# LouisBearing/BirdSoundClassif

Measured on AMD Instinct MI355X. Metric: clips/sec (3 s @ 22.05 kHz) detect fwd, higher is better.
Workload: dtype f32; 1 GPU; BASELINE.json configs[1]: 1xMI355X inference, batch=64 synthetic 3 s clips (PCM16 @22.05 kHz resident in HBM) through the HIP STFT front end + detector forward + device post-processing, detections returned to the host; batch_per_gpu=64, distinct_clips=64, lanes=2

## Files before the change

birdsoundclassif_amd/_lib.py:

```python
import ctypes as C
import os
import subprocess

_HERE = os.path.dirname(os.path.abspath(__file__))
LIB_PATH = os.environ.get('NBM_LIB') or os.path.join(_HERE, 'libnbm_hip.so')
CSRC = os.path.join(_HERE, 'csrc')

_lib = None


class GemmDesc(C.Structure):
    _fields_ = [('x', C.c_void_p), ('w', C.c_void_p), ('y', C.c_void_p),
                ('scale', C.c_void_p), ('shift', C.c_void_p), ('residual', C.c_void_p),
                ('x_gs', C.c_int64), ('w_gs', C.c_int64), ('y_gs', C.c_int64), ('res_gs', C.c_int64),
                ('groups', C.c_int),
                ('B', C.c_int), ('H', C.c_int), ('W', C.c_int), ('Cin', C.c_int),
                ('N', C.c_int),
                ('kh', C.c_int), ('kw', C.c_int), ('stride', C.c_int), ('pad', C.c_int),
                ('Ho', C.c_int), ('Wo', C.c_int),
                ('x_ld', C.c_int), ('w_ld', C.c_int), ('y_ld', C.c_int), ('res_ld', C.c_int),
                ('alpha', C.c_float), ('act', C.c_int), ('shift_per_row', C.c_int),
                ('up', C.c_void_p), ('up_H', C.c_int), ('up_W', C.c_int),
                ('rows', C.c_void_p), ('rows_blocks', C.c_void_p),
                ('rows_mode', C.c_int), ('rows_count', C.c_int), ('rows_TH', C.c_int), ('rows_TW', C.c_int),
                ('mask', C.c_void_p), ('mask_ld', C.c_int), ('bits_out', C.c_void_p)]


class GconvDesc(C.Structure):
    _fields_ = [('x', C.c_void_p), ('w', C.c_void_p), ('y', C.c_void_p), ('scale', C.c_void_p), ('shift', C.c_void_p),
                ('B', C.c_int), ('H', C.c_int), ('W', C.c_int), ('groups', C.c_int), ('Cg', C.c_int),
                ('kh', C.c_int), ('kw', C.c_int), ('stride', C.c_int), ('pad', C.c_int), ('Ho', C.c_int), ('Wo', C.c_int),
                ('x_ld', C.c_int), ('y_ld', C.c_int), ('relu', C.c_int)]


class GconvBwdDesc(C.Structure):
    _fields_ = [('g', C.c_void_p), ('y', C.c_void_p), ('w', C.c_void_p), ('x', C.c_void_p), ('out', C.c_void_p),
                ('scale', C.c_void_p), ('workspace', C.c_void_p), ('workspace_bytes', C.c_longlong),
                ('B', C.c_int), ('H', C.c_int), ('W', C.c_int), ('groups', C.c_int), ('Cg', C.c_int),
                ('kh', C.c_int), ('kw', C.c_int), ('stride', C.c_int), ('pad', C.c_int), ('Ho', C.c_int), ('Wo', C.c_int),
                ('g_ld', C.c_int), ('y_ld', C.c_int), ('x_ld', C.c_int), ('out_ld', C.c_int),
                ('accumulate', C.c_int), ('splits', C.c_int)]


class RoiDesc(C.Structure):
    _fields_ = [('fmap', C.c_void_p * 5), ('fh', C.c_int * 5), ('fw', C.c_int * 5),
                ('n_levels', C.c_int), ('C', C.c_int),
                ('rois', C.c_void_p), ('n_roi', C.c_void_p), ('B', C.c_int), ('roi_cap', C.c_int),
                ('pe_f', C.c_void_p), ('pe_t', C.c_void_p), ('img_h', C.c_int), ('img_w', C.c_int),
                ('pool', C.c_void_p), ('pe', C.c_void_p), ('level', C.c_void_p)]


class AugmentParams(C.Structure):
    _fields_ = [('gain', C.c_float), ('coef', C.c_float), ('denom', C.c_float), ('neg_coef', C.c_float),
                ('neg_denom', C.c_float), ('flags', C.c_int32), ('hard_index', C.c_int32), ('pad', C.c_int32),
                ('noise_seed', C.c_uint64)]


class BwdDesc(C.Structure):
    _fields_ = [('g', C.c_void_p), ('w', C.c_void_p), ('x', C.c_void_p), ('out', C.c_void_p),
                ('a_scale', C.c_void_p), ('row_scale', C.c_void_p), ('residual', C.c_void_p), ('mask', C.c_void_p),
                ('g_gs', C.c_int64), ('w_gs', C.c_int64), ('x_gs', C.c_int64), ('out_gs', C.c_int64), ('res_gs', C.c_int64),
                ('groups', C.c_int),
                ('B', C.c_int), ('H', C.c_int), ('W', C.c_int), ('Cin', C.c_int), ('N', C.c_int),
                ('kh', C.c_int), ('kw', C.c_int), ('stride', C.c_int), ('pad', C.c_int), ('Ho', C.c_int), ('Wo', C.c_int),
                ('g_ld', C.c_int), ('w_ld', C.c_int), ('x_ld', C.c_int), ('out_ld', C.c_int), ('res_ld', C.c_int),
                ('mask_ld', C.c_int), ('alpha', C.c_float), ('bias_grad', C.c_void_p), ('residual2', C.c_void_p), ('res2_ld', C.c_int),
                ('mask_bits', C.c_void_p)]


class GemmPlan(C.Structure):
    _fields_ = [('name', C.c_char_p), ('rc', C.c_int), ('kernel', C.c_int), ('grid', C.c_int * 3), ('block', C.c_int),
                ('m_tiles', C.c_int), ('n_tiles', C.c_int), ('vec_epi', C.c_int), ('fast', C.c_int), ('slices', C.c_int),
                ('phased', C.c_int), ('ph_tiles', C.c_int * 4), ('splits', C.c_int), ('k_chunk', C.c_int),
                ('plain', C.c_int), ('b_generic', C.c_int), ('narrow_m', C.c_int), ('halves', C.c_int)]


_P, _I, _L, _F, _U64 = C.c_void_p, C.c_int, C.c_int64, C.c_float, C.c_uint64

SIGNATURES = {
    'nbm_graph_census': [_P, C.POINTER(C.c_longlong * 6)],
    'nbm_copy_rect': [_P, _P, _L, _L, _I, _L, _L, _I, _I, _P],
    'nbm_gemm_conv': [C.POINTER(GemmDesc), _P],
    'nbm_gconv3x3': [C.POINTER(GconvDesc), _P],
    'nbm_gconv3x3_dgrad': [C.POINTER(GconvBwdDesc), _P],
    'nbm_gconv3x3_wgrad': [C.POINTER(GconvBwdDesc), _P],
    'nbm_gconv3x3_wgrad_workspace': [C.POINTER(GconvBwdDesc), C.POINTER(C.c_longlong)],
    'nbm_pcm16_to_wave': [_P, _L, _I, _I, _I, _P, _L, _L, _P, _L, _I, _I, _P],
    'nbm_resample_to_wave': [_P, _L, _I, _L, _I, _I, _P, _I, _L, _L, _P, _L, _I, _I, _I, _P],
    'nbm_wav_decode': [_P, _L, _I, _I, _I, _I, _L, _P, _L, _P],
    'nbm_minmax_init': [_P, _I, _P],
    'nbm_stft_db': [_P, _L, _I, _I, _I, _I, _P, _I, _I, _I, _F, _P, _L, _I, _P, _P],
    'nbm_spec_windows': [_P, _L, _I, _I, _I, _I, _P, _P, _I, _I, _I, _P, _P],
    'nbm_spec_windows_table': [_P, _I, _I, _P, _I, _I, _P],
    'nbm_init_conv': [_P, _L, _P, _P, _I, _P, _P],
    'nbm_stem7x7': [_P, _I, _I, _I, _P, _P, _P, _P, _P, _P, _P],
    'nbm_stem7x7_wgrad': [_P, _P, _I, _I, _I, _P, _P, _P],
    'nbm_maxpool3x3s2': [_P, _I, _I, _I, _I, _P, _I, _I, _P, _P],
    'nbm_space_to_batch2': [_P, _I, _I, _I, _I, _P, _I, _P],
    'nbm_avgpool2x2': [_P, _I, _I, _I, _I, _P, _P],
    'nbm_avgpool2x2_bwd': [_P, _I, _I, _I, _I, _P, _P],
    'nbm_upsample_bilinear_add': [_P, _I, _I, _I, _I, _P, _P, _I, _I, _P],
    'nbm_softmax_rows': [_P, _L, _I, _L, _P],
    'nbm_dwconv3x3': [_P, _I, _I, _I, _I, _I, _I, _P, _P, _P, _L, _P, _I, _I, _P],
    'nbm_silu': [_P, _P, _L, _P],
    'nbm_layernorm': [_P, _L, _I, _P, _P, _F, _P, _P],
    'nbm_mha_small': [_P, _P, _P, _I, _I, _I, _P, _I, _I, _I, _I, _I, _L, _L, _P, _F, _P],
    'nbm_mha_segments': [_P, _P, _P, _I, _I, _I, _P, _I, _I, _I, _I, _I, _I, _P, _P, _I, _F, _P],
    'nbm_pair_softmax': [_P, _L, _I, _I, _P, _I, _P],
    'nbm_rpn_decode': [_P, _P, _P, _I, _I, _I, _I, _I, _I, _P, _P, _P, _P],
    'nbm_nan_images': [_P, _I, _L, _P, _P],
    'nbm_rpn_select': [_P, _P, _P, _I, _I, _I, _I, _I, _P, _P, _P, _P, _P],
    'nbm_nms_batched': [_P, _P, _P, _I, _I, _F, _I, _P, _P, _P, _P, _P, _P, _P],
    'nbm_rpn_select_big_workspace': [_I, _I, C.POINTER(C.c_int64)],
    'nbm_rpn_select_big': [_P, _P, _P, _I, _I, _I, _I, _I, _P, _L, _P, _P, _P, _P, _P],
    'nbm_nms_big_workspace': [_I, _I, C.POINTER(C.c_int64)],
    'nbm_nms_big': [_P, _P, _P, _I, _I, _F, _I, _P, _L, _P, _P, _P, _P, _P],
    'nbm_roi_pool': [C.POINTER(RoiDesc), _P],
    'nbm_rcnn_post': [_P, _P, _I, _I, _P, _P, _I, _I, _I, _F, _F, _I, _P, _P, _P],
    'nbm_merge_collect': [_P, _P, _I, _I, _I, _I, _I, _L, _P, _P, _P, _P, _P, _P],
    'nbm_merge_nms_workspace': [_I, C.POINTER(C.c_int64)],
    'nbm_merge_nms': [_P, _P, _I, _F, _P, _L, _P, _P, _P],
    'nbm_merge_gather': [_P, _P, _P, _P, _P, _I, _P, _P, _P],
    'nbm_conv_dgrad': [C.POINTER(BwdDesc), _P],
    'nbm_conv_wgrad': [C.POINTER(BwdDesc), _P],
    'nbm_gemm_plan': [_I, _P, C.POINTER(GemmPlan)],
    'nbm_relu_bwd': [_P, _P, _P, _L, _P],
    'nbm_silu_bwd': [_P, _P, _P, _L, _P],
    'nbm_axpby': [_P, _P, _P, _F, _F, _L, _L, _P],
    'nbm_colsum': [_P, _L, _I, _I, _P, _P],
    'nbm_leaky_relu_bwd': [_P, _P, _P, _F, _L, _P],
    'nbm_layernorm_bwd': [_P, _P, _P, _L, _I, _F, _P, _P, _P, _P],
    'nbm_mha_small_bwd': [_P, _P, _P, _P, _I, _I, _I, _I, _P, _P, _P, _I, _I, _I, _P, _I, _I, _I, _I, _L, _L, _P, _F, _P],
    'nbm_zero_roi_windows': [_P, _I, _I, _I, _P, _P, _I, _I, _I, _P],
    'nbm_zero_pattern': [_P, _I, _I, _I, _I, _I, _P],
    'nbm_zero_tiles': [_P, _I, _I, _I, _I, _P, _I, _P, _P],
    'nbm_tiles_gather': [_P, _I, _I, _I, _I, _P, _I, _P, _P, _P],
    'nbm_tiles_scatter_add': [_P, _I, _I, _I, _I, _P, _I, _P, _P, _P],
    'nbm_proposal_iou': [_P, _P, _P, _I, _I, _I, _P, _P, _P],
    'nbm_anchor_targets': [_P, _I, _P, _P, _I, _I, _F, _F, _P, _P, _P, _P],
    'nbm_maxpool3x3s2_bwd': [_P, _P, _P, _I, _I, _I, _I, _I, _I, _P, _P, _P],
    'nbm_upsample_bilinear_bwd': [_P, _I, _I, _I, _I, _P, _I, _I, _I, _P],
    'nbm_tiles_upsample_bilinear_bwd_add': [_P, _I, _I, _I, _I, _P, _I, _P, _P, _I, _I, _P],
    'nbm_png_unfilter_gray8': [_P, _L, _I, _I, _I, _P, _L, _P, _P],
    'nbm_image_half_std_u8': [_P, _L, _I, _L, _P, _P],
    'nbm_randn_fill': [_U64, _L, _P, _P],
    'nbm_augment_batch': [_P, _P, _P, _I, _I, _I, _P, _P, _P, _P, _P, _P, _P],
    'nbm_u8_to_unit': [_P, _L, _P, _P],
    'nbm_wino_input': [_P, _I, _I, _I, _I, _P, _I, _P],
    'nbm_wino_output': [_P, _P, _P, _P, _I, _I, _I, _I, _I, _P, _I, _P, _P],
    'nbm_wino_outgrad': [_P, _I, _I, _I, _I, _P, _P, _I, _P],
    'nbm_wino_weight': [_P, _P, _I, _I, _I, _I, _P, _P],
    'nbm_wino_weight_grad': [_P, _P, _I, _I, _I, _P, _P],
    'nbm_wino23_rows': [_P, _I, _I, _I, _I, _P, _P],
    'nbm_wino23_conv_fused': [_P, _P, _P, _P, _P, _I, _I, _I, _I, _I, _I, _P, _I, _P],
    'nbm_wino23_rows_tiles': [_P, _I, _I, _I, _I, _P, _I, _P, _P, _P, _I, _P],
    'nbm_wino23_conv_fused_tiles': [_P, _P, _P, _P, _P, _I, _I, _I, _I, _I, _I, _P, _P, _I, _P, _P, _P],
    'nbm_roi_tiles': [_P, _P, _I, _I, _I, _I, _P, _P, _P, _I, _P, _P, _P],
    'nbm_wino23_input_tiles': [_P, _I, _I, _I, _I, _P, _I, _P, _P, _P],
    'nbm_wino23_outgrad_tiles': [_P, _I, _I, _I, _I, _P, _I, _P, _P, _P, _I, _P],
    'nbm_cell_outgrad': [_P, _I, _I, _I, _I, _I, _P, _P, _P],
    'nbm_cell_weight': [_P, _I, _I, _P, _I, _P, _I, _P],
    'nbm_cell_weight_fold': [_P, _P, _I, _I, _I, _I, _F, _P, _I, _P, _I, _P],
    'nbm_cell_weight_grad': [_P, _I, _I, _I, _P, _P],
    'nbm_cell_input': [_P, _I, _I, _I, _I, _I, _P, _I, _I, _P],
    'nbm_cell_input_up': [_P, _P, _I, _I, _I, _I, _I, _I, _I, _P, _I, _I, _P],
    'nbm_cell_patches': [_P, _I, _I, _I, _I, _I, _P, _I, _I, _P],
    'nbm_cell_patches_up': [_P, _P, _I, _I, _I, _I, _I, _I, _I, _P, _I, _I, _P],
    'nbm_cell_dgrad_output': [_P, _I, _I, _I, _I, _I, _P, _I, _I, _I, _P, _P],
    'nbm_cell_output': [_P, _P, _I, _I, _I, _I, _I, _P, _P],
    'nbm_weighted_sum': [_P, _P, _P, _P, _P, _L, _P],
    'nbm_weighted_sum_bwd': [_P, _P, _P, _P, _P, _P, _P, _P, _P, _L, _P],
    'nbm_softmax_rows_bwd': [_P, _P, _P, _L, _I, _F, _P],
    'nbm_pair_softmax_bwd': [_P, _P, _P, _L, _P],
    'nbm_dwconv3x3_bwd': [_P, _P, _P, _I, _I, _I, _I, _I, _I, _P, _P, _P, _I, _I, _P],
    'nbm_dwconv3x3_bwd_acc': [_P, _P, _I, _I, _I, _I, _I, _I, _P, _I, _I, _P],
    'nbm_film_fwd': [_P, _P, _P, _L, _I, _P],
    'nbm_film_bwd': [_P, _P, _P, _P, _P, _L, _I, _P],
    'nbm_bn_train_fwd': [_P, _L, _I, _P, _P, _F, _F, _P, _P, _P, _P, _P, _P, _P],
    'nbm_bn_train_bwd': [_P, _P, _L, _I, _P, _P, _P, _P, _P, _P, _P, _P],
    'nbm_roi_pool_bwd': [C.POINTER(C.c_void_p), C.POINTER(C.c_int), C.POINTER(C.c_int), _I, _I, _P, _P, _I, _I, _P, _P],
    'nbm_sqnorm_accum': [_P, _L, _P, _P],
    'nbm_adamw_step': [_P, _P, _P, _P, _L, _F, _F, _F, _F, _F, _I, _P, _F, _P],
}


def build(verbose=False):
    r = subprocess.run(['make', '-C', CSRC, '-j4'], capture_output=True, text=True)
    if verbose or r.returncode:
        print(r.stdout[-4000:], r.stderr[-4000:])
    if r.returncode:
        raise RuntimeError('building libnbm_hip.so failed')
    return LIB_PATH


def load():
    global _lib
    if _lib is not None:
        return _lib
    import torch
    if not os.path.isfile(LIB_PATH):
        raise RuntimeError(f'{LIB_PATH} is missing: build it with `python -c "import __graft_entry__ as g; g.build()"` '
                           '(the NBM hot path has no CPU / eager fallback)')
    lib = C.CDLL(LIB_PATH)
    lib.nbm_version.restype = C.c_char_p
    lib.nbm_version.argtypes = []
    for name, argtypes in SIGNATURES.items():
        fn = getattr(lib, name)
        fn.argtypes = argtypes
        fn.restype = C.c_int
    _lib = lib
    return lib


class NbmHipError(RuntimeError):
    pass


_CODES = {-1: 'NBM_EINVAL (bad argument / shape)', -2: 'NBM_EALIGN (pointer or pitch not 16-byte aligned)',
          -3: 'NBM_EUNSUPPORTED'}


def check(rc, name):
    if rc != 0:
        raise NbmHipError(f'{name} failed: {_CODES.get(rc, f"hipError_t {rc}")}')
```

birdsoundclassif_amd/csrc/igemm.hip:

```cpp
#include <stdlib.h>
#include "nbm_common.h"
#include "igemm_params.h"
#include "igemm_plan.h"
#include <type_traits>

namespace {

constexpr int BK = 32;
constexpr int PITCH = 36;

enum { A_FAST = 0, A_GENERIC = 1 };
enum { EPI_STD = 0 };

using nbm_igemm::IgemmParams;

template <int BM, int BN, int WM, int WN, int AMODE, int EPI, int STAGES = 2, bool ROWS = false>
__global__ __launch_bounds__(256, BM > 128 ? 1 : STAGES == 1 ? 3 : 2) void igemm_kernel(const IgemmParams p) {
  constexpr int MT = WM / 32, NT = WN / 32;
  constexpr int WAVES_N = BN / WN;
  constexpr int AR = BM / 32, BR = BN / 32;
  static_assert((BM / WM) * (BN / WN) == 4, "4 waves per workgroup");

  __shared__ __attribute__((aligned(16))) float lds[STAGES * (BM + BN) * PITCH];
  if constexpr (STAGES == 2) nbm_stagger_priority();
  float* As = lds;
  float* Bs = lds + STAGES * BM * PITCH;

  const int nwg = gridDim.x, bid = blockIdx.x;
  const int q8 = nwg >> 3, r8 = nwg & 7, xcd = bid & 7;
  const int wg = (xcd < r8 ? xcd * (q8 + 1) : r8 * (q8 + 1) + (xcd - r8) * q8) + (bid >> 3);
  int tile_m = wg / p.n_tiles, tile_n = wg - tile_m * p.n_tiles;
  auto row_pixel = [&](int m) -> long long {
    if (p.rows_mode == 1) return p.rows[m];
    const int t = p.rows[m >> 4];
    if (t < 0) return -1;
    const int thw = p.rows_TH * p.rows_TW, k = m & 15;
    const int b = (int)nbm_fdiv((unsigned)t, p.fd_rows_thw), rem = t - b * thw;
    const int ty = (int)nbm_fdiv((unsigned)rem, p.fd_rows_tw), tx = rem - ty * p.rows_TW;
    const int y = 2 * ty - 1 + (k >> 2), x = 2 * tx - 1 + (k & 3);
    if ((unsigned)y >= (unsigned)p.H || (unsigned)x >= (unsigned)p.W) return -1;
    return ((long long)b * p.H + y) * p.W + x;
  };
  if constexpr (ROWS) {
    if (p.rows_blocks) {
      const int j = bid >> 3;
      tile_n = j % p.n_tiles;
      tile_m = (j / p.n_tiles) * 8 + xcd;
      if (tile_m >= p.m_tiles || tile_m * (BM / 128) >= *p.rows_blocks * (p.rows_mode == 2 ? 16 : 1)) return;
    }
    if (p.rows[p.rows_mode == 2 ? (tile_m * BM) >> 4 : tile_m * BM] < 0) return;
  }
  const int bm0 = tile_m * BM, bn0 = tile_n * BN;
  const int g = blockIdx.z;

  const float* __restrict__ xg = p.x + (long long)g * p.x_gs;
  const float* __restrict__ wgp = p.w + (long long)g * p.w_gs;

  const int tid = threadIdx.x, lane = tid & 63, wave = tid >> 6;
  const int wm0 = (wave / WAVES_N) * WM, wn0 = (wave % WAVES_N) * WN;
  const int lrow = lane & 31, lh = lane >> 5;

  const int c4 = tid & 7, r0 = tid >> 3;
  long long a_base[AR];
  int a_iy0[AR], a_ix0[AR];
  bool a_ok[AR];
  unsigned a_rel[AR];
  unsigned long long a_taps[AR];
  long long blk_base = 0;
  if constexpr (ROWS) {
    const int e0 = p.rows[p.rows_mode == 2 ? bm0 >> 4 : bm0];
    const int b = (int)nbm_fdiv((unsigned)e0, p.rows_mode == 2 ? p.fd_rows_thw : p.fd_howo);
    blk_base = (long long)b * p.HoWo * p.x_ld;
  } else {
    const int m0 = bm0 < p.M ? bm0 : 0;
    const int b = (int)nbm_fdiv((unsigned)m0, p.fd_howo), rem = m0 - b * p.HoWo;
    const int oy = (int)nbm_fdiv((unsigned)rem, p.fd_wo), ox = rem - oy * p.Wo;
    blk_base = ((long long)(b * p.H + oy * p.stride - p.pad) * p.W + (ox * p.stride - p.pad)) * p.x_ld;
  }
#pragma unroll
  for (int i = 0; i < AR; ++i) {
    const int m = bm0 + r0 + 32 * i;
    a_ok[i] = m < p.M;
    long long mm = a_ok[i] ? m : 0;
    if constexpr (ROWS) {
      if (a_ok[i]) { mm = row_pixel(m); a_ok[i] = mm >= 0; }
      if (!a_ok[i]) mm = blk_base / p.x_ld;
    }
    const int b = (int)nbm_fdiv((unsigned)mm, p.fd_howo), rem = (int)(mm - (long long)b * p.HoWo);
    const int oy = (int)nbm_fdiv((unsigned)rem, p.fd_wo), ox = rem - oy * p.Wo;
    a_iy0[i] = oy * p.stride - p.pad;
    a_ix0[i] = ox * p.stride - p.pad;
    a_base[i] = ((long long)(b * p.H + a_iy0[i]) * p.W + a_ix0[i]) * p.x_ld;
    a_rel[i] = ((unsigned)(a_base[i] - blk_base) + c4 * 4) * 4u;
    unsigned long long mk = 0ull;
    if constexpr (AMODE == A_FAST) {
      unsigned rowm = 0u, colm = 0u;
      for (int r = 0; r < p.kh; ++r) rowm |= ((unsigned)(a_iy0[i] + r) < (unsigned)p.H ? 1u : 0u) << r;
      for (int s2 = 0; s2 < p.kw; ++s2) colm |= ((unsigned)(a_ix0[i] + s2) < (unsigned)p.W ? 1u : 0u) << s2;
      for (int r = 0; r < p.kh; ++r) mk |= ((rowm >> r) & 1u) ? (unsigned long long)colm << (r * p.kw) : 0ull;
      mk = a_ok[i] ? mk : 0ull;
    }
    a_taps[i] = mk;
  }
  const float* b_ptr[BR];
  bool b_ok[BR];
  unsigned b_rel[BR];
#pragma unroll
  for (int i = 0; i < BR; ++i) {
    const int n = bn0 + r0 + 32 * i;
    b_ok[i] = n < p.N;
    b_ptr[i] = wgp + (long long)(b_ok[i] ? n : 0) * p.w_ld + c4 * 4;
    b_rel[i] = b_ok[i] ? (unsigned)(n * p.w_ld + c4 * 4) * 4u : 0x80000000u;
  }
  const __amdgpu_buffer_rsrc_t rsrc_a = __builtin_amdgcn_make_buffer_rsrc(const_cast<float*>(xg + blk_base), 0, 0x7ffffff0, 0x00020000);
  const __amdgpu_buffer_rsrc_t rsrc_b = __builtin_amdgcn_make_buffer_rsrc(const_cast<float*>(wgp), 0, 0x7ffffff0, 0x00020000);

  f32x4 ra[AR], rb[BR];
  const f32x4 zero4 = {0.f, 0.f, 0.f, 0.f};

  int cur_r = 0, cur_s = 0, cur_c0 = 0;

  auto load_tiles = [&](int kt) {
    if constexpr (AMODE == A_FAST) {
      const int tap = cur_r * p.kw + cur_s;
      const unsigned a_soff = (unsigned)((((long long)cur_r * p.W + cur_s) * p.x_ld + cur_c0) * 4);
      const unsigned b_soff = (unsigned)((tap * p.Cin + cur_c0) * 4);
#pragma unroll
      for (int i = 0; i < AR; ++i) {
        const unsigned vo = ((a_taps[i] >> tap) & 1ull) ? a_rel[i] : 0x80000000u;
        ra[i] = __builtin_bit_cast(f32x4, __builtin_amdgcn_raw_buffer_load_b128(rsrc_a, vo, a_soff, 0));
      }
#pragma unroll
      for (int i = 0; i < BR; ++i)
        rb[i] = __builtin_bit_cast(f32x4, __builtin_amdgcn_raw_buffer_load_b128(rsrc_b, b_rel[i], b_soff, 0));
      if (++cur_s == p.kw) { cur_s = 0; if (++cur_r == p.kh) { cur_r = 0; cur_c0 += BK; } }
    } else {
      const int k0 = kt * BK + c4 * 4;
#pragma unroll
      for (int i = 0; i < AR; ++i) {
        f32x4 v = zero4;
#pragma unroll
        for (int e = 0; e < 4; ++e) {
          const int k = k0 + e;
          if (a_ok[i] && k < p.K) {
            const int tap = k / p.Cin, c = k - tap * p.Cin;
            const int r = tap / p.kw, s = tap - r * p.kw;
            const int iy = a_iy0[i] + r, ix = a_ix0[i] + s;
            if ((unsigned)iy < (unsigned)p.H && (unsigned)ix < (unsigned)p.W)
              v[e] = xg[a_base[i] + ((long long)r * p.W + s) * p.x_ld + c];
          }
        }
        ra[i] = v;
      }
#pragma unroll
      for (int i = 0; i < BR; ++i)
        rb[i] = b_ok[i] ? *reinterpret_cast<const f32x4*>(b_ptr[i] + kt * BK) : zero4;
    }
  };
  auto store_lds = [&](int buf) {
#pragma unroll
    for (int i = 0; i < AR; ++i)
      *reinterpret_cast<f32x4*>(As + (buf * BM + r0 + 32 * i) * PITCH + c4 * 4) = ra[i];
#pragma unroll
    for (int i = 0; i < BR; ++i)
      *reinterpret_cast<f32x4*>(Bs + (buf * BN + r0 + 32 * i) * PITCH + c4 * 4) = rb[i];
  };

  f32x16 acc[MT][NT];
#pragma unroll
  for (int i = 0; i < MT; ++i)
#pragma unroll
    for (int j = 0; j < NT; ++j)
#pragma unroll
      for (int e = 0; e < 16; ++e) acc[i][j][e] = 0.f;

  if constexpr (STAGES == 2) {
    load_tiles(0);
    store_lds(0);
    if (p.nk > 1) load_tiles(1);
  }

  auto mfma_group = [&](const float* Ab, const float* Bb, int q) {
    f32x4 a[MT], b[NT];
#pragma unroll
    for (int i = 0; i < MT; ++i) a[i] = *reinterpret_cast<const f32x4*>(Ab + i * 32 * PITCH + q * 4);
#pragma unroll
    for (int j = 0; j < NT; ++j) b[j] = *reinterpret_cast<const f32x4*>(Bb + j * 32 * PITCH + q * 4);
#pragma unroll
    for (int e = 0; e < 4; ++e)
#pragma unroll
      for (int i = 0; i < MT; ++i)
#pragma unroll
        for (int j = 0; j < NT; ++j)
          acc[i][j] = __builtin_amdgcn_mfma_f32_32x32x2f32(a[i][e], b[j][e], acc[i][j], 0, 0, 0);
  };

  auto k_step = [&](int kt, auto store_c, auto load_c) {
    constexpr bool STORE = decltype(store_c)::value, LOAD = decltype(load_c)::value;
    const int cur = kt & 1;
    __syncthreads();
    const float* Ab = As + (cur * BM + wm0 + lrow) * PITCH + lh * 16;
    const float* Bb = Bs + (cur * BN + wn0 + lrow) * PITCH + lh * 16;
    mfma_group(Ab, Bb, 0);
    if constexpr (STORE) {
      store_lds(cur ^ 1);
      __builtin_amdgcn_sched_group_barrier(0x100, MT + NT, 0);
#pragma unroll
      for (int z = 0; z < AR + BR; ++z) {
        __builtin_amdgcn_sched_group_barrier(0x008, (4 * MT * NT) / (AR + BR) > 0 ? (4 * MT * NT) / (AR + BR) : 1, 0);
        __builtin_amdgcn_sched_group_barrier(0x200, 1, 0);
      }
    }
    __builtin_amdgcn_sched_barrier(0);
    mfma_group(Ab, Bb, 1);
    if constexpr (LOAD) {
      load_tiles(kt + 2);
      __builtin_amdgcn_sched_group_barrier(0x100, MT + NT, 0);
#pragma unroll
      for (int z = 0; z < AR + BR; ++z) {
        __builtin_amdgcn_sched_group_barrier(0x008, (4 * MT * NT) / (AR + BR) > 0 ? (4 * MT * NT) / (AR + BR) : 1, 0);
        __builtin_amdgcn_sched_group_barrier(0x002, 3, 0);
        __builtin_amdgcn_sched_group_barrier(0x020, 1, 0);
      }
    }
    __builtin_amdgcn_sched_barrier(0);
    mfma_group(Ab, Bb, 2);
    mfma_group(Ab, Bb, 3);
  };
  if constexpr (STAGES == 2) {
    using T = std::true_type;
    using F = std::false_type;
    int kt = 0;
    for (; kt + 2 < p.nk; ++kt) k_step(kt, T{}, T{});
    if (p.nk >= 2) { k_step(kt, T{}, F{}); ++kt; }
    k_step(kt, F{}, F{});
  } else {
    load_tiles(0);
    for (int kt = 0; kt < p.nk; ++kt) {
      if (kt) __syncthreads();
      store_lds(0);
      if (kt + 1 < p.nk) load_tiles(kt + 1);
      __syncthreads();
      const float* Ab = As + (wm0 + lrow) * PITCH + lh * 16;
      const float* Bb = Bs + (wn0 + lrow) * PITCH + lh * 16;
#pragma unroll
      for (int q = 0; q < 4; ++q) mfma_group(Ab, Bb, q);
    }
  }
  __syncthreads();

#define NBM_EPI_LDS_FLOATS (STAGES * (BM + BN) * PITCH)
#include "igemm_epilogue.inc"
#undef NBM_EPI_LDS_FLOATS
}

struct StreamParams {
  const float* x; const float* w; float* y; const float* scale; const float* shift; const float* residual;
  int M, x_ld, w_ld, y_ld, res_ld, m_tiles; float alpha; int act;
  unsigned* bits_out; int n_words;
};
constexpr int SPITCH = 36;
template <int K32, int NT, int NTG, int WAVES>
__global__ __launch_bounds__(WAVES * 64, 1) void stream1x1_kernel(const StreamParams p) {
  constexpr int K = K32 * 32, N = NT * 32, WP = K + 4;
  constexpr bool CHUNKED = K32 > 2;
  static_assert(NT % NTG == 0 && (!CHUNKED || NTG == NT), "groups");
  __shared__ __attribute__((aligned(16))) float Ws[N * WP];
  __shared__ __attribute__((aligned(16))) float Stg[WAVES][32 * SPITCH];
  __shared__ __attribute__((aligned(16))) unsigned Bw[WAVES][32 * NT];
  const int tid = threadIdx.x, lane = tid & 63, wave = tid >> 6, li = lane & 31, lh = lane >> 5;
  const int n_off = blockIdx.y * N;
  for (int i = tid; i < N * (K / 4); i += WAVES * 64) {
    const int n = i / (K / 4), c = i - n * (K / 4);
    *reinterpret_cast<f32x4*>(Ws + n * WP + c * 4) = *reinterpret_cast<const f32x4*>(p.w + (long long)(n_off + n) * p.w_ld + c * 4);
  }
  __syncthreads();
  float* stg = Stg[wave];
  const int er = lane >> 3, ec = (lane & 7) * 4;
  f32x4 a[K32][4], an[CHUNKED ? 1 : K32][4];
  auto row_ptr = [&](int tile) {
    int m = tile * 32 + li;
    m = m < p.M ? m : p.M - 1;
    return p.x + (long long)m * p.x_ld + 16 * lh;
  };
  auto load_chunk = [&](const float* xp, int kc, f32x4* dst) {
#pragma unroll
    for (int q = 0; q < 4; ++q) dst[q] = *reinterpret_cast<const f32x4*>(xp + kc * 32 + 4 * q);
  };
  const int step = gridDim.x * WAVES;
  int tile = blockIdx.x * WAVES + wave;
  if (tile < p.m_tiles) {
    const float* xp = row_ptr(tile);
#pragma unroll
    for (int kc = 0; kc < K32; ++kc) load_chunk(xp, kc, CHUNKED ? a[kc] : an[kc]);
  }
  for (; tile < p.m_tiles; tile += step) {
    const bool more = tile + step < p.m_tiles;
    const float* xn = row_ptr(more ? tile + step : tile);
    if constexpr (!CHUNKED) {
#pragma unroll
      for (int kc = 0; kc < K32; ++kc)
#pragma unroll
        for (int q = 0; q < 4; ++q) a[kc][q] = an[kc][q];
#pragma unroll
      for (int kc = 0; kc < K32; ++kc) load_chunk(xn, kc, an[kc]);
    }
    const int m0 = tile * 32;
    f32x4 rq[NTG][4];
    auto load_res = [&](int jj, f32x4* dst) {
      if (!p.residual) return;
#pragma unroll
      for (int pass = 0; pass < 4; ++pass) {
        const int m = m0 + pass * 8 + er;
        dst[pass] = *reinterpret_cast<const f32x4*>(p.residual + (long long)(m < p.M ? m : p.M - 1) * p.res_ld + n_off + jj * 32 + ec);
      }
    };
#pragma unroll
    for (int g = 0; g < NT / NTG; ++g) {
#pragma unroll
      for (int j = 0; j < NTG; ++j) load_res(g * NTG + j, rq[j]);
      f32x16 acc[NTG];
#pragma unroll
      for (int j = 0; j < NTG; ++j)
#pragma unroll
        for (int e = 0; e < 16; ++e) acc[j][e] = 0.f;
      if constexpr (CHUNKED) {
#pragma unroll
        for (int kc = 0; kc < K32; ++kc) {
#pragma unroll
          for (int j = 0; j < NTG; ++j) {
            const float* wb = Ws + (j * 32 + li) * WP + 16 * lh + kc * 32;
            f32x4 b[4];
#pragma unroll
            for (int q = 0; q < 4; ++q) b[q] = *reinterpret_cast<const f32x4*>(wb + 4 * q);
#pragma unroll
            for (int q = 0; q < 4; ++q)
#pragma unroll
              for (int e = 0; e < 4; ++e) acc[j] = __builtin_amdgcn_mfma_f32_32x32x2f32(a[kc][q][e], b[q][e], acc[j], 0, 0, 0);
          }
          __builtin_amdgcn_sched_barrier(0);
          load_chunk(xn, kc, a[kc]);
          __builtin_amdgcn_sched_barrier(0);
        }
      } else {
#pragma unroll
        for (int j = 0; j < NTG; ++j) {
          const float* wb = Ws + ((g * NTG + j) * 32 + li) * WP + 16 * lh;
#pragma unroll
          for (int kc = 0; kc < K32; ++kc) {
            f32x4 b[4];
#pragma unroll
            for (int q = 0; q < 4; ++q) b[q] = *reinterpret_cast<const f32x4*>(wb + kc * 32 + 4 * q);
#pragma unroll
            for (int q = 0; q < 4; ++q)
#pragma unroll
              for (int e = 0; e < 4; ++e) acc[j] = __builtin_amdgcn_mfma_f32_32x32x2f32(a[kc][q][e], b[q][e], acc[j], 0, 0, 0);
          }
        }
      }
#pragma unroll
      for (int j = 0; j < NTG; ++j) {
        const int jj = g * NTG + j;
        __builtin_amdgcn_fence(__ATOMIC_ACQ_REL, "wavefront");
#pragma unroll
        for (int e = 0; e < 16; ++e) stg[((e & 3) + 8 * (e >> 2) + 4 * lh) * SPITCH + li] = acc[j][e];
        __builtin_amdgcn_fence(__ATOMIC_ACQ_REL, "wavefront");
        const int n = n_off + jj * 32 + ec;
        f32x4 sc = {1.f, 1.f, 1.f, 1.f}, sh = {0.f, 0.f, 0.f, 0.f};
        if (p.scale) sc = *reinterpret_cast<const f32x4*>(p.scale + n);
        if (p.shift) sh = *reinterpret_cast<const f32x4*>(p.shift + n);
#pragma unroll
        for (int pass = 0; pass < 4; ++pass) {
          const int r = pass * 8 + er, m = m0 + r;
          if (m >= p.M) continue;
          f32x4 v = *reinterpret_cast<const f32x4*>(stg + r * SPITCH + ec);
#pragma unroll
          for (int e = 0; e < 4; ++e) v[e] = (v[e] * p.alpha) * sc[e] + sh[e] + 0.f;
          if (p.residual) { v[0] += rq[j][pass][0]; v[1] += rq[j][pass][1]; v[2] += rq[j][pass][2]; v[3] += rq[j][pass][3]; }
          if (p.act == NBM_ACT_RELU) {
#pragma unroll
            for (int e = 0; e < 4; ++e) v[e] = fmaxf(v[e], 0.0f);
          } else if (p.act == NBM_ACT_SILU) {
#pragma unroll
            for (int e = 0; e < 4; ++e) v[e] = v[e] / (1.0f + expf(-v[e]));
          } else if (p.act == NBM_ACT_LEAKY) {
#pragma unroll
            for (int e = 0; e < 4; ++e) v[e] = v[e] > 0.f ? v[e] : 0.01f * v[e];
          }
          if (p.bits_out) {
            const int grp8 = 8 * er;
            const unsigned wb = ((unsigned)(__builtin_amdgcn_ballot_w64(v[0] > 0.f) >> grp8) & 0xffu) |
                                (((unsigned)(__builtin_amdgcn_ballot_w64(v[1] > 0.f) >> grp8) & 0xffu) << 8) |
                                (((unsigned)(__builtin_amdgcn_ballot_w64(v[2] > 0.f) >> grp8) & 0xffu) << 16) |
                                (((unsigned)(__builtin_amdgcn_ballot_w64(v[3] > 0.f) >> grp8) & 0xffu) << 24);
            if (ec == 0) Bw[wave][r * NT + jj] = wb;
          }
          *reinterpret_cast<f32x4*>(p.y + (long long)m * p.y_ld + n) = v;
        }
      }
    }
    if (p.bits_out) {
      static_assert(NT >= 2 && NT % 2 == 0, "two lanes per tile row");
      constexpr int WPL = NT / 2;
      __builtin_amdgcn_fence(__ATOMIC_ACQ_REL, "wavefront");
      const int r = lane >> 1, j0 = (lane & 1) * WPL;
      const int m = m0 + r;
      if (m < p.M) {
        unsigned* dst = p.bits_out + (long long)m * p.n_words + (n_off >> 5) + j0;
        const unsigned* src = Bw[wave] + r * NT + j0;
        if constexpr (WPL == 4) *reinterpret_cast<uint4*>(dst) = *reinterpret_cast<const uint4*>(src);
        else if constexpr (WPL == 2) *reinterpret_cast<uint2*>(dst) = *reinterpret_cast<const uint2*>(src);
        else {
#pragma unroll
          for (int q = 0; q < WPL; ++q) dst[q] = src[q];
        }
      }
      __builtin_amdgcn_fence(__ATOMIC_ACQ_REL, "wavefront");
    }
  }
}

}

using namespace nbm_igemm;

extern "C" int nbm_gemm_conv(const nbm_gemm_desc* d, void* stream) {
  if (!d) return NBM_EINVAL;
  const GemmPlan pl = plan_fwd(*d, read_gemm_switches(0));
  if (pl.rc) return pl.rc;
  if (pl.halves) {
    nbm_gemm_desc a = *d, b = *d;
    const int n0 = d->N - 64;
    a.N = n0;
    b.N = 64;
    b.w = d->w + (long long)n0 * d->w_ld;
    b.y = d->y + n0;
    if (d->scale) b.scale = d->scale + n0;
    if (d->shift) b.shift = d->shift + n0;
    if (d->residual) b.residual = d->residual + n0;
    if (d->mask) b.mask = d->mask + n0;
    const int rc = nbm_gemm_conv(&a, stream);
    return rc ? rc : nbm_gemm_conv(&b, stream);
  }
  const dim3 grid(pl.grid[0], pl.grid[1], pl.grid[2]), block(pl.block);
  hipStream_t st = (hipStream_t)stream;
  const int M = d->B * d->Ho * d->Wo;
  if (pl.slices) {
    const StreamParams sp{d->x, d->w, d->y, d->scale, d->shift, d->residual, M, d->x_ld, d->w_ld, d->y_ld, d->res_ld, pl.m_tiles,
                          d->alpha, d->act, d->bits_out, d->N >> 5};
    switch (pl.kernel) {
      case K_STREAM_64_256: hipLaunchKernelGGL((stream1x1_kernel<2, 8, 4, 8>), grid, block, 0, st, sp); break;
      case K_STREAM_64_64: hipLaunchKernelGGL((stream1x1_kernel<2, 2, 2, 8>), grid, block, 0, st, sp); break;
      case K_STREAM_128_SLICED: hipLaunchKernelGGL((stream1x1_kernel<4, 4, 4, 8>), grid, block, 0, st, sp); break;
      default: hipLaunchKernelGGL((stream1x1_kernel<8, 2, 2, 8>), grid, block, 0, st, sp); break;
    }
    return nbm_launch_status();
  }
  IgemmParams p{};
  p.x = d->x; p.w = d->w; p.y = d->y; p.scale = d->scale; p.shift = d->shift; p.residual = d->residual;
  p.x_gs = d->x_gs; p.w_gs = d->w_gs; p.y_gs = d->y_gs; p.res_gs = d->res_gs;
  p.M = M; p.N = d->N; p.K = d->kh * d->kw * d->Cin;
  p.nk = (p.K + BK - 1) / BK;
  p.H = d->H; p.W = d->W; p.Cin = d->Cin; p.kh = d->kh; p.kw = d->kw; p.stride = d->stride; p.pad = d->pad;
  p.Ho = d->Ho; p.Wo = d->Wo; p.HoWo = d->Ho * d->Wo;
  p.fd_howo = nbm_fastdiv_make((unsigned)p.HoWo); p.fd_wo = nbm_fastdiv_make((unsigned)p.Wo);
  p.x_ld = d->x_ld; p.w_ld = d->w_ld; p.y_ld = d->y_ld; p.res_ld = d->res_ld;
  p.alpha = d->alpha; p.act = d->act; p.shift_per_row = d->shift_per_row;
  p.m_tiles = pl.m_tiles; p.n_tiles = pl.n_tiles; p.vec_epi = pl.vec_epi;
  if (d->mask) { p.mask = d->mask; p.mask_ld = d->mask_ld; }
  p.bits_out = d->bits_out;
  if (d->up) {
    p.up = d->up; p.up_H = d->up_H; p.up_W = d->up_W;
    p.up_sh = d->Ho > 1 ? (float)(d->up_H - 1) / (float)(d->Ho - 1) : 0.f;
    p.up_sw = d->Wo > 1 ? (float)(d->up_W - 1) / (float)(d->Wo - 1) : 0.f;
  }
  if (d->rows) {
    p.rows = d->rows; p.rows_blocks = d->rows_blocks; p.rows_mode = d->rows_mode; p.rows_TH = d->rows_TH; p.rows_TW = d->rows_TW;
    p.fd_rows_thw = nbm_fastdiv_make((unsigned)(d->rows_TH * d->rows_TW)); p.fd_rows_tw = nbm_fastdiv_make((unsigned)d->rows_TW);
    p.M = d->rows_count;
  }
  switch (pl.kernel) {
    case K_FWD_ROWS: hipLaunchKernelGGL((igemm_kernel<128, 128, 64, 64, A_FAST, EPI_STD, 1, true>), grid, block, 0, st, p); break;
    case K_FWD_SPLIT_R0: case K_FWD_SPLIT_R2: case K_FWD_SPLIT_R4: return split_launch(p, pl, st);
    case K_FWD_H16: return h16_launch(p, pl, st);
    case K_FWD_128_S1: hipLaunchKernelGGL((igemm_kernel<128, 128, 64, 64, A_FAST, EPI_STD, 1>), grid, block, 0, st, p); break;
    case K_FWD_128_FAST: hipLaunchKernelGGL((igemm_kernel<128, 128, 64, 64, A_FAST, EPI_STD>), grid, block, 0, st, p); break;
    case K_FWD_128_GENERIC: hipLaunchKernelGGL((igemm_kernel<128, 128, 64, 64, A_GENERIC, EPI_STD>), grid, block, 0, st, p); break;
    case K_FWD_64_S1: hipLaunchKernelGGL((igemm_kernel<128, 64, 64, 32, A_FAST, EPI_STD, 1>), grid, block, 0, st, p); break;
    case K_FWD_64_FAST: hipLaunchKernelGGL((igemm_kernel<128, 64, 64, 32, A_FAST, EPI_STD>), grid, block, 0, st, p); break;
    case K_FWD_64_GENERIC: hipLaunchKernelGGL((igemm_kernel<128, 64, 64, 32, A_GENERIC, EPI_STD>), grid, block, 0, st, p); break;
    case K_FWD_32_FAST: hipLaunchKernelGGL((igemm_kernel<128, 32, 32, 32, A_FAST, EPI_STD>), grid, block, 0, st, p); break;
    case K_FWD_32_GENERIC: hipLaunchKernelGGL((igemm_kernel<128, 32, 32, 32, A_GENERIC, EPI_STD>), grid, block, 0, st, p); break;
    default: return NBM_EINVAL;
  }
  return nbm_launch_status();
}

extern "C" int nbm_gemm_plan(int kind, const void* desc, nbm_gemm_plan_t* out) {
  if (!desc || !out || kind < 0 || kind > 2) return NBM_EINVAL;
  const GemmSwitches sw = read_gemm_switches(kind);
  *out = kind == 0 ? plan_fwd(*(const nbm_gemm_desc*)desc, sw)
         : kind == 1 ? plan_dgrad(*(const nbm_bwd_desc*)desc, sw) : plan_wgrad(*(const nbm_bwd_desc*)desc, sw);
  return out->rc;
}
```

birdsoundclassif_amd/csrc/igemm_h16.hip:

```cpp
#include <stdlib.h>
#include "nbm_common.h"
#include "igemm_params.h"
#include <type_traits>

namespace {

using nbm_igemm::IgemmParams;
constexpr int BM = 128, BN = 128, WM = 64, WN = 64, MT = 2, NT = 2;
constexpr int P16 = 20;
enum { EPI_STD = 0 };

__global__ __launch_bounds__(256, 3) void igemm_h16_kernel(const IgemmParams p) {
  constexpr int STAGES = 1, EPI = EPI_STD;
  constexpr bool ROWS = false;
  __shared__ __attribute__((aligned(16))) float lds[2 * (BM + BN) * P16];
  float* As = lds;
  float* Bs = lds + 2 * BM * P16;

  const int nwg = gridDim.x, bid = blockIdx.x;
  const int q8 = nwg >> 3, r8 = nwg & 7, xcd = bid & 7;
  const int wg = (xcd < r8 ? xcd * (q8 + 1) : r8 * (q8 + 1) + (xcd - r8) * q8) + (bid >> 3);
  const int tile_m = wg / p.n_tiles, tile_n = wg - tile_m * p.n_tiles;
  const int bm0 = tile_m * BM, bn0 = tile_n * BN;
  const int g = blockIdx.z;
  const float* __restrict__ xg = p.x + (long long)g * p.x_gs;
  const float* __restrict__ wgp = p.w + (long long)g * p.w_gs;
  auto row_pixel = [&](int m) -> long long { return m; };

  const int tid = threadIdx.x, lane = tid & 63, wave = tid >> 6;
  const int wm0 = (wave >> 1) * WM, wn0 = (wave & 1) * WN;
  const int lrow = lane & 31, lh = lane >> 5;

  const int c = tid & 3, r0 = tid >> 2;
  const int koff = c < 2 ? 4 * c : 16 + 4 * (c - 2);
  long long blk_base;
  {
    const int m0 = bm0 < p.M ? bm0 : 0;
    const int b = (int)nbm_fdiv((unsigned)m0, p.fd_howo), rem = m0 - b * p.HoWo;
    const int oy = (int)nbm_fdiv((unsigned)rem, p.fd_wo), ox = rem - oy * p.Wo;
    blk_base = ((long long)(b * p.H + oy * p.stride - p.pad) * p.W + (ox * p.stride - p.pad)) * p.x_ld;
  }
  unsigned a_rel[2], b_rel[2];
  unsigned long long a_taps[2];
#pragma unroll
  for (int i = 0; i < 2; ++i) {
    const int m = bm0 + r0 + 64 * i;
    const bool ok = m < p.M;
    const int mm = ok ? m : 0;
    const int b = (int)nbm_fdiv((unsigned)mm, p.fd_howo), rem = mm - b * p.HoWo;
    const int oy = (int)nbm_fdiv((unsigned)rem, p.fd_wo), ox = rem - oy * p.Wo;
    const int iy0 = oy * p.stride - p.pad, ix0 = ox * p.stride - p.pad;
    const long long base = ((long long)(b * p.H + iy0) * p.W + ix0) * p.x_ld;
    a_rel[i] = ((unsigned)(base - blk_base) + koff) * 4u;
    unsigned rowm = 0u, colm = 0u;
    unsigned long long mk = 0ull;
    for (int r = 0; r < p.kh; ++r) rowm |= ((unsigned)(iy0 + r) < (unsigned)p.H ? 1u : 0u) << r;
    for (int s2 = 0; s2 < p.kw; ++s2) colm |= ((unsigned)(ix0 + s2) < (unsigned)p.W ? 1u : 0u) << s2;
    for (int r = 0; r < p.kh; ++r) mk |= ((rowm >> r) & 1u) ? (unsigned long long)colm << (r * p.kw) : 0ull;
    a_taps[i] = ok ? mk : 0ull;
    const int n = bn0 + r0 + 64 * i;
    b_rel[i] = n < p.N ? (unsigned)(n * p.w_ld + koff) * 4u : 0x80000000u;
  }
  const __amdgpu_buffer_rsrc_t rsrc_a = __builtin_amdgcn_make_buffer_rsrc(const_cast<float*>(xg + blk_base), 0, 0x7ffffff0, 0x00020000);
  const __amdgpu_buffer_rsrc_t rsrc_b = __builtin_amdgcn_make_buffer_rsrc(const_cast<float*>(wgp), 0, 0x7ffffff0, 0x00020000);

  f32x4 ra[2], rb[2];
  int cur_r = 0, cur_s = 0, cur_c0 = 0, cur_h = 0;
  auto load_tiles = [&]() {
    const int tap = cur_r * p.kw + cur_s;
    const unsigned a_soff = (unsigned)((((long long)cur_r * p.W + cur_s) * p.x_ld + cur_c0 + 8 * cur_h) * 4);
    const unsigned b_soff = (unsigned)((tap * p.Cin + cur_c0 + 8 * cur_h) * 4);
#pragma unroll
    for (int i = 0; i < 2; ++i) {
      const unsigned vo = ((a_taps[i] >> tap) & 1ull) ? a_rel[i] : 0x80000000u;
      ra[i] = __builtin_bit_cast(f32x4, __builtin_amdgcn_raw_buffer_load_b128(rsrc_a, vo, a_soff, 0));
    }
#pragma unroll
    for (int i = 0; i < 2; ++i)
      rb[i] = __builtin_bit_cast(f32x4, __builtin_amdgcn_raw_buffer_load_b128(rsrc_b, b_rel[i], b_soff, 0));
    if (cur_h ^= 1, cur_h == 0) {
      if (++cur_s == p.kw) { cur_s = 0; if (++cur_r == p.kh) { cur_r = 0; cur_c0 += 32; } }
    }
  };
  auto store_lds = [&](int buf) {
#pragma unroll
    for (int i = 0; i < 2; ++i) {
      *reinterpret_cast<f32x4*>(As + (buf * BM + r0 + 64 * i) * P16 + c * 4) = ra[i];
      *reinterpret_cast<f32x4*>(Bs + (buf * BN + r0 + 64 * i) * P16 + c * 4) = rb[i];
    }
  };

  f32x16 acc[MT][NT];
#pragma unroll
  for (int i = 0; i < MT; ++i)
#pragma unroll
    for (int j = 0; j < NT; ++j)
#pragma unroll
      for (int e = 0; e < 16; ++e) acc[i][j][e] = 0.f;

  auto mfma_group = [&](const float* Ab, const float* Bb, int q) {
    f32x4 a[MT], b[NT];
#pragma unroll
    for (int i = 0; i < MT; ++i) a[i] = *reinterpret_cast<const f32x4*>(Ab + i * 32 * P16 + q * 4);
#pragma unroll
    for (int j = 0; j < NT; ++j) b[j] = *reinterpret_cast<const f32x4*>(Bb + j * 32 * P16 + q * 4);
#pragma unroll
    for (int e = 0; e < 4; ++e)
#pragma unroll
      for (int i = 0; i < MT; ++i)
#pragma unroll
        for (int j = 0; j < NT; ++j)
          acc[i][j] = __builtin_amdgcn_mfma_f32_32x32x2f32(a[i][e], b[j][e], acc[i][j], 0, 0, 0);
  };

  auto h_step = [&](int t, auto store_c, auto load_c) {
    constexpr bool STORE = decltype(store_c)::value, LOAD = decltype(load_c)::value;
    const int cur = t & 1;
    __syncthreads();
    const float* Ab = As + (cur * BM + wm0 + lrow) * P16 + lh * 8;
    const float* Bb = Bs + (cur * BN + wn0 + lrow) * P16 + lh * 8;
    mfma_group(Ab, Bb, 0);
    if constexpr (STORE) {
      store_lds(cur ^ 1);
      __builtin_amdgcn_sched_group_barrier(0x100, MT + NT, 0);
#pragma unroll
      for (int z = 0; z < 4; ++z) {
        __builtin_amdgcn_sched_group_barrier(0x008, 4, 0);
        __builtin_amdgcn_sched_group_barrier(0x200, 1, 0);
      }
    }
    __builtin_amdgcn_sched_barrier(0);
    mfma_group(Ab, Bb, 1);
    if constexpr (LOAD) {
      load_tiles();
      __builtin_amdgcn_sched_group_barrier(0x100, MT + NT, 0);
#pragma unroll
      for (int z = 0; z < 4; ++z) {
        __builtin_amdgcn_sched_group_barrier(0x008, 4, 0);
        __builtin_amdgcn_sched_group_barrier(0x002, 3, 0);
        __builtin_amdgcn_sched_group_barrier(0x020, 1, 0);
      }
    }
    __builtin_amdgcn_sched_barrier(0);
  };
  {
    using T = std::true_type;
    using F = std::false_type;
    const int S = 2 * p.nk;
    load_tiles();
    store_lds(0);
    load_tiles();
    int t = 0;
    for (; t + 2 < S; ++t) h_step(t, T{}, T{});
    h_step(t, T{}, F{});
    ++t;
    h_step(t, F{}, F{});
  }
  __syncthreads();

#define NBM_EPI_LDS_FLOATS (2 * (BM + BN) * P16)
#include "igemm_epilogue.inc"
#undef NBM_EPI_LDS_FLOATS
}

}

int nbm_igemm::h16_launch(const IgemmParams& p, const GemmPlan& pl, hipStream_t st) {
  hipLaunchKernelGGL(igemm_h16_kernel, dim3(pl.grid[0], pl.grid[1], pl.grid[2]), dim3(256), 0, st, p);
  return nbm_launch_status();
}
```

birdsoundclassif_amd/csrc/igemm_params.h:

```cpp
#pragma once
#include "nbm_common.h"
#include "igemm_plan.h"

namespace nbm_igemm {

struct IgemmParams {
  const float* x; const float* w; float* y;
  const float* scale; const float* shift; const float* residual;
  long long x_gs, w_gs, y_gs, res_gs;
  int M, N, K;
  int nk;
  int H, W, Cin, kh, kw, stride, pad, Ho, Wo, HoWo;
  int x_ld, w_ld, y_ld, res_ld;
  int m_tiles, n_tiles;
  float alpha; int act; int shift_per_row;
  int vec_epi;
  const float* up; int up_H, up_W; float up_sh, up_sw;
  const int* rows; const int* rows_blocks; int rows_mode, rows_TH, rows_TW;
  const float* mask; int mask_ld;
  unsigned* bits_out;
  nbm_fastdiv fd_howo, fd_wo, fd_rows_thw, fd_rows_tw;
};

int split_launch(const IgemmParams& p, const GemmPlan& pl, hipStream_t st);

int h16_launch(const IgemmParams& p, const GemmPlan& pl, hipStream_t st);

}
```

birdsoundclassif_amd/csrc/igemm_plan.h:

```cpp
#pragma once
#include <stdint.h>
#include <stdlib.h>
#include "nbm_hip.h"

namespace nbm_igemm {

struct GemmSwitches { bool stream1x1, split_bf16, h16, nn_h16, split_tn; };
constexpr GemmSwitches kDefaultSwitches = {true, false, true, true, true};
inline bool switch_on(const char* v, bool dflt) { return dflt ? !(v && v[0] == '0') : (v && v[0] == '1'); }
inline GemmSwitches read_gemm_switches(int kind) {
  GemmSwitches s = kDefaultSwitches;
  if (kind == 0) {
    s.stream1x1 = switch_on(getenv("NBM_STREAM1X1"), true);
    s.split_bf16 = switch_on(getenv("NBM_SPLIT_BF16"), false);
    s.h16 = switch_on(getenv("NBM_H16"), true);
  } else if (kind == 1) {
    s.nn_h16 = switch_on(getenv("NBM_NN_H16"), true);
  } else {
    s.split_bf16 = switch_on(getenv("NBM_SPLIT_BF16"), false);
    s.split_tn = switch_on(getenv("NBM_SPLIT_TN"), true);
  }
  return s;
}

#define NBM_GEMM_KERNELS(X)                                                                                                          \
  X(K_FWD_ROWS, "igemm_kernel<128,128,64,64,0,0,1,true>")                                        \
  X(K_STREAM_64_256, "stream1x1_kernel<2,8,4,8>")                                          \
  X(K_STREAM_64_64, "stream1x1_kernel<2,2,2,8>")                                                \
  X(K_STREAM_256_64, "stream1x1_kernel<8,2,2,8>")                                                                     \
  X(K_STREAM_128_SLICED, "stream1x1_kernel<4,4,4,8>")                   \
  X(K_STREAM_256_SLICED, "stream1x1_kernel<8,2,2,8>")                     \
  X(K_FWD_SPLIT_R0, "igemm_split_kernel<0>")                                                        \
  X(K_FWD_SPLIT_R2, "igemm_split_kernel<2>")                                                                                         \
  X(K_FWD_SPLIT_R4, "igemm_split_kernel<4>")                                                                                         \
  X(K_FWD_H16, "igemm_h16_kernel")                                                                 \
  X(K_FWD_128_S1, "igemm_kernel<128,128,64,64,0,0,1,false>")                                              \
  X(K_FWD_128_FAST, "igemm_kernel<128,128,64,64,0,0,2,false>")                                                       \
  X(K_FWD_128_GENERIC, "igemm_kernel<128,128,64,64,1,0,2,false>")                                                                    \
  X(K_FWD_64_S1, "igemm_kernel<128,64,64,32,0,0,1,false>")                                                                           \
  X(K_FWD_64_FAST, "igemm_kernel<128,64,64,32,0,0,2,false>")                                                                         \
  X(K_FWD_64_GENERIC, "igemm_kernel<128,64,64,32,1,0,2,false>")                                                                      \
  X(K_FWD_32_FAST, "igemm_kernel<128,32,32,32,0,0,2,false>")                                                                         \
  X(K_FWD_32_GENERIC, "igemm_kernel<128,32,32,32,1,0,2,false>")                                                                      \
  X(K_NN_128_S1, "igemm_nn_kernel<128,1,false>")                                                                                     \
  X(K_NN_128_H16, "igemm_nn_kernel<128,2,true>")                                                                                     \
  X(K_NN_128, "igemm_nn_kernel<128,2,false>")                                                                                        \
  X(K_NN_64_S1, "igemm_nn_kernel<64,1,false>")                                                                                       \
  X(K_NN_64_H16, "igemm_nn_kernel<64,2,true>")                                                                                       \
  X(K_NN_64, "igemm_nn_kernel<64,2,false>")                                                                                          \
  X(K_TN_GENERIC, "igemm_tn_kernel<64,2,128>")                                                                                       \
  X(K_TN_128_SAME_M64, "igemm_tn_kernel<128,0,64>")                                                                                  \
  X(K_TN_128_STRIDED_M64, "igemm_tn_kernel<128,1,64>")                                                                               \
  X(K_TN_64_SAME_M64, "igemm_tn_kernel<64,0,64>")                                                                                    \
  X(K_TN_64_STRIDED_M64, "igemm_tn_kernel<64,1,64>")                                                                                 \
  X(K_TN_128_SAME, "igemm_tn_kernel<128,0,128>")                                                                                     \
  X(K_TN_128_STRIDED, "igemm_tn_kernel<128,1,128>")                                                                                  \
  X(K_TN_64_SAME, "igemm_tn_kernel<64,0,128>")                                                                                       \
  X(K_TN_64_STRIDED, "igemm_tn_kernel<64,1,128>")                                                                                    \
  X(K_SPLIT_TN_R0, "igemm_split_tn_kernel<0>")                              \
  X(K_SPLIT_TN_R2, "igemm_split_tn_kernel<2>")                                                                                       \
  X(K_SPLIT_TN_R4, "igemm_split_tn_kernel<4>")

enum GemmKernel {
#define X(id, name) id,
  NBM_GEMM_KERNELS(X)
#undef X
  K_COUNT
};
inline const char* gemm_kernel_name(int k) {
  static const char* const names[] = {
#define X(id, name) name,
      NBM_GEMM_KERNELS(X)
#undef X
  };
  return k >= 0 && k < K_COUNT ? names[k] : "";
}

constexpr int PLAN_BK = 32;
constexpr int SHORTK_STEPS = 8, DEEPK_STEPS = SHORTK_STEPS + 1;
constexpr int SHORTK_STEPS_64 = 20;
constexpr int SHORTK_STEPS_PHASED = 16;
constexpr int DEEPK_MAX_TAPS = 63;
constexpr int STREAM_MIN_ROWS = 8192;
constexpr int SPLIT_TN_MIN_ROWS = 192;
constexpr long long ROWS_SPAN_MAX = 0x7fffffffll;
constexpr long long DGRAD_SPAN_MAX = 0x70000000ll;
constexpr long long TN_SPAN_MAX = 0x40000000ll;

inline bool aligned16(const void* p) { return (((uintptr_t)p) & 15u) == 0; }

using GemmPlan = nbm_gemm_plan_t;

inline GemmPlan plan_error(int rc) {
  GemmPlan pl{};
  pl.rc = rc;
  pl.kernel = -1;
  pl.name = "";
  return pl;
}
inline void plan_kernel(GemmPlan& pl, int kernel, int gx, int gy, int gz, int block = 256) {
  pl.kernel = kernel;
  pl.name = gemm_kernel_name(kernel);
  pl.grid[0] = gx; pl.grid[1] = gy; pl.grid[2] = gz;
  pl.block = block;
}

inline GemmPlan plan_fwd(const nbm_gemm_desc& d, GemmSwitches sw) {
  if (!d.x || !d.w || !d.y) return plan_error(NBM_EINVAL);
  if (d.B <= 0 || d.H <= 0 || d.W <= 0 || d.Cin <= 0 || d.N <= 0 || d.kh <= 0 || d.kw <= 0 || d.stride <= 0 || d.Ho <= 0 || d.Wo <= 0 ||
      d.groups <= 0)
    return plan_error(NBM_EINVAL);
  if ((d.H + 2 * d.pad - d.kh) / d.stride + 1 != d.Ho || (d.W + 2 * d.pad - d.kw) / d.stride + 1 != d.Wo) return plan_error(NBM_EINVAL);
  if (d.x_ld < d.Cin || d.y_ld < d.N || (d.residual && d.res_ld < d.N)) return plan_error(NBM_EINVAL);
  GemmPlan pl{};
  const int taps = d.kh * d.kw, K = taps * d.Cin, nk = (K + PLAN_BK - 1) / PLAN_BK;
  if (d.N > 128 && (d.N & 127) == 64 && !d.rows && !d.up && !d.bits_out && !d.shift_per_row && (d.Cin % PLAN_BK) == 0 && K > SHORTK_STEPS * PLAN_BK) {
    nbm_gemm_desc a = d;
    a.N = d.N - 64;
    pl = plan_fwd(a, sw);
    pl.halves = 1;
    return pl;
  }
  if (d.w_ld < nk * PLAN_BK) return plan_error(NBM_EINVAL);
  if (d.mask && (d.rows || d.groups != 1 || d.mask_ld < d.N)) return plan_error(NBM_EUNSUPPORTED);
  pl.vec_epi = ((d.N & 3) == 0 && (d.y_ld & 3) == 0 && (d.y_gs & 3) == 0 && aligned16(d.y) &&
                (!d.residual || ((d.res_ld & 3) == 0 && (d.res_gs & 3) == 0 && aligned16(d.residual))) &&
                (!d.scale || aligned16(d.scale)) && (!d.shift || d.shift_per_row || aligned16(d.shift)) &&
                (!d.mask || ((d.mask_ld & 3) == 0 && aligned16(d.mask))))
                   ? 1 : 0;
  if ((d.w_ld & 3) || (d.w_gs & 3) || !aligned16(d.w)) return plan_error(NBM_EALIGN);
  if (d.bits_out && (!pl.vec_epi || (d.N & 31) || d.groups != 1 || d.rows)) return plan_error(NBM_EUNSUPPORTED);
  if (d.up && (!pl.vec_epi || d.groups != 1 || d.up_H <= 0 || d.up_W <= 0 || !aligned16(d.up))) return plan_error(NBM_EUNSUPPORTED);
  pl.fast = ((d.Cin % PLAN_BK) == 0 && (d.x_ld & 3) == 0 && (d.x_gs & 3) == 0 && aligned16(d.x)) ? 1 : 0;
  const bool fast_vec = pl.fast && pl.vec_epi;
  const int M = d.B * d.Ho * d.Wo;
  pl.m_tiles = (M + 127) / 128;
  if (d.rows) {
    if (d.kh != 1 || d.kw != 1 || d.stride != 1 || d.pad != 0 || d.groups != 1 || !fast_vec || d.shift_per_row || nk > SHORTK_STEPS ||
        d.N <= 64 || (d.rows_mode != 1 && d.rows_mode != 2) || d.rows_count <= 0 || (d.rows_count % 128))
      return plan_error(NBM_EUNSUPPORTED);
    if (d.rows_mode == 2 && (d.rows_TH != (d.H + 1) / 2 || d.rows_TW != (d.W + 1) / 2)) return plan_error(NBM_EINVAL);
    if (2ll * d.H * d.W * d.x_ld * 4 > ROWS_SPAN_MAX) return plan_error(NBM_EUNSUPPORTED);
    pl.m_tiles = d.rows_count / 128;
    pl.n_tiles = (d.N + 127) / 128;
    plan_kernel(pl, K_FWD_ROWS, (d.rows_blocks ? (pl.m_tiles + 7) / 8 * 8 : pl.m_tiles) * pl.n_tiles, 1, 1);
    return pl;
  }
  if (sw.stream1x1 && d.kh == 1 && d.kw == 1 && d.stride == 1 && d.pad == 0 && d.groups == 1 && fast_vec && !d.up && !d.mask &&
      !d.shift_per_row && (d.N % 32) == 0 && M >= STREAM_MIN_ROWS) {
    const int k32 = d.Cin / 32, nt = d.N / 32;
    int kernel = -1, wg_per_cu = 1, slices = 1;
    if (k32 == 2 && nt == 8 && d.residual) kernel = K_STREAM_64_256;
    else if (k32 == 2 && nt == 2) kernel = K_STREAM_64_64, wg_per_cu = 2;
    else if (k32 == 8 && nt == 2) kernel = K_STREAM_256_64;
    else if (d.residual && k32 == 4 && nt % 4 == 0 && nt <= 32) kernel = K_STREAM_128_SLICED, slices = nt / 4;
    else if (d.residual && k32 == 8 && nt % 2 == 0 && nt <= 64) kernel = K_STREAM_256_SLICED, slices = nt / 2;
    if (kernel >= 0) {
      const int waves = 8;
      pl.m_tiles = (M + 31) / 32;
      pl.slices = slices;
      const int wgs = (pl.m_tiles + waves - 1) / waves;
      int gx = 256 * wg_per_cu / slices;
      if (gx < 1) gx = 1;
      plan_kernel(pl, kernel, wgs < gx ? wgs : gx, slices, 1, waves * 64);
      return pl;
    }
  }
  if (d.N > 64) {
    pl.n_tiles = (d.N + 127) / 128;
    const bool deep = fast_vec && nk >= DEEPK_STEPS && taps < DEEPK_MAX_TAPS;
    if (sw.split_bf16 && deep) {
      pl.m_tiles = (M + 255) / 256;
      const int rem = (2 * nk) % 6;
      plan_kernel(pl, rem == 0 ? K_FWD_SPLIT_R0 : rem == 2 ? K_FWD_SPLIT_R2 : K_FWD_SPLIT_R4, pl.m_tiles * pl.n_tiles, 1, d.groups);
    }
    else if (sw.h16 && deep) plan_kernel(pl, K_FWD_H16, pl.m_tiles * pl.n_tiles, 1, d.groups);
    else if (fast_vec && nk <= SHORTK_STEPS) plan_kernel(pl, K_FWD_128_S1, pl.m_tiles * pl.n_tiles, 1, d.groups);
    else plan_kernel(pl, pl.fast ? K_FWD_128_FAST : K_FWD_128_GENERIC, pl.m_tiles * pl.n_tiles, 1, d.groups);
  } else if (d.N > 32) {
    pl.n_tiles = 1;
    if (fast_vec && nk <= SHORTK_STEPS_64) plan_kernel(pl, K_FWD_64_S1, pl.m_tiles, 1, d.groups);
    else plan_kernel(pl, pl.fast ? K_FWD_64_FAST : K_FWD_64_GENERIC, pl.m_tiles, 1, d.groups);
  } else {
    pl.n_tiles = 1;
    plan_kernel(pl, pl.fast ? K_FWD_32_FAST : K_FWD_32_GENERIC, pl.m_tiles, 1, d.groups);
  }
  return pl;
}

inline int check_bwd_common(const nbm_bwd_desc& d) {
  if (!d.g || !d.out) return NBM_EINVAL;
  if (d.B <= 0 || d.H <= 0 || d.W <= 0 || d.Cin <= 0 || d.N <= 0 || d.kh <= 0 || d.kw <= 0 || d.stride <= 0 || d.groups <= 0 ||
      d.kh * d.kw > 64)
    return NBM_EINVAL;
  if ((d.H + 2 * d.pad - d.kh) / d.stride + 1 != d.Ho || (d.W + 2 * d.pad - d.kw) / d.stride + 1 != d.Wo) return NBM_EINVAL;
  return NBM_OK;
}

inline GemmPlan plan_dgrad(const nbm_bwd_desc& d, GemmSwitches sw) {
  if (int rc = check_bwd_common(d)) return plan_error(rc);
  if (!d.w) return plan_error(NBM_EINVAL);
  if ((d.g_ld & 3) || d.g_ld < ((d.N + 31) / 32) * 32 || (d.Cin & 3) || (d.w_ld & 3) || (d.g_gs & 3) || (d.w_gs & 3) || !aligned16(d.g) ||
      !aligned16(d.w) || (d.a_scale && !aligned16(d.a_scale)))
    return plan_error(NBM_EALIGN);
  if (d.out_ld < d.Cin || (d.residual && d.res_ld < d.Cin) || (d.mask && d.mask_ld < d.Cin)) return plan_error(NBM_EINVAL);
  if (d.residual2 && (d.stride != 1 || d.groups != 1 || d.res2_ld < d.Cin)) return plan_error(NBM_EINVAL);
  if (d.a_scale && (d.N & 31)) return plan_error(NBM_EINVAL);
  if (d.mask_bits && ((d.Cin & 31) || d.groups != 1)) return plan_error(NBM_EUNSUPPORTED);
  {
    const long long row = (long long)d.Wo * d.g_ld * 4;
    const long long span = (d.W == 1 && d.kh == 1) ? 130ll * d.g_ld * 4
                                                    : (d.kh + 130) * row + (long long)d.Ho * row;
    if (span > DGRAD_SPAN_MAX) return plan_error(NBM_EUNSUPPORTED);
  }
  GemmPlan pl{};
  pl.vec_epi = ((d.out_ld & 3) == 0 && (d.out_gs & 3) == 0 && aligned16(d.out) &&
                (!d.residual || ((d.res_ld & 3) == 0 && (d.res_gs & 3) == 0 && aligned16(d.residual))) &&
                (!d.mask || ((d.mask_ld & 3) == 0 && aligned16(d.mask))) &&
                (!d.residual2 || ((d.res2_ld & 3) == 0 && aligned16(d.residual2)))) ? 1 : 0;
  pl.m_tiles = (d.B * d.H * d.W + 127) / 128;
  if (d.stride == 2) {
    pl.phased = 1;
    int tmax = 0;
    for (int ph = 0; ph < 4; ++ph) {
      const int y0 = ((ph >> 1) + d.pad) & 1, x0 = ((ph & 1) + d.pad) & 1;
      const int Hp = (d.H - y0 + 1) >> 1, Wp = (d.W - x0 + 1) >> 1;
      pl.ph_tiles[ph] = (int)(((long long)d.B * Hp * Wp + 127) / 128);
      if (pl.ph_tiles[ph] > tmax) tmax = pl.ph_tiles[ph];
    }
    pl.m_tiles = 4 * tmax;
  }
  const int n_steps = (d.N + PLAN_BK - 1) / PLAN_BK;
  const int ph_max = n_steps * ((d.kh + 1) / 2) * ((d.kw + 1) / 2);
  const bool shortk = pl.vec_epi && (pl.phased ? ph_max <= SHORTK_STEPS_PHASED
                                               : n_steps * d.kh * d.kw <= (d.Cin <= 64 ? SHORTK_STEPS_64 : SHORTK_STEPS));
  const bool hs = sw.nn_h16 && pl.vec_epi;
  const bool wide = d.Cin > 64;
  pl.n_tiles = wide ? (d.Cin + 127) / 128 : 1;
  plan_kernel(pl, wide ? (shortk ? K_NN_128_S1 : hs ? K_NN_128_H16 : K_NN_128) : (shortk ? K_NN_64_S1 : hs ? K_NN_64_H16 : K_NN_64),
              pl.m_tiles * pl.n_tiles, 1, d.groups);
  return pl;
}

inline int best_split(int M, int tiles, int slots, int rows_per_split_min) {
  const int max_splits = (M + rows_per_split_min - 1) / rows_per_split_min;
  int splits = 1;
  double best = -1.0;
  for (int sp = 1; sp <= max_splits && (long long)sp * tiles <= 16ll * slots; ++sp) {
    const long long wg = (long long)sp * tiles;
    const long long rounds = (wg + slots - 1) / slots;
    const double fill = (double)wg / (double)(rounds * slots);
    if (fill > best + 0.005) { best = fill; splits = sp; }
  }
  return splits;
}
inline void plan_splits(GemmPlan& pl, int M, int tiles, int slots, int rows_per_split_min) {
  const int sp = best_split(M, tiles, slots, rows_per_split_min);
  pl.k_chunk = (((M + sp - 1) / sp) + PLAN_BK - 1) / PLAN_BK * PLAN_BK;
  pl.splits = (M + pl.k_chunk - 1) / pl.k_chunk;
}

inline GemmPlan plan_wgrad(const nbm_bwd_desc& d, GemmSwitches sw) {
  if (int rc = check_bwd_common(d)) return plan_error(rc);
  if (!d.x) return plan_error(NBM_EINVAL);
  if ((d.g_ld & 3) || (d.g_gs & 3) || !aligned16(d.g) || d.g_ld < ((d.N + 3) / 4) * 4) return plan_error(NBM_EALIGN);
  GemmPlan pl{};
  pl.b_generic = ((d.Cin & 3) || (d.x_ld & 3) || (d.x_gs & 3) || !aligned16(d.x)) ? 1 : 0;
  const int taps = d.kh * d.kw;
  if (d.out_ld < taps * d.Cin) return plan_error(NBM_EINVAL);
  pl.plain = (taps == 1 && d.stride == 1 && d.pad == 0) ? 1 : 0;
  if (pl.plain && !pl.b_generic && d.Cin > 128 && (d.Cin & 127) == 64) {
    nbm_bwd_desc a = d;
    a.Cin = d.Cin - 64;
    pl = plan_wgrad(a, sw);
    pl.halves = 1;
    return pl;
  }
  const int M = d.B * d.Ho * d.Wo;
  if (sw.split_bf16 && sw.split_tn && pl.plain && !pl.b_generic && !d.bias_grad && d.N >= SPLIT_TN_MIN_ROWS && d.Cin > 64 && d.out_ld >= d.Cin &&
      32ll * d.g_ld * 4 < TN_SPAN_MAX && 32ll * d.x_ld * 4 < TN_SPAN_MAX) {
    pl.m_tiles = (d.N + 255) / 256;
    pl.n_tiles = (d.Cin + 127) / 128;
    plan_splits(pl, M, pl.m_tiles * pl.n_tiles * d.groups, 256, 16 * 32);
    const int rem = (pl.k_chunk >> 4) % 6;
    plan_kernel(pl, rem == 0 ? K_SPLIT_TN_R0 : rem == 2 ? K_SPLIT_TN_R2 : K_SPLIT_TN_R4, pl.m_tiles * pl.n_tiles, pl.splits, d.groups);
    return pl;
  }
  pl.narrow_m = (d.N <= 64 && !pl.b_generic) ? 1 : 0;
  pl.m_tiles = pl.narrow_m ? 1 : (d.N + 127) / 128;
  const bool wide = !pl.b_generic && d.Cin > 64;
  const int BN = wide ? 128 : 64;
  pl.n_tiles = pl.b_generic ? (taps * d.Cin + BN - 1) / BN : taps * ((d.Cin + BN - 1) / BN);
  plan_splits(pl, M, pl.m_tiles * pl.n_tiles * d.groups, 512, 8 * PLAN_BK);
  const bool same = !pl.b_generic && d.stride == 1 && d.Ho == d.H && d.Wo == d.W && (d.Wo >= PLAN_BK || pl.plain) &&
                    (long long)PLAN_BK * d.x_ld * 4 < TN_SPAN_MAX;
  const int kernel = pl.b_generic ? K_TN_GENERIC
                     : pl.narrow_m ? (wide ? (same ? K_TN_128_SAME_M64 : K_TN_128_STRIDED_M64) : (same ? K_TN_64_SAME_M64 : K_TN_64_STRIDED_M64))
                                   : (wide ? (same ? K_TN_128_SAME : K_TN_128_STRIDED) : (same ? K_TN_64_SAME : K_TN_64_STRIDED));
  plan_kernel(pl, kernel, pl.m_tiles * pl.n_tiles, pl.splits, d.groups);
  return pl;
}

}
```

birdsoundclassif_amd/csrc/pointwise.hip:

```cpp
#include <stdlib.h>
#include "nbm_common.h"

namespace {

constexpr int TPB = 256;
inline int grid_for(long long n, int per_block = TPB, int cap = 256 * 16) {
  long long g = (n + per_block - 1) / per_block;
  return (int)(g < 1 ? 1 : (g > cap ? cap : g));
}

__device__ __forceinline__ int pcm16_sample(const int16_t* __restrict__ x, int n, int upsample,
                                            const int32_t* __restrict__ hq, long long i) {
  if (!upsample) return x[i];
  if ((i & 1) == 0) return x[i >> 1];
  const int n0 = (int)(i >> 1);
  long long acc = 0;
#pragma unroll
  for (int k = 0; k < 16; ++k) {
    const int ia = n0 - k, ib = n0 + 1 + k;
    const int va = x[min(max(ia, 0), n - 1)], vb = x[min(max(ib, 0), n - 1)];
    const int xa = (ia >= 0 && ia < n) ? va : 0;
    const int xb = (ib >= 0 && ib < n) ? vb : 0;
    acc += (long long)hq[k] * (xa + xb);
  }
// ... 235 lines not shown
    long long t = pix;
    const int ox = (int)(t % Wo); t /= Wo;
    const int oy = (int)(t % Ho);
    const int b = (int)(t / Ho);
    const int ci = o / mult;
    float acc = 0.f;
#pragma unroll
    for (int r = 0; r < 3; ++r) {
      const int iy = oy * stride - 1 + r;
      if ((unsigned)iy >= (unsigned)H) continue;
#pragma unroll
      for (int s = 0; s < 3; ++s) {
        const int ix = ox * stride - 1 + s;
        if ((unsigned)ix >= (unsigned)W) continue;
        acc += x[((long long)(b * H + iy) * W + ix) * Cin + ci] * w[o * 9 + r * 3 + s];
      }
    }
    if (bias) acc += bias[o];
    if (film) acc = acc * film[pix * film_ld + o] + film[pix * film_ld + Cout + o];
    y[i] = acc;
  }
}

template <int MULT>
__global__ void dwconv3x3_vec_kernel(const float* __restrict__ x, int B, int H, int W, int Cin, int stride,
                                     const float* __restrict__ w, const float* __restrict__ bias,
                                     const float* __restrict__ film, long long film_ld, float* __restrict__ y,
                                     int Ho, int Wo) {
  constexpr int NIN = 4 / MULT;
  const int Cout = Cin * MULT, C4 = Cout >> 2;
  const long long total = (long long)B * Ho * Wo * C4;
  const long long gstride = (long long)gridDim.x * blockDim.x;
  const bool fixed_chunk = (gstride % C4) == 0;
  float wr[4][9];
  int w_chunk = -1;
  for (long long i = blockIdx.x * (long long)blockDim.x + threadIdx.x; i < total; i += gstride) {
    const int c4 = (int)(i % C4);
    const long long pix = i / C4;
    long long t = pix;
    const int ox = (int)(t % Wo); t /= Wo;
    const int oy = (int)(t % Ho);
    const int b = (int)(t / Ho);
    const int o0 = c4 * 4, ci0 = o0 / MULT;
    if (!fixed_chunk || w_chunk != c4) {
#pragma unroll
      for (int j = 0; j < 4; ++j)
#pragma unroll
        for (int k = 0; k < 9; ++k) wr[j][k] = w[(o0 + j) * 9 + k];
      w_chunk = c4;
    }
    float acc[4] = {0.f, 0.f, 0.f, 0.f};
    float xv[9][NIN];
#pragma unroll
    for (int r = 0; r < 3; ++r) {
      const int iyc = min(max(oy * stride - 1 + r, 0), H - 1);
#pragma unroll
      for (int s = 0; s < 3; ++s) {
        const int ixc = min(max(ox * stride - 1 + s, 0), W - 1);
        const float* xp = x + ((long long)(b * H + iyc) * W + ixc) * Cin + ci0;
        float* v = xv[r * 3 + s];
        if constexpr (NIN == 4) {
          const f32x4 q = *reinterpret_cast<const f32x4*>(xp);
          v[0] = q[0]; v[1] = q[1]; v[2] = q[2]; v[3] = q[3];
        } else if constexpr (NIN == 2) {
          const float2 q = *reinterpret_cast<const float2*>(xp);
          v[0] = q.x; v[1] = q.y;
        } else {
          v[0] = *xp;
        }
      }
    }
#pragma unroll
    for (int r = 0; r < 3; ++r) {
      const bool oky = (unsigned)(oy * stride - 1 + r) < (unsigned)H;
#pragma unroll
      for (int s = 0; s < 3; ++s) {
        const bool ok = oky && (unsigned)(ox * stride - 1 + s) < (unsigned)W;
#pragma unroll
        for (int j = 0; j < 4; ++j) acc[j] += (ok ? xv[r * 3 + s][j / MULT] : 0.f) * wr[j][r * 3 + s];
      }
    }
    f32x4 out = {acc[0], acc[1], acc[2], acc[3]};
    if (bias) {
      const f32x4 bv = *reinterpret_cast<const f32x4*>(bias + o0);
      out += bv;
    }
    if (film) {
      const f32x4 ga = *reinterpret_cast<const f32x4*>(film + pix * film_ld + o0);
      const f32x4 be = *reinterpret_cast<const f32x4*>(film + pix * film_ld + Cout + o0);
#pragma unroll
      for (int j = 0; j < 4; ++j) out[j] = out[j] * ga[j] + be[j];
    }
    *reinterpret_cast<f32x4*>(y + i * 4) = out;
  }
}

__global__ void layernorm_kernel(const float* __restrict__ x, long long rows, int E, const float* __restrict__ w,
                                 const float* __restrict__ b, float eps, float* __restrict__ y) {
  const int lane = threadIdx.x & 63;
  for (long long row = blockIdx.x * 4ll + (threadIdx.x >> 6); row < rows; row += (long long)gridDim.x * 4) {
    const float* r = x + row * E;
    float s = 0.f;
    for (int c = lane; c < E; c += 64) s += r[c];
    const float mean = nbm_wave_sum(s) / (float)E;
    float q = 0.f;
    for (int c = lane; c < E; c += 64) { const float d = r[c] - mean; q += d * d; }
    const float rstd = 1.0f / sqrtf(nbm_wave_sum(q) / (float)E + eps);
    float* o = y + row * E;
    for (int c = lane; c < E; c += 64) o[c] = (r[c] - mean) * rstd * w[c] + b[c];
  }
}

#define MHA_SMAX 128
__global__ __launch_bounds__(256) void mha_small_kernel(const float* __restrict__ q, const float* __restrict__ k,
                                                        const float* __restrict__ v, int q_ld, int k_ld, int v_ld,
                                                        float* __restrict__ out, int out_ld, int S, int nhead, int hd,
                                                        long long seq_stride, long long batch_stride,
                                                        const int* __restrict__ n_valid, float scale) {
  __shared__ float Ks[MHA_SMAX][65];
  __shared__ float Vs[MHA_SMAX][64];
  __shared__ float qs[4][64];
  __shared__ float ps[4][MHA_SMAX];
  const int n = blockIdx.x / nhead, h = blockIdx.x - n * nhead;
  const int nv = n_valid ? min(*n_valid, S) : S;
  const int lane = threadIdx.x & 63, wave = threadIdx.x >> 6;
  for (int i = threadIdx.x; i < nv * hd; i += 256) {
    const int j = i / hd, d = i - j * hd;
    const long long row = j * seq_stride + n * batch_stride;
    Ks[j][d] = k[row * k_ld + h * hd + d];
    Vs[j][d] = v[row * v_ld + h * hd + d];
  }
  __syncthreads();
  for (int r = wave; r < nv; r += 4) {
    const long long row = r * seq_stride + n * batch_stride;
    if (lane < hd) qs[wave][lane] = q[row * q_ld + h * hd + lane] * scale;
    __builtin_amdgcn_wave_barrier();
    float sc[MHA_SMAX / 64];
    float m = -INFINITY;
#pragma unroll
    for (int t = 0; t < MHA_SMAX / 64; ++t) {
      const int j = lane + 64 * t;
      float a = -INFINITY;
      if (j < nv) {
        a = 0.f;
        for (int d = 0; d < hd; ++d) a += qs[wave][d] * Ks[j][d];
      }
      sc[t] = a;
      m = fmaxf(m, a);
    }
    m = nbm_wave_max(m);
    float sum = 0.f;
#pragma unroll
    for (int t = 0; t < MHA_SMAX / 64; ++t) {
      const int j = lane + 64 * t;
      const float e = j < nv ? expf(sc[t] - m) : 0.f;
      if (j < nv) ps[wave][j] = e;
      sum += e;
    }
    sum = nbm_wave_sum(sum);
    __builtin_amdgcn_wave_barrier();
    if (lane < hd) {
      float o = 0.f;
      for (int j = 0; j < nv; ++j) o += ps[wave][j] * Vs[j][lane];
      out[row * out_ld + h * hd + lane] = o / sum;
    }
    __builtin_amdgcn_wave_barrier();
  }
}

#define MHA_SHORT 8
__device__ __forceinline__ void mha_segments_row(const float* __restrict__ qrow, float* __restrict__ orow, int hd, int nv,
                                                 float scale, const float (*Kp)[65], const float (*Vp)[64], float* qsw,
                                                 float* psw, int lane) {
  if (lane < hd) qsw[lane] = qrow[lane] * scale;
  __builtin_amdgcn_wave_barrier();
  float sc[MHA_SMAX / 64];
  float m = -INFINITY;
#pragma unroll
  for (int t = 0; t < MHA_SMAX / 64; ++t) {
    const int j = lane + 64 * t;
    float a = -INFINITY;
    if (j < nv) {
      a = 0.f;
      for (int d = 0; d < hd; ++d) a += qsw[d] * Kp[j][d];
    }
    sc[t] = a;
    m = fmaxf(m, a);
  }
  m = nbm_wave_max(m);
  float sum = 0.f;
#pragma unroll
  for (int t = 0; t < MHA_SMAX / 64; ++t) {
    const int j = lane + 64 * t;
    const float e = j < nv ? expf(sc[t] - m) : 0.f;
    if (j < nv) psw[j] = e;
    sum += e;
  }
  sum = nbm_wave_sum(sum);
  __builtin_amdgcn_wave_barrier();
  if (lane < hd) {
    float o = 0.f;
    for (int j = 0; j < nv; ++j) o += psw[j] * Vp[j][lane];
    orow[lane] = o / sum;
  }
  __builtin_amdgcn_wave_barrier();
}

__global__ __launch_bounds__(256) void mha_segments_kernel(const float* __restrict__ q, const float* __restrict__ k,
                                                           const float* __restrict__ v, int q_ld, int k_ld, int v_ld,
                                                           float* __restrict__ out, int out_ld, int B, int R, int nhead,
                                                           int hd, int mode, const int* __restrict__ segments,
                                                           const int* __restrict__ n_roi, int max_count, float scale) {
  __shared__ float Ks[MHA_SMAX][65];
  __shared__ float Vs[MHA_SMAX][64];
  __shared__ float qs[4][64];
  __shared__ float ps[4][MHA_SMAX];
  const int b = blockIdx.x / nhead, h = blockIdx.x - b * nhead;
  const int lane = threadIdx.x & 63, wave = threadIdx.x >> 6;
  const long long col = (long long)h * hd;
  int first = b, cnt = 1;
  bool ok = true;
  if (mode == NBM_MHA_ACROSS_IMAGES) {
    first = segments[b];
    cnt = segments[B + b];
    ok = first >= 0 && first <= b && cnt >= 1 && cnt <= max_count && b - first < cnt && first + cnt <= B;
  }
  const int n = ok ? min(max(n_roi[first], 0), R) : 0;
  for (int r = n + wave; r < R; r += 4)
    if (lane < hd) out[((long long)b * R + r) * out_ld + col + lane] = 0.f;
  if (mode == NBM_MHA_ACROSS_ROIS) {
    const long long row0 = (long long)b * R;
    for (int i = threadIdx.x; i < n * hd; i += 256) {
      const int j = i / hd, d = i - j * hd;
      Ks[j][d] = k[(row0 + j) * k_ld + col + d];
      Vs[j][d] = v[(row0 + j) * v_ld + col + d];
    }
    __syncthreads();
    for (int r = wave; r < n; r += 4)
      mha_segments_row(q + (row0 + r) * q_ld + col, out + (row0 + r) * out_ld + col, hd, n, scale, Ks, Vs, qs[wave],
                           ps[wave], lane);
    return;
  }
  const int me = b - first;
  if (cnt <= MHA_SHORT) {
    float(*Kw)[65] = Ks + wave * MHA_SHORT;
    float(*Vw)[64] = Vs + wave * MHA_SHORT;
    for (int r = me + wave * cnt; r < n; r += 4 * cnt) {
      if (lane < hd)
        for (int j = 0; j < cnt; ++j) {
          const long long row = (long long)(first + j) * R + r;
          Kw[j][lane] = k[row * k_ld + col + lane];
          Vw[j][lane] = v[row * v_ld + col + lane];
        }
      __builtin_amdgcn_wave_barrier();
      for (int i = 0; i < cnt; ++i) {
        const long long row = (long long)(first + i) * R + r;
        mha_segments_row(q + row * q_ld + col, out + row * out_ld + col, hd, cnt, scale, Kw, Vw, qs[wave], ps[wave], lane);
      }
    }
    return;
  }
  for (int r = me; r < n; r += cnt) {
    __syncthreads();
    for (int i = threadIdx.x; i < cnt * hd; i += 256) {
      const int j = i / hd, d = i - j * hd;
      const long long row = (long long)(first + j) * R + r;
      Ks[j][d] = k[row * k_ld + col + d];
      Vs[j][d] = v[row * v_ld + col + d];
    }
    __syncthreads();
    for (int i = wave; i < cnt; i += 4) {
      const long long row = (long long)(first + i) * R + r;
      mha_segments_row(q + row * q_ld + col, out + row * out_ld + col, hd, cnt, scale, Ks, Vs, qs[wave], ps[wave], lane);
    }
  }
}

__global__ void silu_kernel(const float* __restrict__ x, float* __restrict__ y, long long n) {
  for (long long i = blockIdx.x * (long long)blockDim.x + threadIdx.x; i < n;
       i += (long long)gridDim.x * blockDim.x) {
    const float v = x[i];
    y[i] = v / (1.0f + expf(-v));
  }
}

__global__ void pair_softmax_kernel(const float* __restrict__ x, long long n_pix, int n_anchor, int x_ld,
                                    float* __restrict__ y, int y_ld) {
  const long long total = n_pix * n_anchor;
  for (long long i = blockIdx.x * (long long)blockDim.x + threadIdx.x; i < total;
       i += (long long)gridDim.x * blockDim.x) {
    const long long p = i / n_anchor;
    const int a = (int)(i - p * n_anchor);
    const float v0 = x[p * x_ld + 2 * a], v1 = x[p * x_ld + 2 * a + 1];
    const float m = fmaxf(v0, v1);
    const float e0 = expf(v0 - m), e1 = expf(v1 - m);
    const float s = e0 + e1;
    y[p * y_ld + 2 * a] = e0 / s;
    y[p * y_ld + 2 * a + 1] = e1 / s;
  }
}

}

extern "C" const char* nbm_version(void) { return "nbm_hip 0.5 (gfx950)"; }

extern "C" int nbm_graph_census(void* graph, long long counts[6]) {
  if (!graph || !counts) return NBM_EINVAL;
  for (int i = 0; i < 6; ++i) counts[i] = 0;
  size_t n = 0;
  hipError_t e = hipGraphGetNodes((hipGraph_t)graph, nullptr, &n);
  if (e != hipSuccess) return (int)e;
  if (!n) return NBM_OK;
  hipGraphNode_t* nodes = (hipGraphNode_t*)malloc(n * sizeof(hipGraphNode_t));
  if (!nodes) return NBM_EINVAL;
  e = hipGraphGetNodes((hipGraph_t)graph, nodes, &n);
  for (size_t i = 0; e == hipSuccess && i < n; ++i) {
    hipGraphNodeType t;
    e = hipGraphNodeGetType(nodes[i], &t);
    if (e != hipSuccess) break;
    const int k = t == hipGraphNodeTypeKernel ? 0 : t == hipGraphNodeTypeMemcpy ? 1 : t == hipGraphNodeTypeMemset ? 2
                : t == hipGraphNodeTypeHost ? 3 : t == hipGraphNodeTypeEmpty ? 4 : 5;
    counts[k] += 1;
  }
  free(nodes);
  return e == hipSuccess ? NBM_OK : (int)e;
}

extern "C" int nbm_pcm16_to_wave(const int16_t* pcm, int64_t pcm_ld, int batch, int n, int upsample,
                                 const int32_t* hq, int64_t first, int64_t count, float* out, int64_t out_ld, int lead,
                                 int pad_mode, void* stream) {
  if (!pcm || !out || batch <= 0 || n <= 0 || lead < 0 || (upsample && !hq)) return NBM_EINVAL;
  const int64_t n_out = upsample ? 2 * (int64_t)n : n;
  if (first < 0 || count <= 0 || first + count > n_out) return NBM_EINVAL;
  if (pad_mode != 0 && pad_mode != 1) return NBM_EINVAL;
  if ((int64_t)lead + count + (pad_mode ? lead : 0) > out_ld) return NBM_EINVAL;
  if (pad_mode == 1 && lead >= count) return NBM_EINVAL;
  dim3 grid(grid_for(out_ld, TPB, 1024), batch);
  hipLaunchKernelGGL(pcm16_to_wave_kernel, grid, dim3(TPB), 0, (hipStream_t)stream, pcm, (long long)pcm_ld, n,
                     upsample, hq, (long long)first, (long long)count, out, (long long)out_ld, lead, pad_mode);
  return nbm_launch_status();
}

extern "C" int nbm_resample_to_wave(const float* x, int64_t x_ld, int batch, int64_t n, int L, int M, const double* taps,
                                    int T, int64_t first, int64_t count, float* out, int64_t out_ld, int lead, int pad_mode,
                                    int quant16, void* stream) {
  if (!x || !out || batch <= 0 || n <= 0 || L <= 0 || M <= 0 || lead < 0) return NBM_EINVAL;
  const bool copy = L == 1 && M == 1;
  if (!copy && (!taps || T <= 0 || (T & 1))) return NBM_EINVAL;
  const int64_t n_out = copy ? n : (n * L + M - 1) / M;
  if (first < 0 || count <= 0 || first + count > n_out) return NBM_EINVAL;
  if (pad_mode != 0 && pad_mode != 1) return NBM_EINVAL;
  if ((int64_t)lead + count + (pad_mode ? lead : 0) > out_ld) return NBM_EINVAL;
  if (pad_mode == 1 && lead >= count) return NBM_EINVAL;
  dim3 grid(grid_for(out_ld, TPB, 1024), batch);
  hipLaunchKernelGGL(resample_to_wave_kernel, grid, dim3(TPB), 0, (hipStream_t)stream, x, (long long)x_ld, (long long)n, L,
                     M, taps, T, (long long)first, (long long)count, out, (long long)out_ld, lead, pad_mode, quant16);
  return nbm_launch_status();
}

extern "C" int nbm_minmax_init(uint32_t* minmax, int batch, void* stream) {
  if (!minmax || batch <= 0) return NBM_EINVAL;
  hipLaunchKernelGGL(minmax_init_kernel, dim3((batch + 63) / 64), dim3(64), 0, (hipStream_t)stream, minmax, batch);
  return nbm_launch_status();
}

extern "C" int nbm_spec_windows(const float* db, int64_t db_bs, int db_ld, int batch, int n_bins, int n_frames,
                                const uint32_t* minmax, float* img, int n_img, int w_pix, int hop_img,
                                const int32_t* last_cols, void* stream) {
  if (!db || !minmax || !img || !last_cols || batch <= 0 || n_img <= 0 || n_frames <= 0) return NBM_EINVAL;
  if ((n_img - 1) * hop_img >= n_frames) return NBM_EINVAL;
  if ((n_img - 2) * (long long)hop_img + w_pix > n_frames && n_img > 1) return NBM_EINVAL;
  dim3 grid(grid_for((long long)n_bins * w_pix, TPB, 512), n_img, batch);
  hipLaunchKernelGGL(spec_windows_kernel, grid, dim3(TPB), 0, (hipStream_t)stream, db, (long long)db_bs, db_ld,
                     n_bins, minmax, img, n_img, w_pix, hop_img, last_cols);
  return nbm_launch_status();
}

extern "C" int nbm_spec_windows_table(const nbm_window_entry* table, int batch, int n_bins, float* img, int w_pix,
                                      int hop_img, void* stream) {
  if (!table || !img || batch <= 0 || n_bins <= 0 || w_pix <= 0 || hop_img <= 0) return NBM_EINVAL;
  dim3 grid(grid_for((long long)n_bins * w_pix, TPB, 512), batch);
  hipLaunchKernelGGL(spec_windows_table_kernel, grid, dim3(TPB), 0, (hipStream_t)stream, table, n_bins, img, w_pix, hop_img);
  return nbm_launch_status();
}

extern "C" int nbm_init_conv(const float* x, int64_t n_pix, const float* w, const float* b, int C, float* y,
                             void* stream) {
  if (!x || !w || !b || !y || n_pix <= 0 || C <= 0) return NBM_EINVAL;
  hipLaunchKernelGGL(init_conv_kernel, dim3(grid_for(n_pix * C)), dim3(TPB), 0, (hipStream_t)stream, x,
                     (long long)n_pix, w, b, C, y);
  return nbm_launch_status();
}

extern "C" int nbm_maxpool3x3s2(const float* x, int B, int H, int W, int C, float* y, int Ho, int Wo, uint8_t* idx,
                                void* stream) {
  if (!x || !y || B <= 0 || C <= 0 || (C & 3)) return NBM_EINVAL;
  if ((H + 2 - 3) / 2 + 1 != Ho || (W + 2 - 3) / 2 + 1 != Wo) return NBM_EINVAL;
  if (!nbm_aligned16(x) || !nbm_aligned16(y) || (((uintptr_t)idx) & 3u)) return NBM_EALIGN;
  if (idx)
    hipLaunchKernelGGL(maxpool3x3s2_kernel<true>, dim3(grid_for((long long)B * Ho * Wo * (C / 4))), dim3(TPB), 0,
                       (hipStream_t)stream, x, B, H, W, C / 4, y, Ho, Wo, idx);
  else
    hipLaunchKernelGGL(maxpool3x3s2_kernel<false>, dim3(grid_for((long long)B * Ho * Wo * (C / 4))), dim3(TPB), 0,
                       (hipStream_t)stream, x, B, H, W, C / 4, y, Ho, Wo, idx);
  return nbm_launch_status();
}

__global__ void space_to_batch2_kernel(const float* __restrict__ x, int B, int H, int W, int C4, float* __restrict__ y, int inverse) {
  const int Hh = H >> 1, Wh = W >> 1;
  const long long total = (long long)B * H * W * C4;
  const f32x4* x4 = reinterpret_cast<const f32x4*>(x);
  f32x4* y4 = reinterpret_cast<f32x4*>(y);
  for (long long i = blockIdx.x * (long long)blockDim.x + threadIdx.x; i < total; i += (long long)gridDim.x * blockDim.x) {
    const int c = (int)(i % C4);
    long long t = i / C4;
    const int xx = (int)(t % W); t /= W;
    const int yy = (int)(t % H);
    const int n = (int)(t / H);
    const long long packed = ((((long long)((yy & 1) * 2 + (xx & 1)) * B + n) * Hh + (yy >> 1)) * Wh + (xx >> 1)) * C4 + c;
    if (inverse) y4[i] = x4[packed]; else y4[packed] = x4[i];
  }
}

__global__ void avgpool2x2_kernel(const float* __restrict__ x, int B, int Ho, int Wo, int C4, float* __restrict__ y) {
  const long long total = (long long)B * Ho * Wo * C4;
  const f32x4* x4 = reinterpret_cast<const f32x4*>(x);
  f32x4* y4 = reinterpret_cast<f32x4*>(y);
  const int W = 2 * Wo;
  for (long long i = blockIdx.x * (long long)blockDim.x + threadIdx.x; i < total; i += (long long)gridDim.x * blockDim.x) {
    const int c = (int)(i % C4);
    long long t = i / C4;
    const int ox = (int)(t % Wo); t /= Wo;
    const int oy = (int)(t % Ho);
    const int b = (int)(t / Ho);
    const long long r0 = (((long long)b * 2 * Ho + 2 * oy) * W + 2 * ox) * C4 + c;
    const f32x4 a = x4[r0], b1 = x4[r0 + C4], c1 = x4[r0 + (long long)W * C4], d = x4[r0 + (long long)W * C4 + C4];
    f32x4 o;
#pragma unroll
    for (int e = 0; e < 4; ++e) o[e] = (((a[e] + b1[e]) + c1[e]) + d[e]) * 0.25f;
    y4[i] = o;
  }
}

extern "C" int nbm_space_to_batch2(const float* x, int B, int H, int W, int C, float* y, int inverse, void* stream) {
  if (!x || !y || B <= 0 || H <= 0 || W <= 0 || C <= 0 || (C & 3) || (H & 1) || (W & 1)) return NBM_EINVAL;
  if (!nbm_aligned16(x) || !nbm_aligned16(y)) return NBM_EALIGN;
  hipLaunchKernelGGL(space_to_batch2_kernel, dim3(grid_for((long long)B * H * W * (C / 4))), dim3(TPB), 0, (hipStream_t)stream, x, B, H, W,
                     C / 4, y, inverse ? 1 : 0);
  return nbm_launch_status();
}

extern "C" int nbm_avgpool2x2(const float* x, int B, int Ho, int Wo, int C, float* y, void* stream) {
  if (!x || !y || B <= 0 || Ho <= 0 || Wo <= 0 || C <= 0 || (C & 3)) return NBM_EINVAL;
  if (!nbm_aligned16(x) || !nbm_aligned16(y)) return NBM_EALIGN;
  hipLaunchKernelGGL(avgpool2x2_kernel, dim3(grid_for((long long)B * Ho * Wo * (C / 4))), dim3(TPB), 0, (hipStream_t)stream, x, B, Ho, Wo,
                     C / 4, y);
  return nbm_launch_status();
}

extern "C" int nbm_upsample_bilinear_add(const float* src, int B, int Hi, int Wi, int C, const float* add, float* y,
                                         int Ho, int Wo, void* stream) {
  if (!src || !y || B <= 0 || C <= 0 || (C & 3) || Hi <= 0 || Wi <= 0 || Ho <= 0 || Wo <= 0) return NBM_EINVAL;
  if (!nbm_aligned16(src) || !nbm_aligned16(y) || (add && !nbm_aligned16(add))) return NBM_EALIGN;
  const float sh = Ho > 1 ? (float)(Hi - 1) / (float)(Ho - 1) : 0.f;
  const float sw = Wo > 1 ? (float)(Wi - 1) / (float)(Wo - 1) : 0.f;
  hipLaunchKernelGGL(upsample_add_kernel, dim3(grid_for((long long)B * Ho * Wo * (C / 4))), dim3(TPB), 0,
                     (hipStream_t)stream, src, B, Hi, Wi, C / 4, add, y, Ho, Wo, sh, sw);
  return nbm_launch_status();
}

extern "C" int nbm_softmax_rows(float* x, int64_t rows, int cols, int64_t ld, void* stream) {
  if (!x || rows <= 0 || cols <= 0 || ld < cols) return NBM_EINVAL;
  hipLaunchKernelGGL(softmax_rows_kernel, dim3(grid_for(rows, 4, 256 * 32)), dim3(256), 0, (hipStream_t)stream, x,
                     (long long)rows, cols, (long long)ld);
  return nbm_launch_status();
}

extern "C" int nbm_dwconv3x3(const float* x, int B, int H, int W, int Cin, int mult, int stride, const float* w,
                             const float* bias, const float* film, int64_t film_ld, float* y, int Ho, int Wo,
                             void* stream) {
  if (!x || !w || !y || B <= 0 || Cin <= 0 || mult <= 0 || stride <= 0) return NBM_EINVAL;
  if ((H + 2 - 3) / stride + 1 != Ho || (W + 2 - 3) / stride + 1 != Wo) return NBM_EINVAL;
  if (film && film_ld < 2ll * Cin * mult) return NBM_EINVAL;
  const int Cout = Cin * mult;
  const bool vec = (mult == 1 || mult == 2 || mult == 4) && (Cout & 3) == 0 && (Cin % (4 / mult)) == 0 && nbm_aligned16(y) &&
                   nbm_aligned16(x) && (!bias || nbm_aligned16(bias)) && (!film || (nbm_aligned16(film) && (film_ld & 3) == 0));
  if (vec) {
    const dim3 grid(grid_for((long long)B * Ho * Wo * (Cout / 4))), blk(TPB);
    hipStream_t st = (hipStream_t)stream;
    if (mult == 1) hipLaunchKernelGGL(dwconv3x3_vec_kernel<1>, grid, blk, 0, st, x, B, H, W, Cin, stride, w, bias, film, (long long)film_ld, y, Ho, Wo);
    else if (mult == 2) hipLaunchKernelGGL(dwconv3x3_vec_kernel<2>, grid, blk, 0, st, x, B, H, W, Cin, stride, w, bias, film, (long long)film_ld, y, Ho, Wo);
    else hipLaunchKernelGGL(dwconv3x3_vec_kernel<4>, grid, blk, 0, st, x, B, H, W, Cin, stride, w, bias, film, (long long)film_ld, y, Ho, Wo);
    return nbm_launch_status();
  }
  hipLaunchKernelGGL(dwconv3x3_kernel, dim3(grid_for((long long)B * Ho * Wo * Cin * mult)), dim3(TPB), 0,
                     (hipStream_t)stream, x, B, H, W, Cin, mult, stride, w, bias, film, (long long)film_ld, y, Ho, Wo);
  return nbm_launch_status();
}

extern "C" int nbm_layernorm(const float* x, int64_t rows, int E, const float* w, const float* b, float eps, float* y,
                             void* stream) {
  if (!x || !w || !b || !y || rows <= 0 || E <= 0) return NBM_EINVAL;
  hipLaunchKernelGGL(layernorm_kernel, dim3(grid_for(rows, 4, 256 * 32)), dim3(256), 0, (hipStream_t)stream, x,
                     (long long)rows, E, w, b, eps, y);
  return nbm_launch_status();
}

extern "C" int nbm_mha_small(const float* q, const float* k, const float* v, int q_ld, int k_ld, int v_ld, float* out,
                             int out_ld, int S, int N, int nhead, int hd, int64_t seq_stride, int64_t batch_stride,
                             const int32_t* n_valid, float scale, void* stream) {
  if (!q || !k || !v || !out || S <= 0 || S > MHA_SMAX || N <= 0 || nhead <= 0 || hd <= 0 || hd > 64) return NBM_EINVAL;
  if (q_ld < nhead * hd || k_ld < nhead * hd || v_ld < nhead * hd || out_ld < nhead * hd) return NBM_EINVAL;
  hipLaunchKernelGGL(mha_small_kernel, dim3(N * nhead), dim3(256), 0, (hipStream_t)stream, q, k, v, q_ld, k_ld, v_ld, out,
                     out_ld, S, nhead, hd, (long long)seq_stride, (long long)batch_stride, n_valid, scale);
  return nbm_launch_status();
}

extern "C" int nbm_mha_segments(const float* q, const float* k, const float* v, int q_ld, int k_ld, int v_ld, float* out,
                                int out_ld, int B, int R, int nhead, int hd, int mode, const int32_t* segments,
                                const int32_t* n_roi, int max_count, float scale, void* stream) {
  if (!q || !k || !v || !out || !n_roi || B <= 0 || R <= 0 || nhead <= 0 || hd <= 0 || hd > 64) return NBM_EINVAL;
  if (q_ld < nhead * hd || k_ld < nhead * hd || v_ld < nhead * hd || out_ld < nhead * hd) return NBM_EINVAL;
  if (mode == NBM_MHA_ACROSS_ROIS) {
    if (R > MHA_SMAX) return NBM_EINVAL;
  } else if (mode == NBM_MHA_ACROSS_IMAGES) {
    if (!segments || max_count < 1 || max_count > MHA_SMAX) return NBM_EINVAL;
  } else {
    return NBM_EINVAL;
  }
  hipLaunchKernelGGL(mha_segments_kernel, dim3(B * nhead), dim3(256), 0, (hipStream_t)stream, q, k, v, q_ld, k_ld, v_ld, out,
                     out_ld, B, R, nhead, hd, mode, segments, n_roi, max_count, scale);
  return nbm_launch_status();
}

extern "C" int nbm_silu(const float* x, float* y, int64_t n, void* stream) {
  if (!x || !y || n <= 0) return NBM_EINVAL;
  hipLaunchKernelGGL(silu_kernel, dim3(grid_for(n)), dim3(TPB), 0, (hipStream_t)stream, x, y, (long long)n);
  return nbm_launch_status();
}

extern "C" int nbm_pair_softmax(const float* x, int64_t n_pix, int n_anchor, int x_ld, float* y, int y_ld,
                                void* stream) {
  if (!x || !y || n_pix <= 0 || n_anchor <= 0 || x_ld < 2 * n_anchor || y_ld < 2 * n_anchor) return NBM_EINVAL;
  hipLaunchKernelGGL(pair_softmax_kernel, dim3(grid_for(n_pix * n_anchor)), dim3(TPB), 0, (hipStream_t)stream, x,
                     (long long)n_pix, n_anchor, x_ld, y, y_ld);
  return nbm_launch_status();
}
```

birdsoundclassif_amd/nets/_prep.py:

```python
import weakref

import torch
import torch.nn.functional as F

_cache = {}
_epoch = 0


def bump():
    global _epoch
    _epoch += 1


_DEBUG = __import__('os').environ.get('NBM_PREP_DEBUG') == '1'


def _evict(obj_id):
    for k in [k for k in _cache if k[0] == obj_id]:
        hit = _cache.pop(k, None)
        if _DEBUG and hit is not None:
            v = hit[2]
            ts = [t for t in (v if isinstance(v, (tuple, list)) else [v]) if torch.is_tensor(t)]
            print(f'_prep: evicted {k[1]} (key tensor died), values at {[hex(t.data_ptr()) for t in ts]}', flush=True)


def _cached(key_t, tag, fn, extra=(), epoch=True):
    key = (id(key_t), tag)
    ver = (key_t.data_ptr(), key_t._version, key_t.device, _epoch if epoch else -1) + tuple(extra)
    hit = _cache.get(key)
    if hit is not None and hit[0]() is key_t and hit[1] == ver:
        return hit[2]
    with torch.no_grad():
        val = fn()
    if _DEBUG:
        cap = torch.cuda.is_available() and torch.cuda.is_current_stream_capturing()
        print(f'_prep: made {tag} for a {tuple(key_t.shape)} key (replaces an entry: {hit is not None}; during a capture: {cap})', flush=True)
    obj_id = id(key_t)
    _cache[key] = (weakref.ref(key_t, lambda _r, obj_id=obj_id: _evict(obj_id)), ver, val)
    return val


def krsc(weight):
    def make():
        co, ci, kh, kw = weight.shape
        w = weight.detach().permute(0, 2, 3, 1).reshape(co, kh * kw * ci)
        if ci % 32:
            w = F.pad(w, (0, (-w.shape[1]) % 32))
        return w.contiguous()
    return _cached(weight, 'krsc', make)


def _gconv_fragments(weight, groups):
    C, Cg, kh, kw = weight.shape
    if (kh, kw) != (3, 3) or C != groups * Cg or 16 % min(Cg, 16) or Cg % 16 not in (0, Cg) or C % 16:
        raise ValueError(f'gconv: no fragment layout for a {tuple(weight.shape)} weight in {groups} groups')
    w = weight.reshape(C, Cg, 9)
    CI = max(Cg, 16)
    if Cg < 16:
        same = (torch.arange(16, device=w.device)[None, :] // Cg) == ((torch.arange(C, device=w.device) % 16) // Cg)[:, None]
        w = w.repeat(1, 16 // Cg, 1) * same[:, :, None].to(w.dtype)
    return w.reshape(C // 16, 16, CI // 16, 4, 4, 9).permute(0, 5, 2, 3, 1, 4).reshape(C // 16, 9, CI // 16, 64, 4).contiguous()


def gconv(weight, groups):
    return _cached(weight, ('gconv', int(groups)), lambda: _gconv_fragments(weight.detach(), groups))


def gconv_dgrad(weight, groups, scale=None):
    def make():
        C, Cg, kh, kw = weight.shape
        if (kh, kw) != (3, 3) or C != groups * Cg:
            raise ValueError(f'gconv_dgrad: no fragment layout for a {tuple(weight.shape)} weight in {groups} groups')
        w = weight.detach().reshape(groups, Cg, Cg, 3, 3)
        if scale is not None:
            w = w * scale.detach().reshape(groups, Cg, 1, 1, 1)
        return _gconv_fragments(w.transpose(1, 2).flip(3, 4).reshape(C, Cg, 3, 3), groups)
    extra = () if scale is None else (scale.data_ptr(), scale._version)
    return _cached(weight, ('gconv_dgrad', int(groups), scale is not None), make, extra=extra)


def wino23(weight, transposed=False, m=2, scale=None):
    from .. import ops

    def make():
        return ops.wino_weight(weight.detach().contiguous(), transposed, m, None if scale is None else scale.detach().contiguous())
    extra = () if scale is None else (scale.data_ptr(), scale._version)
    return _cached(weight, ('wino', m, transposed, scale is not None), make, extra=extra)


def wino23_weight_grad(dU, m=2, row_scale=None):
    from .. import ops
    return ops.wino_weight_grad(dU, m, row_scale)


def cell_weight(weight, forward=False):
    from .. import ops
    return _cached(weight, ('cell', forward), lambda: ops.cell_weight(weight.detach().contiguous(), forward=forward))


def cell_weight_folded(w_out, wk_lat, alpha, transposed=False):
    from .. import ops
    pair = _cached(w_out, ('cellfold', float(alpha)),
                   lambda: ops.cell_weight(w_out.detach().contiguous(), lateral=wk_lat.detach(), alpha=alpha, both=True),
                   extra=(wk_lat.data_ptr(), wk_lat._version, tuple(wk_lat.shape)))
    return pair[1] if transposed else pair[0]


def cell_weight_grad(dU):
    from .. import ops
    return ops.cell_weight_grad(dU)


def stem_fold(w1, w_init, b_init):
    def make():
        w = w1.detach().double()
        a, b = w_init.detach().double().view(3), b_init.detach().double().view(3)
        we = (w * a.view(1, 3, 1, 1)).sum(1)
        wb = (w * b.view(1, 3, 1, 1)).sum(1)
        weff = torch.zeros((7, 8, 64), dtype=torch.float64, device=w.device)
        weff[:, :7] = we.permute(1, 2, 0)
        return (weff.view(56, 64).float().contiguous(), wb.reshape(64, 49).float().contiguous(), wb.sum((1, 2)).float().contiguous())
    return _cached(w1, 'stem', make, extra=(w_init.data_ptr(), w_init._version, b_init.data_ptr(), b_init._version))


def bn_affine(weight, bias, mean, var, eps, conv_bias=None, frozen=False):
    def make():
        scale = weight.detach() * (var + eps).rsqrt()
        shift = bias.detach() - mean * scale
        if conv_bias is not None:
            shift = shift + conv_bias.detach() * scale
        return scale.contiguous(), shift.contiguous()
    extra = (weight._version, bias._version, mean._version, var._version, None if conv_bias is None else conv_bias._version,
             mean.data_ptr(), var.data_ptr(), bias.data_ptr())
    return _cached(weight, ('bn', conv_bias is not None), make, extra=extra, epoch=not frozen)


def _rpn_composite64(out_w, out_b, dw_w, dw_b, pt_w, rmask, smask, lat_wk, alpha):
    n1, c = out_w.shape[0], out_w.shape[1]
    m_ = dw_w.shape[0]
    mult = m_ // n1
    wo = out_w.detach().double().repeat_interleave(mult, 0)
    wd = dw_w.detach().double().reshape(m_, 3, 3)
    bo = (out_b.detach().double() if out_b is not None else torch.zeros(n1, dtype=torch.float64, device=out_w.device)).repeat_interleave(mult)
    d = torch.zeros((m_, c, 5, 5), dtype=torch.float64, device=out_w.device)
    cb = torch.zeros((m_,), dtype=torch.float64, device=out_w.device)
    for r in range(3):
        for s_ in range(3):
            if (rmask >> r) & 1 and (smask >> s_) & 1:
                d[:, :, r:r + 3, s_:s_ + 3] += wd[:, r, s_, None, None, None] * wo
                cb += wd[:, r, s_] * bo
    if dw_b is not None:
        cb += dw_b.detach().double()
    wp = pt_w.detach().double().reshape(pt_w.shape[0], m_)
    we = torch.einsum('nm,mcae->naec', wp, d)
    const = wp @ cb
    if lat_wk is not None:
        wl = lat_wk.detach().double()
        we = torch.cat([we, float(alpha) * torch.einsum('naec,ci->naei', we, wl)], -1)
    return we, const


def _rpn_extra(out_b, dw_w, dw_b, pt_w, scale, shift, lat_wk, alpha):
    others = [t for t in (out_b, dw_w, dw_b, pt_w, scale, shift, lat_wk) if t is not None]
    return tuple(v for t in others for v in (t.data_ptr(), t._version)) + (float(alpha),)


def rpn_composite(out_w, out_b, dw_w, dw_b, pt_w, scale, shift, lat_wk=None, alpha=1.0, parts=None):
    def make():
        we, const = _rpn_composite64(out_w, out_b, dw_w, dw_b, pt_w, 7, 7, lat_wk, alpha)
        rng = parts if parts is not None else ((0, we.shape[-1]),)
        ws = tuple(we[..., c0:c1].reshape(we.shape[0], -1).float().contiguous() for c0, c1 in rng)
        return ws, scale, (scale.double() * const + shift.double()).float().contiguous()
    return _cached(out_w, ('rpnc', lat_wk is not None, parts), make, extra=_rpn_extra(out_b, dw_w, dw_b, pt_w, scale, shift, lat_wk, alpha))


def rpn_composite_delta(out_w, out_b, dw_w, dw_b, pt_w, scale, shift, rmask, smask, taps, lat_wk=None, alpha=1.0):
    def make():
        we, const = _rpn_composite64(out_w, out_b, dw_w, dw_b, pt_w, rmask, smask, lat_wk, alpha)
        wi, ci = _rpn_composite64(out_w, out_b, dw_w, dw_b, pt_w, 7, 7, lat_wk, alpha)
        d = (we - wi).reshape(we.shape[0], 25, -1)[:, list(taps)] * scale.double()[:, None, None]
        return d.reshape(d.shape[0], -1).float().contiguous(), (scale.double() * (const - ci)).float().contiguous()
    return _cached(out_w, ('rpnd', int(rmask), int(smask), tuple(taps), lat_wk is not None), make,
                   extra=_rpn_extra(out_b, dw_w, dw_b, pt_w, scale, shift, lat_wk, alpha))


def lateral_of_projection(lat_w, lat_b, proj_w, proj_b):
    def make():
        wl = lat_w.detach().double().reshape(lat_w.shape[0], -1)
        wc = wl @ proj_w.detach().double()
        sh = wl @ proj_b.detach().double() + (lat_b.detach().double() if lat_b is not None else 0.0)
        return wc.float().contiguous(), sh.float().contiguous()
    others = [t for t in (lat_b, proj_w, proj_b) if t is not None]
    return _cached(lat_w, 'latproj', make, extra=tuple(v for t in others for v in (t.data_ptr(), t._version)))


def value_of_lateral(lat_w, proj_w, val_w, val_b):
    def make():
        wlo = lat_w.detach().double().reshape(lat_w.shape[0], -1) @ proj_w.detach().double()
        return (wlo @ val_w.detach().double()).float().contiguous(), (wlo @ val_b.detach().double()).float().contiguous()
    others = [proj_w, val_w, val_b]
    return _cached(lat_w, 'vallat', make, extra=tuple(v for t in others for v in (t.data_ptr(), t._version)))


def cat_rows(tag, *tensors):
    def make():
        return torch.cat([t.detach().reshape(t.shape[0], -1) if t.dim() > 1 else t.detach() for t in tensors], 0).contiguous()
    extra = tuple(v for t in tensors for v in (t.data_ptr(), t._version))
    return _cached(tensors[0], ('cat', tag), make, extra=extra)


def clear():
    _cache.clear()
```

birdsoundclassif_amd/nets/backbone.py:

```python
import torch
from torch import nn

from .. import ops
from . import _prep, functional as Fn
from .position_encoding import build_position_encoding

bcbk_channels = {'resnet': {'2': 64, '3': 256, '4': 512, '5': 1024, '6': 2048}}
_RESNET_LAYERS = {'resnet50': [3, 4, 6, 3], 'resnet101': [3, 4, 23, 3], 'resnet152': [3, 8, 36, 3]}
_RESNEXT = {'resnext50_32x4d': ([3, 4, 6, 3], 32, 4), 'resnext101_32x8d': ([3, 4, 23, 3], 32, 8),
            'resnext101_64x4d': ([3, 4, 23, 3], 64, 4)}


class FrozenBatchNorm2d(nn.Module):

    def __init__(self, n):
        super().__init__()
        self.register_buffer('weight', torch.ones(n))
        self.register_buffer('bias', torch.zeros(n))
        self.register_buffer('running_mean', torch.zeros(n))
        self.register_buffer('running_var', torch.ones(n))

    def _load_from_state_dict(self, state_dict, prefix, local_metadata, strict, missing_keys, unexpected_keys,
                              error_msgs):
        state_dict.pop(prefix + 'num_batches_tracked', None)
        super()._load_from_state_dict(state_dict, prefix, local_metadata, strict, missing_keys, unexpected_keys,
                                      error_msgs)

    def affine(self):
        return _prep.bn_affine(self.weight, self.bias, self.running_mean, self.running_var, 1e-5, frozen=True)


class _Bottleneck(nn.Module):

    def __init__(self, inplanes, planes, stride, downsample, norm_layer):
        super().__init__()
        self.conv1 = nn.Conv2d(inplanes, planes, 1, bias=False)
        self.bn1 = norm_layer(planes)
        self.conv2 = nn.Conv2d(planes, planes, 3, stride=stride, padding=1, bias=False)
        self.bn2 = norm_layer(planes)
        self.conv3 = nn.Conv2d(planes, planes * 4, 1, bias=False)
        self.bn3 = norm_layer(planes * 4)
        self.downsample = downsample
        self.stride = stride
        self.mask_input, self.mask_gy = False, True

    def forward(self, x):
        if torch.is_grad_enabled() and x.dim() == 4 and self.conv1.weight.shape[0] % 32 == 0:
            ds = self.downsample
            sd, bd = ds[1].affine() if ds is not None else (None, None)
            return Fn.Bottleneck.apply(x, self.conv1.weight, self.conv2.weight, self.conv3.weight,
                                       ds[0].weight if ds is not None else None, *self.bn1.affine(), *self.bn2.affine(),
                                       *self.bn3.affine(), sd, bd, self.stride, self.mask_input, self.mask_gy)
        s, b = self.bn1.affine()
        o = Fn.conv(x, self.conv1.weight, scale=s, shift=b, act=ops.ACT_RELU)
        s, b = self.bn2.affine()
        if self.stride == 1 and Fn._winograd_ok(o, self.conv2.weight, 3, 3, 1, 1):
            o = ops.conv3x3_winograd(o, _prep.wino23(self.conv2.weight), b, scale=s, relu=True)
        else:
            o = Fn.conv(o, self.conv2.weight, scale=s, shift=b, kh=3, kw=3, stride=self.stride, pad=1, act=ops.ACT_RELU)
        if self.downsample is not None:
            s, b = self.downsample[1].affine()
            idt = Fn.conv(x, self.downsample[0].weight, scale=s, shift=b, stride=self.stride)
        else:
            idt = x
        s, b = self.bn3.affine()
        return Fn.conv(o, self.conv3.weight, scale=s, shift=b, residual=idt, act=ops.ACT_RELU)


class _GroupedBottleneck(nn.Module):

    def __init__(self, inplanes, planes, stride, downsample, norm_layer, groups, base_width):
        super().__init__()
        width = int(planes * base_width / 64) * groups
        self.conv1 = nn.Conv2d(inplanes, width, 1, bias=False)
        self.bn1 = norm_layer(width)
        self.conv2 = nn.Conv2d(width, width, 3, stride=stride, padding=1, groups=groups, bias=False)
        self.bn2 = norm_layer(width)
        self.conv3 = nn.Conv2d(width, planes * 4, 1, bias=False)
        self.bn3 = norm_layer(planes * 4)
        self.downsample = downsample
        self.stride, self.groups = stride, groups
        self.mask_input, self.mask_gy = False, True

    def forward(self, x):
        grad = torch.is_grad_enabled() and (x.requires_grad or any(p.requires_grad for p in self.parameters()))
        if grad and not self.training:
            raise NotImplementedError('a ResNeXt block in eval mode has no backward pass: call .train() on the model to train through it '
                                      '(FrozenBN makes the two modes compute the same), or train with --lr_backbone 0 (a frozen '
                                      'backbone), or run it under torch.no_grad()')
        s, b = self.bn1.affine()
        o = Fn.conv(x, self.conv1.weight, scale=s, shift=b, act=ops.ACT_RELU)
        s, b = self.bn2.affine()
        if grad:
            o = Fn.GConv3x3.apply(o, self.conv2.weight, s, b, self.groups, self.stride)
        else:
            o = ops.gconv3x3(o, _prep.gconv(self.conv2.weight, self.groups), self.groups, stride=self.stride, scale=s, shift=b, relu=True)
        if self.downsample is not None:
            s, b = self.downsample[1].affine()
            idt = Fn.conv(x, self.downsample[0].weight, scale=s, shift=b, stride=self.stride)
        else:
            idt = x
        s, b = self.bn3.affine()
        return Fn.conv(o, self.conv3.weight, scale=s, shift=b, residual=idt, act=ops.ACT_RELU)


class _ResNetBody(nn.Module):

    def __init__(self, layers, norm_layer, dilation=False, groups=1, base_width=64):
        super().__init__()
        self.conv1 = nn.Conv2d(3, 64, 7, stride=2, padding=3, bias=False)
        self.bn1 = norm_layer(64)
        self.dilation = bool(dilation)
        inplanes = 64
        for li, (planes, n, stride) in enumerate(zip((64, 128, 256, 512), layers, (1, 2, 2, 1 if dilation else 2)), start=1):
            blocks = []
            for bi in range(n):
                st = stride if bi == 0 else 1
                ds = None
                if bi == 0 and (st != 1 or inplanes != planes * 4):
                    ds = nn.Sequential(nn.Conv2d(inplanes, planes * 4, 1, stride=st, bias=False), norm_layer(planes * 4))
                blocks.append(_Bottleneck(inplanes, planes, st, ds, norm_layer) if groups == 1 else
                              _GroupedBottleneck(inplanes, planes, st, ds, norm_layer, groups, base_width))
                if dilation and li == 4 and bi > 0:
                    blocks[-1].conv2.dilation, blocks[-1].conv2.padding = (2, 2), (2, 2)
                blocks[-1].mask_input = not (li == 1 and bi == 0)
                blocks[-1].mask_gy = bi == n - 1
                inplanes = planes * 4
            setattr(self, f'layer{li}', nn.Sequential(*blocks))

    def forward(self, x, init_conv=None):
        s, b = self.bn1.affine()
        if init_conv is not None:
            x = Fn.Stem.apply(x, init_conv.weight, init_conv.bias, self.conv1.weight, s, b)
        else:
            x = Fn.conv(x, self.conv1.weight, scale=s, shift=b, kh=7, kw=7, stride=2, pad=3, act=ops.ACT_RELU)
        taps = [x]
        x = Fn.MaxPool.apply(x, True)
        for li in range(1, 5):
            for bi, blk in enumerate(getattr(self, f'layer{li}')):
                if self.dilation and li == 4 and bi == 1:
                    x = Fn.SpaceToBatch2.apply(x, False)
                x = blk(x)
            if self.dilation and li == 4 and len(self.layer4) > 1:
                x = Fn.SpaceToBatch2.apply(x, True)
            taps.append(x)
        return taps


class BackboneBase(nn.Module):

    def __init__(self, backbone, name, in_channels, train_backbone):
        super().__init__()
        for _, parameter in backbone.named_parameters():
            if not train_backbone:
                parameter.requires_grad_(False)
        self.body = backbone
        self.num_channels = list(bcbk_channels['resnet'].values())
        if in_channels != 3:
            self.init_conv = nn.Conv2d(in_channels, 3, 1)
        self.in_channels = in_channels
        self.strides = [2 ** (i + 1) for i in range(len(self.num_channels))]

    def forward(self, x):
        if hasattr(self, 'init_conv'):
            if self.in_channels != 1:
                raise NotImplementedError('init_conv is implemented for 1 input channel (reference default)')
            return self.body(x, self.init_conv)
        return self.body(x)


class Backbone(BackboneBase):

    def __init__(self, name, in_channels, train_backbone, dilation, norm_layer_name):
        if name not in _RESNET_LAYERS and name not in _RESNEXT:
            raise ValueError(f'not supported {name}: the accelerated path implements {sorted(_RESNET_LAYERS) + sorted(_RESNEXT)}')
        if norm_layer_name != 'frozen_batchnorm':
            raise NotImplementedError('only --norm_layer_backbone frozen_batchnorm (reference default) is implemented')
        layers, groups, base_width = _RESNEXT[name] if name in _RESNEXT else (_RESNET_LAYERS[name], 1, 64)
        super().__init__(_ResNetBody(layers, FrozenBatchNorm2d, dilation=dilation, groups=groups, base_width=base_width), name,
                         in_channels, train_backbone)
        if groups > 1 and not train_backbone and hasattr(self, 'init_conv'):
            self.init_conv.requires_grad_(False)


class Joiner(nn.Sequential):
    def __init__(self, backbone, position_embedding):
        super().__init__(backbone, position_embedding)

    def forward(self, x):
        return self[0](x), None


def build_backbone(args):
    position_embedding = build_position_encoding(args)
    train_backbone = args.lr_backbone > 0
    backbone = Backbone(args.backbone, args.inpt_channels, train_backbone, args.dilation, args.norm_layer_backbone)
    model = Joiner(backbone, position_embedding)
    model.num_channels = backbone.num_channels
    model.strides = backbone.strides
    setattr(args, 'n_layers', len(backbone.num_channels))
    return model
```

birdsoundclassif_amd/ops.py:

```python
import collections
import ctypes as C
import os
import math

import torch

from . import _lib
from ._lib import GconvBwdDesc, GconvDesc, GemmDesc, RoiDesc, check

ACT_NONE, ACT_RELU, ACT_SILU, ACT_LEAKY = 0, 1, 2, 3

PROFILE = None
FLOPS = None
FLOPS_DEFERRED = []


def flops_total():
    tot = FLOPS[0] + sum(float(c.item()) * f for c, f in FLOPS_DEFERRED)
    FLOPS_DEFERRED.clear()
    return tot


_PROFILE_LABEL = None
PROFILE_ONLY = None


def _prof_all():
    return PROFILE is not None and PROFILE_ONLY is None


def _prof_fused():
    return PROFILE is not None and PROFILE_ONLY in (None, 'fused')


def is_deepk(Cin, N, kh, kw, rows=None):
    return rows is None and N > 64 and Cin % 32 == 0 and kh * kw * Cin > 256



def _stream():
    return C.c_void_p(torch.cuda.current_stream().cuda_stream)


def _ptr(t):
    return C.c_void_p(t.data_ptr()) if t is not None else C.c_void_p(0)


def _chk(t, dtype=torch.float32, name='tensor'):
    if not (isinstance(t, torch.Tensor) and t.is_cuda):
        raise RuntimeError(f'{name}: the NBM HIP path needs CUDA (ROCm) tensors; no CPU fallback exists')
    if t.dtype != dtype:
        raise TypeError(f'{name}: expected {dtype}, got {t.dtype}')
    if not t.is_contiguous():
        raise ValueError(f'{name}: must be contiguous')
    return t


def lib():
    return _lib.load()


def gemm_conv(x, w, y, *, B, H, W, Cin, N, kh=1, kw=1, stride=1, pad=0, Ho=None, Wo=None,
              x_ld=None, w_ld=None, y_ld=None, scale=None, shift=None, residual=None, res_ld=None,
              groups=1, x_gs=0, w_gs=0, y_gs=0, res_gs=0, alpha=1.0, act=ACT_NONE, shift_per_row=False, up=None,
              rows=None, rows_mode=0, rows_count=0, rows_blocks=None, rows_thw=(0, 0), mask=None, mask_ld=None, bits_out=None):
    Ho = (H + 2 * pad - kh) // stride + 1 if Ho is None else Ho
    Wo = (W + 2 * pad - kw) // stride + 1 if Wo is None else Wo
    d = GemmDesc()
    d.x, d.w, d.y = x.data_ptr(), w.data_ptr(), y.data_ptr()
    d.scale = scale.data_ptr() if scale is not None else None
    d.shift = shift.data_ptr() if shift is not None else None
    d.residual = residual.data_ptr() if residual is not None else None
    d.x_gs, d.w_gs, d.y_gs, d.res_gs = x_gs, w_gs, y_gs, res_gs
    d.groups = groups
    d.B, d.H, d.W, d.Cin, d.N = B, H, W, Cin, N
    d.kh, d.kw, d.stride, d.pad, d.Ho, d.Wo = kh, kw, stride, pad, Ho, Wo
    d.x_ld = Cin if x_ld is None else x_ld
    d.w_ld = kh * kw * Cin if w_ld is None else w_ld
    d.y_ld = N if y_ld is None else y_ld
    d.res_ld = (N if res_ld is None else res_ld) if residual is not None else 0
    d.alpha, d.act, d.shift_per_row = float(alpha), int(act), int(bool(shift_per_row))
    if up is not None:
        d.up, d.up_H, d.up_W = _chk(up, name='up').data_ptr(), up.shape[1], up.shape[2]
    if mask is not None:
        d.mask, d.mask_ld = mask.data_ptr(), int(N if mask_ld is None else mask_ld)
    if bits_out is not None:
        assert bits_out.dtype == torch.int32 and bits_out.is_contiguous() and bits_out.numel() * 32 >= B * Ho * Wo * N and N % 32 == 0
        d.bits_out = bits_out.data_ptr()
    if rows is not None:
        d.rows, d.rows_mode, d.rows_count = rows.data_ptr(), int(rows_mode), int(rows_count)
        d.rows_blocks = rows_blocks.data_ptr() if rows_blocks is not None else None
        d.rows_TH, d.rows_TW = rows_thw
    if FLOPS is not None:
        if rows is None:
            FLOPS[0] += 2.0 * B * Ho * Wo * N * kh * kw * Cin * groups
        elif rows_blocks is None:
            FLOPS[0] += 2.0 * rows_count * N * Cin
        else:
            FLOPS_DEFERRED.append((rows_blocks.clone(), 2.0 * 128 * (16 if rows_mode == 2 else 1) * N * Cin))
    if _prof_all() or (PROFILE is not None and PROFILE_ONLY == 'deepk' and is_deepk(Cin, N, kh, kw, rows)):
        ev0, ev1 = torch.cuda.Event(enable_timing=True), torch.cuda.Event(enable_timing=True)
        ev0.record()
        check(lib().nbm_gemm_conv(C.byref(d), _stream()), 'nbm_gemm_conv')
        ev1.record()
        if rows is None:
            PROFILE.append(((Cin, N, kh, H, W, B, groups, stride, _PROFILE_LABEL), ev0, ev1))
        elif rows_blocks is None:
            PROFILE.append(((Cin, N, kh, rows_count, 1, 1, groups, stride, ('rows', H, W)), ev0, ev1))
        else:
            PROFILE.append(((Cin, N, kh, 0, 1, 1, groups, stride, ('rows-rois', H, W)), ev0, ev1))
        return y
    check(lib().nbm_gemm_conv(C.byref(d), _stream()), 'nbm_gemm_conv')
    return y


def conv2d(x, w, kh=1, kw=1, stride=1, pad=0, scale=None, shift=None, residual=None, act=ACT_NONE,
           alpha=1.0, out=None, w_ld=None, up=None, bits_out=None):
    _chk(x, name='x'), _chk(w, name='w')
    B, H, W, Cin = x.shape
    N = w.shape[0]
    Ho = (H + 2 * pad - kh) // stride + 1
    Wo = (W + 2 * pad - kw) // stride + 1
    y = out if out is not None else torch.empty((B, Ho, Wo, N), device=x.device, dtype=torch.float32)
    if residual is not None:
        _chk(residual, name='residual')
        assert residual.shape == y.shape
    gemm_conv(x, w, y, B=B, H=H, W=W, Cin=Cin, N=N, kh=kh, kw=kw, stride=stride, pad=pad, Ho=Ho, Wo=Wo,
              w_ld=w.shape[1] if w_ld is None else w_ld, scale=scale, shift=shift, residual=residual,
              alpha=alpha, act=act, up=up, bits_out=bits_out)
    return y


def gconv3x3(x, w_prepared, groups, stride=1, scale=None, shift=None, relu=False, out=None, kh=3, kw=3, pad=1):
    _chk(x, name='x'), _chk(w_prepared, name='w_prepared')
    if x.dim() != 4 or w_prepared.dim() != 5 or tuple(w_prepared.shape[1::2]) != (9, 64) or w_prepared.shape[4] != 4 or groups <= 0 \
            or (16 * w_prepared.shape[0]) % groups:
        raise ValueError('gconv3x3: x must be [B,H,W,C] and w_prepared the output of _prep.gconv for these groups')
    B, H, W, x_ld = x.shape
    n_ch = 16 * w_prepared.shape[0]
    Cg = n_ch // groups
    if max(Cg, 16) != 16 * w_prepared.shape[2]:
        raise ValueError(f'gconv3x3: w_prepared {tuple(w_prepared.shape)} does not belong to {groups} groups of {Cg} channels')
    Ho, Wo = (H + 2 * pad - kh) // stride + 1, (W + 2 * pad - kw) // stride + 1
    y = out if out is not None else torch.empty((B, Ho, Wo, n_ch), device=x.device, dtype=torch.float32)
    _chk(y, name='out')
    if y.dim() != 4 or tuple(y.shape[:3]) != (B, Ho, Wo) or y.shape[3] < n_ch or x_ld < n_ch:
        raise ValueError(f'gconv3x3: out must be [{B},{Ho},{Wo},>={n_ch}] and x at least {n_ch} channels wide')
    for v, nm in ((scale, 'scale'), (shift, 'shift')):
        if v is not None and _chk(v, name=nm).numel() != n_ch:
            raise ValueError(f'gconv3x3: {nm} must hold {n_ch} values')
    d = GconvDesc()
    d.x, d.w, d.y = x.data_ptr(), w_prepared.data_ptr(), y.data_ptr()
    d.scale = scale.data_ptr() if scale is not None else None
    d.shift = shift.data_ptr() if shift is not None else None
    d.B, d.H, d.W, d.groups, d.Cg = B, H, W, groups, Cg
    d.kh, d.kw, d.stride, d.pad, d.Ho, d.Wo = kh, kw, stride, pad, Ho, Wo
    d.x_ld, d.y_ld, d.relu = x_ld, y.shape[3], int(bool(relu))
    if FLOPS is not None:
        FLOPS[0] += 2.0 * 9 * Cg * n_ch * B * Ho * Wo
    if _prof_all():
        ev0, ev1 = torch.cuda.Event(enable_timing=True), torch.cuda.Event(enable_timing=True)
        ev0.record()
        check(lib().nbm_gconv3x3(C.byref(d), _stream()), 'nbm_gconv3x3')
        ev1.record()
        PROFILE.append(((Cg, n_ch, kh, H, W, B, groups, stride, 'gconv'), ev0, ev1))
        return y
    check(lib().nbm_gconv3x3(C.byref(d), _stream()), 'nbm_gconv3x3')
    return y


WINO_CHUNK_BYTES = 24 << 30
_WINO_SCRATCH = {}

LANE = 0


class lane:
    def __init__(self, k):
        self.k = int(k)

    def __enter__(self):
        global LANE
        self.prev, LANE = LANE, self.k

    def __exit__(self, *exc):
        global LANE
        LANE = self.prev


def _wino_scratch(device, n_v, n_m):
    need = n_v + n_m
    key = (device, LANE)
    buf = _WINO_SCRATCH.get(key)
    if buf is None or buf.numel() < need:
        if torch.cuda.is_current_stream_capturing():
            raise RuntimeError('the persistent Winograd scratch would have to grow during a graph capture (the warm-up steps of the '
                               'capture must run the same shapes under the same ops.lane)')
        have = 0 if buf is None else buf.numel()
        _WINO_SCRATCH[key] = buf = None
        size = min(max(need, 2 * have), max(need, WINO_CHUNK_BYTES // 4))
        buf = _WINO_SCRATCH[key] = torch.empty((size,), device=device, dtype=torch.float32)
    return buf[:n_v], buf[n_v:need]


GRAPH_NODE_KINDS = ('kernel', 'memcpy', 'memset', 'host', 'empty', 'other')


def graph_census(raw_graph):
    counts = (C.c_longlong * 6)()
    check(_lib.load().nbm_graph_census(C.c_void_p(int(raw_graph)), C.byref(counts)), 'nbm_graph_census')
    return dict(zip(GRAPH_NODE_KINDS, (int(v) for v in counts)))


def lane_buffers(lanes):
    from . import ondemand
    held = [buf for key, buf in _WINO_SCRATCH.items() if key[1] in lanes and buf is not None]
    for key, bufs in ondemand._ROI_TILE_BUF.items():
        if key[2] in lanes:
            held.extend(bufs)
    return held


def release_lane_scratch(keep=(0,)):
    from . import ondemand
    for key in [k for k in _WINO_SCRATCH if k[1] not in keep]:
        del _WINO_SCRATCH[key]
    for key in [k for k in ondemand._ROI_TILE_BUF if k[2] not in keep]:
        del ondemand._ROI_TILE_BUF[key]


def conv3x3_winograd(x, U, bias=None, m=2, scale=None, relu=False, mask=None, residual=None):
    _chk(x, name='x'), _chk(U, name='U')
    B, H, W, C_ = x.shape
    N = U.shape[1]
    nxi = (m + 2) ** 2
    assert U.shape == (nxi, N, C_) and C_ % 32 == 0 and N % 4 == 0
    y = torch.empty((B, H, W, N), device=x.device, dtype=torch.float32)
    tiles = (-(-H // m)) * (-(-W // m))
    fused = m == 2 and C_ >= 64
    assert residual is None or m == 4, 'residual: F(4x4,3x3) output transform only' 
    if fused:
        per_img = 4 * (-(-H // 2)) * (2 * (-(-W // 2)) + 2) * C_ * 4
    else:
        per_img = nxi * tiles * (C_ + N) * 4
    chunk = max(1, min(B, WINO_CHUNK_BYTES // per_img))
    if fused:
        V, M = _wino_scratch(x.device, chunk * per_img // 4, 0)
    else:
        V, M = _wino_scratch(x.device, nxi * chunk * tiles * C_, nxi * chunk * tiles * N)
    st = _stream()
    if _prof_all():
        ev = (torch.cuda.Event(enable_timing=True), torch.cuda.Event(enable_timing=True))
        ev[0].record()
    for b0 in range(0, B, chunk):
        nb = min(chunk, B - b0)
        T = nb * tiles
        mk = _ptr(mask[b0:b0 + nb]) if mask is not None else None
        if fused:
            check(lib().nbm_wino23_rows(_ptr(x[b0:b0 + nb]), nb, H, W, C_, _ptr(V), st), 'nbm_wino23_rows')
            if FLOPS is not None:
                FLOPS[0] += 2.0 * nxi * T * C_ * N
            if _prof_fused():
                e0, e1 = torch.cuda.Event(enable_timing=True), torch.cuda.Event(enable_timing=True)
                e0.record()
            check(lib().nbm_wino23_conv_fused(_ptr(V), _ptr(U), _ptr(scale), _ptr(bias), mk, int(relu), nb, H, W, C_, N,
                                              _ptr(y[b0:b0 + nb]), 0, st), 'nbm_wino23_conv_fused')
            if _prof_fused():
                e1.record()
                PROFILE.append(((C_, N, 1, T, 1, 1, nxi, 1, ('wino23', H, W)), e0, e1))
            continue
        check(lib().nbm_wino_input(_ptr(x[b0:b0 + nb]), nb, H, W, C_, _ptr(V), m, st), 'nbm_wino_input')
        global _PROFILE_LABEL
        _PROFILE_LABEL = ('wino23', H, W)
        try:
            gemm_conv(V, U, M, B=1, H=T, W=1, Cin=C_, N=N, groups=nxi, x_gs=T * C_, w_gs=N * C_, y_gs=T * N)
        finally:
            _PROFILE_LABEL = None
        check(lib().nbm_wino_output(_ptr(M), _ptr(scale), _ptr(bias), mk, int(relu), nb, H, W, N, _ptr(y[b0:b0 + nb]), m,
                                    _ptr(residual[b0:b0 + nb]) if residual is not None else None, st), 'nbm_wino_output')
    if _prof_all():
        ev[1].record()
        PROFILE.append((('wino23', C_, N, H, W, B), *ev))
    return y


def wino_weight(weight, transposed=False, m=2, scale=None):
    _chk(weight, name='weight')
    N, C_ = weight.shape[:2]
    assert tuple(weight.shape[2:]) == (3, 3)
    No, Co = (C_, N) if transposed else (N, C_)
    U = torch.empty(((m + 2) ** 2, No, Co), device=weight.device, dtype=torch.float32)
    check(lib().nbm_wino_weight(_ptr(weight), _ptr(scale), N, C_, int(bool(transposed)), m, _ptr(U), _stream()),
          'nbm_wino_weight')
    return U


def wino_weight_grad(dU, m=2, row_scale=None):
    _chk(dU, name='dU')
    _, N, C_ = dU.shape
    dW = torch.empty((N, C_, 3, 3), device=dU.device, dtype=torch.float32)
    check(lib().nbm_wino_weight_grad(_ptr(dU), _ptr(row_scale), N, C_, m, _ptr(dW), _stream()), 'nbm_wino_weight_grad')
    return dW


def cell_weight(weight, forward=True, lateral=None, alpha=1.0, both=False):
    _chk(weight, name='weight')
    N, C_ = weight.shape[:2]
    assert tuple(weight.shape[2:]) == (3, 3)
    Cin = 0
    if lateral is not None:
        _chk(lateral, name='lateral')
        assert lateral.shape[0] == C_
        Cin = lateral.shape[1]
    K = C_ + Cin
    Unc = torch.empty((25, N, K), device=weight.device, dtype=torch.float32) if (forward or both) else None
    Ucn = torch.empty((25, K, N), device=weight.device, dtype=torch.float32) if (not forward or both) else None
    check(lib().nbm_cell_weight(_ptr(weight), N, C_, _ptr(Unc), K, _ptr(Ucn), K, _stream()), 'nbm_cell_weight')
    if lateral is not None:
        check(lib().nbm_cell_weight_fold(_ptr(weight), _ptr(lateral), lateral.stride(0), N, C_, Cin, float(alpha), _ptr(Unc), K,
                                         _ptr(Ucn), K, _stream()), 'nbm_cell_weight_fold')
    return (Unc, Ucn) if both else (Unc if forward else Ucn)


def copy_rect(strided, base_off, packed, n_outer, outer_pitch, n_rows, row_pitch, width, to_strided=False, zero=False):
    assert strided.dtype == torch.float32 and packed.dtype == torch.float32 and packed.is_contiguous()
    assert packed.numel() >= n_outer * n_rows * width
    assert base_off + (n_outer - 1) * outer_pitch + (n_rows - 1) * row_pitch + width <= strided.numel()
    check(lib().nbm_copy_rect(C.c_void_p(strided.data_ptr() + 4 * base_off), _ptr(packed), n_outer, outer_pitch, n_rows, row_pitch, width,
                              int(bool(to_strided)), int(bool(zero)), _stream()), 'nbm_copy_rect')
    return packed


def cell_weight_grad(dU):
    assert dU.dim() == 3 and dU.shape[0] == 25 and dU.stride(2) == 1 and dU.stride(0) == dU.shape[1] * dU.stride(1)
    _, N, C_ = dU.shape
    dW = torch.empty((N, C_, 3, 3), device=dU.device, dtype=torch.float32)
    check(lib().nbm_cell_weight_grad(_ptr(dU), N, C_, dU.stride(1), _ptr(dW), _stream()), 'nbm_cell_weight_grad')
    return dW


def conv3x3_winograd_wgrad(x, g, want_bias=False, m=2):
    _chk(x, name='x'), _chk(g, name='g')
    B, H, W, C_ = x.shape
    N = g.shape[-1]
    nxi = (m + 2) ** 2
    assert g.shape[:3] == x.shape[:3] and C_ % 4 == 0 and N % 4 == 0
    tiles = (-(-H // m)) * (-(-W // m))
    per_img = nxi * tiles * (C_ + N) * 4
    chunk = max(1, min(B, WINO_CHUNK_BYTES // per_img))
    V, dM = _wino_scratch(x.device, nxi * chunk * tiles * C_, nxi * chunk * tiles * N)
    dU = torch.zeros((nxi, N, C_), device=x.device, dtype=torch.float32)
    gb = torch.zeros((N,), device=x.device, dtype=torch.float32) if want_bias else None
    st = _stream()
    for b0 in range(0, B, chunk):
        nb = min(chunk, B - b0)
        T = nb * tiles
        check(lib().nbm_wino_input(_ptr(x[b0:b0 + nb]), nb, H, W, C_, _ptr(V), m, st), 'nbm_wino_input')
        check(lib().nbm_wino_outgrad(_ptr(g[b0:b0 + nb]), nb, H, W, N, _ptr(dM), _ptr(gb), m, st), 'nbm_wino_outgrad')
        conv_wgrad(dM, V, dU, B=1, H=T, W=1, Cin=C_, N=N, groups=nxi, g_gs=T * N, x_gs=T * C_, out_gs=N * C_)
    return dU, gb


def linear(x2d, w, bias=None, act=ACT_NONE, out=None, alpha=1.0, residual=None, y_ld=None):
    _chk(x2d, name='x'), _chk(w, name='w')
    M, K = x2d.shape
    N = w.shape[0]
    y = out if out is not None else torch.empty((M, N), device=x2d.device, dtype=torch.float32)
    gemm_conv(x2d, w, y, B=1, H=M, W=1, Cin=K, N=N, w_ld=w.shape[1], shift=bias, act=act, alpha=alpha,
              residual=residual, y_ld=y_ld)
    return y


def bgemm_nt(a, b, out=None, alpha=1.0, shift=None, shift_per_row=False, residual=None, act=ACT_NONE):
    _chk(a, name='a'), _chk(b, name='b')
    G, N, K = b.shape
    M = a.shape[-2]
    assert a.shape[-1] == K
    a_gs = M * K if a.dim() == 3 else 0
    y = out if out is not None else torch.empty((G, M, N), device=b.device, dtype=torch.float32)
    gemm_conv(a, b, y, B=1, H=M, W=1, Cin=K, N=N, w_ld=K, groups=G, x_gs=a_gs, w_gs=N * K, y_gs=M * N,
              alpha=alpha, shift=shift, shift_per_row=shift_per_row, residual=residual,
              res_gs=M * N if residual is not None else 0, act=act)
    return y


def pcm16_to_wave(pcm, out_ld, lead, upsample, hq=None, reflect=False, first=0, count=None):
    _chk(pcm, torch.int16, 'pcm')
    batch, n = pcm.shape
    if count is None:
        count = (2 * n if upsample else n) - first
    out = torch.empty((batch, out_ld), device=pcm.device, dtype=torch.float32)
    if upsample:
        _chk(hq, torch.int32, 'hq')
    check(lib().nbm_pcm16_to_wave(_ptr(pcm), n, batch, n, int(bool(upsample)), _ptr(hq), first, count, _ptr(out), out_ld,
                                  lead, int(bool(reflect)), _stream()), 'nbm_pcm16_to_wave')
    return out


WAV_FORMATS = ((1, 8), (1, 16), (1, 24), (1, 32), (3, 32), (3, 64))
WAV_MAX_CHANNELS = 8


def wav_decode(raw, tag, bits, channels, n, out=None):
    if not (isinstance(raw, torch.Tensor) and raw.is_cuda):
        raise RuntimeError('raw: the NBM HIP path needs CUDA (ROCm) tensors; no CPU fallback exists')
    if raw.dtype != torch.uint8 or raw.dim() != 2 or raw.stride(1) != 1:
        raise TypeError('raw: expected uint8 [batch, pitch] rows with unit stride')
    if (int(tag), int(bits)) not in WAV_FORMATS or not 1 <= channels <= WAV_MAX_CHANNELS:
# ... 978 lines not shown
```

include/nbm_hip.h:

```cpp
#ifndef NBM_HIP_H
#define NBM_HIP_H

#include <stdint.h>

#ifdef __cplusplus
extern "C" {
#endif

#define NBM_OK 0
#define NBM_EINVAL (-1)
#define NBM_EALIGN (-2)
#define NBM_EUNSUPPORTED (-3)

#define NBM_ACT_NONE 0
#define NBM_ACT_RELU 1
#define NBM_ACT_SILU 2
#define NBM_ACT_LEAKY 3

const char* nbm_version(void);

int nbm_graph_census(void* graph, long long counts[6]);

typedef struct nbm_gemm_desc {
  const float* x;
  const float* w;
  float* y;
  const float* scale;
  const float* shift;
  const float* residual;
  int64_t x_gs, w_gs, y_gs, res_gs;
  int groups;
  int B, H, W, Cin;
  int N;
  int kh, kw, stride, pad;
  int Ho, Wo;
  int x_ld, w_ld, y_ld, res_ld;
  float alpha;
  int act;
  int shift_per_row;
  const float* up;
  int up_H, up_W;
  const int* rows;
  const int* rows_blocks;
  int rows_mode, rows_count, rows_TH, rows_TW;
  const float* mask;
  int mask_ld;
  unsigned* bits_out;
} nbm_gemm_desc;

int nbm_gemm_conv(const nbm_gemm_desc* d, void* stream);

typedef struct nbm_gconv_desc {
  const float* x;
  const float* w;
  float* y;
  const float* scale;
  const float* shift;
  int B, H, W;
  int groups, Cg;
  int kh, kw, stride, pad;
  int Ho, Wo;
  int x_ld, y_ld;
  int relu;
} nbm_gconv_desc;
int nbm_gconv3x3(const nbm_gconv_desc* d, void* stream);

typedef struct nbm_gconv_bwd_desc {
  const float* g;
  const float* y;
  const float* w;
  const float* x;
  float* out;
  const float* scale;
  void* workspace;
  long long workspace_bytes;
  int B, H, W;
  int groups, Cg;
  int kh, kw, stride, pad;
  int Ho, Wo;
  int g_ld, y_ld, x_ld, out_ld;
  int accumulate;
  int splits;
} nbm_gconv_bwd_desc;
int nbm_gconv3x3_dgrad(const nbm_gconv_bwd_desc* d, void* stream);
int nbm_gconv3x3_wgrad(const nbm_gconv_bwd_desc* d, void* stream);
int nbm_gconv3x3_wgrad_workspace(const nbm_gconv_bwd_desc* d, long long* bytes);

int nbm_wino_input(const float* x, int B, int H, int W, int C, float* V, int m, void* stream);
int nbm_wino_output(const float* M, const float* scale, const float* shift, const float* mask, int relu, int B, int H, int W,
                    int N, float* y, int m, const float* residual, void* stream);
int nbm_wino_outgrad(const float* g, int B, int H, int W, int N, float* dM, float* bias_grad, int m, void* stream);

int nbm_wino_weight(const float* g, const float* scale, int N, int C, int transposed, int m, float* U, void* stream);
int nbm_wino_weight_grad(const float* dU, const float* row_scale, int N, int C, int m, float* dW, void* stream);

int nbm_wino23_rows(const float* x, int B, int H, int W, int C, float* R, void* stream);
int nbm_wino23_conv_fused(const float* R, const float* U, const float* scale, const float* shift, const float* mask,
                          int relu, int B, int H, int W, int C, int N, float* y, int variant, void* stream);

int nbm_wino23_rows_tiles(const float* x, int B, int H, int W, int C, const int* tiles, int n_entries, const int* n_blocks,
                          const unsigned* blk_info, float* R,
                          int skip_pattern_stride ,
                          void* stream);
int nbm_wino23_conv_fused_tiles(const float* R, const float* U, const float* scale, const float* shift, const float* mask,
                                int relu ,
                                int B, int H, int W, int C, int N, float* y, const int* tiles, int n_entries,
                                const int* n_blocks, const unsigned* blk_info, void* stream);
int nbm_roi_tiles(const float* rois, const int* n_roi, int B, int roi_cap, int n_levels, int level, const int* fh,
                  const int* fw, const unsigned char* skip, int dilate, int* tiles, int* n_blocks, void* stream);
int nbm_wino23_input_tiles(const float* x, int B, int H, int W, int C, const int* tiles, int n_list, const unsigned* plane_mask,
                           float* V, void* stream);
int nbm_wino23_outgrad_tiles(const float* g, int B, int H, int W, int N, const int* tiles, int n_list, const unsigned* plane_mask,
                             float* dM, float* bias_grad, int skip_pattern_stride, void* stream);
int nbm_cell_outgrad(const float* g, int B, int H, int W, int N, int stride, float* Vg, float* bias_grad, void* stream);
int nbm_cell_weight(const float* w, int N, int C, float* U_nc, int ld, float* U_cn, int ldt, void* stream);
int nbm_cell_weight_fold(const float* w, const float* w_lat, int wl_ld, int N, int C, int Cin, float alpha, float* U_nc, int ld,
                         float* U_cn, int ldt, void* stream);
int nbm_cell_weight_grad(const float* dU, int N, int C, int ld, float* dW, void* stream);
int nbm_cell_input(const float* x, int B, int H, int W, int C, int stride, float* Vx, int ld ,
                   int c_off , void* stream);
int nbm_cell_input_up(const float* x1, const float* bias, int B, int H, int W, int C, int Hc, int Wc, int stride, float* Vx, int ld,
                      int c_off, void* stream);
int nbm_cell_patches(const float* x, int B, int H, int W, int C, int stride, float* Vx, int ld, int c_off, void* stream);
int nbm_cell_patches_up(const float* x1, const float* bias, int B, int H, int W, int C, int Hc, int Wc, int stride, float* Vx, int ld,
                        int c_off, void* stream);

int nbm_copy_rect(float* strided, float* packed, int64_t n_outer, int64_t outer_pitch, int n_rows, int64_t row_pitch, int64_t width,
                  int to_strided, int zero_strided, void* stream);
int nbm_cell_dgrad_output(const float* M, int B, int H, int W, int C, int stride, float* gx, int parity_class,
                          int ld , int c_off ,
                          float* bias_grad , void* stream);
int nbm_cell_output(const float* M, const float* bias, int B, int H, int W, int N, int stride, float* y, void* stream);


int nbm_pcm16_to_wave(const int16_t* pcm, int64_t pcm_ld, int batch, int n, int upsample,
                      const int32_t* hq, int64_t first, int64_t count, float* out, int64_t out_ld, int lead,
                      int pad_mode, void* stream);

int nbm_resample_to_wave(const float* x, int64_t x_ld, int batch, int64_t n, int L, int M, const double* taps, int T,
                         int64_t first, int64_t count, float* out, int64_t out_ld, int lead, int pad_mode, int quant16,
                         void* stream);

#define NBM_WAV_MAX_CHANNELS 8
int nbm_wav_decode(const void* raw, int64_t raw_pitch, int batch, int tag, int bits, int channels, int64_t n, float* out,
                   int64_t out_pitch, void* stream);

int nbm_minmax_init(uint32_t* minmax, int batch, void* stream);
int nbm_stft_db(const float* wave, int64_t wave_ld, int batch, int n_frames, int hop, int n_fft,
                const double* basis, int basis_bin_tiles, int basis_ksteps, int n_bins, float floor_amp,
                float* db, int64_t db_bs, int db_ld, uint32_t* minmax, void* stream);

int nbm_spec_windows(const float* db, int64_t db_bs, int db_ld, int batch, int n_bins, int n_frames,
                     const uint32_t* minmax, float* img, int n_img, int w_pix, int hop_img,
                     const int32_t* last_cols, void* stream);

typedef struct nbm_window_entry {
  const float* db;
  const uint32_t* minmax;
  const int32_t* last_cols;
  int32_t db_ld, n_frames, window, n_img;
} nbm_window_entry;

int nbm_spec_windows_table(const nbm_window_entry* table, int batch, int n_bins, float* img, int w_pix, int hop_img,
                           void* stream);


int nbm_init_conv(const float* x, int64_t n_pix, const float* w, const float* b, int C, float* y, void* stream);

int nbm_stem7x7(const float* img, int B, int H, int W, const float* weff, const float* wb, const float* wb_full,
                const float* scale, const float* shift, float* y, void* stream);

int nbm_stem7x7_wgrad(const float* img, const float* g, int B, int H, int W, float* D, float* Cb, void* stream);

int nbm_maxpool3x3s2(const float* x, int B, int H, int W, int C, float* y, int Ho, int Wo, uint8_t* idx, void* stream);
int nbm_space_to_batch2(const float* x, int B, int H, int W, int C, float* y, int inverse, void* stream);
int nbm_avgpool2x2(const float* x, int B, int Ho, int Wo, int C, float* y, void* stream);
int nbm_avgpool2x2_bwd(const float* gy, int B, int Ho, int Wo, int C, float* gx, void* stream);

int nbm_upsample_bilinear_add(const float* src, int B, int Hi, int Wi, int C, const float* add,
                              float* y, int Ho, int Wo, void* stream);

int nbm_softmax_rows(float* x, int64_t rows, int cols, int64_t ld, void* stream);

int nbm_dwconv3x3(const float* x, int B, int H, int W, int Cin, int mult, int stride,
                  const float* w , const float* bias, const float* film, int64_t film_ld,
                  float* y, int Ho, int Wo, void* stream);

int nbm_silu(const float* x, float* y, int64_t n, void* stream);

int nbm_layernorm(const float* x, int64_t rows, int E, const float* w, const float* b, float eps, float* y, void* stream);

int nbm_mha_small(const float* q, const float* k, const float* v, int q_ld, int k_ld, int v_ld, float* out, int out_ld,
                  int S, int N, int nhead, int hd, int64_t seq_stride, int64_t batch_stride, const int32_t* n_valid,
                  float scale, void* stream);

#define NBM_MHA_ACROSS_ROIS 0
#define NBM_MHA_ACROSS_IMAGES 1
int nbm_mha_segments(const float* q, const float* k, const float* v, int q_ld, int k_ld, int v_ld, float* out, int out_ld,
                     int B, int R, int nhead, int hd, int mode, const int32_t* segments, const int32_t* n_roi, int max_count,
                     float scale, void* stream);

int nbm_pair_softmax(const float* x, int64_t n_pix, int n_anchor, int x_ld, float* y, int y_ld, void* stream);


int nbm_rpn_decode(const float* cls, const float* reg, const float* anchors , int B, int KA,
                   int n_anchor , int img_w, int img_h, int min_size, float* boxes,
                   uint32_t* keys, int* keep_count, void* stream);

int nbm_nan_images(const float* img, int B, int64_t n, int* keep_count, void* stream);


int nbm_rpn_select(const float* boxes, const uint32_t* keys, const int* keep_count, int B, int KA,
                   int top_n, int fail_below, int cap, float* sel_boxes, float* sel_scores, int* n_sel,
                   const int* seg, void* stream);

int nbm_nms_batched(const float* boxes, const float* scores, const int* n_in, int B, int cap, float thresh,
                    int post_n, uint64_t* mask_ws, int* keep_ws, float* rois, float* roi_scores, int* n_out,
                    const int* seg, void* stream);

int nbm_rpn_select_big_workspace(int B, int cap, int64_t* bytes);
int nbm_rpn_select_big(const float* boxes, const uint32_t* keys, const int* keep_count, int B, int KA, int top_n,
                       int fail_below, int cap, void* ws, int64_t ws_bytes, float* sel_boxes, float* sel_scores,
                       int* n_sel, const int* seg, void* stream);

int nbm_nms_big_workspace(int B, int cap, int64_t* bytes);
int nbm_nms_big(const float* boxes, const float* scores, const int* n_in, int B, int cap, float thresh, int post_n,
                void* ws, int64_t ws_bytes, float* rois, float* roi_scores, int* n_out, const int* seg, void* stream);

typedef struct nbm_roi_desc {
  const float* fmap[5];
  int fh[5], fw[5];
  int n_levels, C;
  const float* rois;
  const int* n_roi;
  int B, roi_cap;
  const float* pe_f; const float* pe_t; int img_h, img_w;
  float* pool; float* pe; int* level;
} nbm_roi_desc;
int nbm_roi_pool(const nbm_roi_desc* d, void* stream);

int nbm_rcnn_post(const float* rois, const int* n_roi, int B, int roi_cap, const float* bbox_reg,
                  const float* bbox_cls, int n_cls1 , int img_w, int img_h,
                  float nms_thresh, float min_score, int proposal_number, float* det, int* n_det, void* stream);

#define NBM_MERGE_MAX_N 131072

int nbm_merge_collect(const float* det, const int* n_det, int n_img, int cap, int num_classes, int w_pix, int hop,
                      int64_t spectrogram_length, int* cell_ws, float* boxes, float* scores, int* species, int* n_out,
                      void* stream);

int nbm_merge_nms_workspace(int cap, int64_t* bytes);

int nbm_merge_nms(const float* boxes, const int* n_in, int cap, float thresh, void* ws, int64_t ws_bytes, int* keep,
                  int* n_keep, void* stream);

int nbm_merge_gather(const float* boxes, const float* scores, const int* species, const int* keep, const int* n_keep, int cap,
                     float* rows, int* n_rows, void* stream);

int nbm_anchor_targets(const float* anchors , int n_in, const float* gt ,
                       const int* n_gt , int B, int G , float neg_t, float pos_t, signed char* lab ,
                       short* amx , int* flag , void* stream);
int nbm_proposal_iou(const float* rois , const float* gt , const int* n_gt , int B, int R, int G,
                     float* mx , int* asg , void* stream);

typedef struct nbm_bwd_desc {
  const float* g;
  const float* w;
  const float* x;
  float* out;
  const float* a_scale;
  const float* row_scale;
  const float* residual;
  const float* mask;
  int64_t g_gs, w_gs, x_gs, out_gs, res_gs;
  int groups;
  int B, H, W, Cin, N, kh, kw, stride, pad, Ho, Wo;
  int g_ld, w_ld, x_ld, out_ld, res_ld, mask_ld;
  float alpha;
  float* bias_grad;
  const float* residual2;
  int res2_ld;
  const unsigned* mask_bits;
} nbm_bwd_desc;

int nbm_conv_dgrad(const nbm_bwd_desc* d, void* stream);
int nbm_conv_wgrad(const nbm_bwd_desc* d, void* stream);

typedef struct nbm_gemm_plan_t {
  const char* name;
  int rc;
  int kernel;
  int grid[3], block;
  int m_tiles, n_tiles;
  int vec_epi;
  int fast;
  int slices;
  int phased;
  int ph_tiles[4];
  int splits, k_chunk;
  int plain, b_generic, narrow_m;
  int halves;
} nbm_gemm_plan_t;
int nbm_gemm_plan(int kind, const void* desc, nbm_gemm_plan_t* out);

int nbm_relu_bwd(const float* gy, const float* y, float* out, int64_t n, void* stream);
int nbm_silu_bwd(const float* gy, const float* x, float* out, int64_t n, void* stream);
int nbm_axpby(const float* a, const float* b, float* out, float alpha, float beta, int64_t n, int64_t b_period, void* stream);
int nbm_weighted_sum(const float* x0, const float* x1, const float* x2, const float* weights, float* out, int64_t n,
                     void* stream);
int nbm_weighted_sum_bwd(const float* x0, const float* x1, const float* x2, const float* weights, const float* g, float* gx0,
                         float* gx1, float* gx2, float* gw, int64_t n, void* stream);
int nbm_zero_roi_windows(float* g, int H, int W, int C, const float* rois , const int* level ,
                         int B, int n_roi, int lvl, void* stream);
int nbm_zero_pattern(float* g, int B, int H, int W, int C, int stride, void* stream);
int nbm_zero_tiles(float* g, int B, int H, int W, int C, const int* tiles, int n_entries, const int* n_blocks, void* stream);
int nbm_tiles_gather(const float* map, int B, int H, int W, int C, const int* tiles, int n_entries, const int* n_blocks, float* compact,
                     void* stream);
int nbm_tiles_scatter_add(float* map, int B, int H, int W, int C, const int* tiles, int n_entries, const int* n_blocks,
                          const float* compact, void* stream);
int nbm_colsum(const float* g, int64_t M, int N, int ld, float* out, void* stream);
int nbm_maxpool3x3s2_bwd(const uint8_t* idx, const float* gy, float* gx, int B, int H, int W, int C, int Ho, int Wo,
                         const float* residual ,
                         const float* mask ,
                         void* stream);
int nbm_leaky_relu_bwd(const float* gy, const float* y, float* out, float slope, int64_t n, void* stream);
int nbm_layernorm_bwd(const float* x, const float* w, const float* g, int64_t rows, int E, float eps, float* gx, float* gw,
                      float* gb, void* stream);
int nbm_mha_small_bwd(const float* q, const float* k, const float* v, const float* go, int q_ld, int k_ld, int v_ld,
                      int go_ld, float* gq, float* gk, float* gv, int gq_ld, int gk_ld, int gv_ld, float* workspace, int S,
                      int N, int nhead, int hd, int64_t seq_stride, int64_t batch_stride, const int32_t* n_valid,
                      float scale, void* stream);
int nbm_upsample_bilinear_bwd(const float* gy, int B, int Hi, int Wi, int C, float* gsrc, int Ho, int Wo, int pattern_stride,
                              void* stream);
int nbm_tiles_upsample_bilinear_bwd_add(const float* compact, int B, int Ho, int Wo, int C, const int* tiles, int n_entries,
                                        const int* n_blocks, float* gsrc, int Hi, int Wi, void* stream);
int nbm_softmax_rows_bwd(const float* p, const float* gp, float* out, int64_t rows, int cols, float alpha, void* stream);
int nbm_pair_softmax_bwd(const float* y, const float* gy, float* gx, int64_t n_pairs, void* stream);
int nbm_dwconv3x3_bwd(const float* x, const float* g, const float* w, int B, int H, int W, int Cin, int mult, int stride,
                      float* gx, float* gw, float* gb, int Ho, int Wo, void* stream);
int nbm_dwconv3x3_bwd_acc(const float* g, const float* w, int B, int H, int W, int Cin, int mult, int stride, float* gx, int Ho,
                          int Wo, void* stream);
int nbm_film_fwd(const float* z, const float* film, float* y, int64_t n_pix, int C, void* stream);
int nbm_film_bwd(const float* gy, const float* z, const float* film, float* gz, float* gfilm, int64_t n_pix, int C,
                 void* stream);
int nbm_bn_train_fwd(const float* x, int64_t M, int C, const float* w, const float* b, float eps, float momentum,
                     float* run_mean, float* run_var, double* stats_ws, float* mean, float* invstd, float* y, void* stream);
int nbm_bn_train_bwd(const float* g, const float* x, int64_t M, int C, const float* mean, const float* invstd,
                     const float* w, double* red_ws, float* gx, float* gw, float* gb, void* stream);
int nbm_roi_pool_bwd(float* const* gfmap_host, const int* fh_host, const int* fw_host, int n_levels, int C,
                     const float* rois, const int* level, int B, int n_roi, const float* gpool, void* stream);
// ... 28 lines not shown
```

Measured before the change: 1064 clips/s.

## Fuse ResNet bottleneck conv3 and downsample shortcut into one concatenated-K GEMM

In inference, the bottleneck block's final 1x1 conv (conv3+bn3) and its projection shortcut (downsample conv+bn) are folded into a single GEMM. The two weight matrices are scaled by their BN factors and concatenated along K, the biases are summed, and a ReLU is applied in the epilogue. A second input pointer (x2, with its own stride and shape) is added to the stream1x1 and h16 kernels so the A operand reads the first Cin channels from o and the rest from x. This removes one kernel launch, the shortcut output write, and the residual read per downsample block. In exchange it adds branching in the inner load path, and it falls back to the old path when planning fails.

After: 1076 clips/s (median of 2 runs). No clear change (+1.1%).

```diff
diff --git a/birdsoundclassif_amd/_lib.py b/birdsoundclassif_amd/_lib.py
--- a/birdsoundclassif_amd/_lib.py
+++ b/birdsoundclassif_amd/_lib.py
@@ -23,7 +23,8 @@
                 ('up', C.c_void_p), ('up_H', C.c_int), ('up_W', C.c_int),
                 ('rows', C.c_void_p), ('rows_blocks', C.c_void_p),
                 ('rows_mode', C.c_int), ('rows_count', C.c_int), ('rows_TH', C.c_int), ('rows_TW', C.c_int),
-                ('mask', C.c_void_p), ('mask_ld', C.c_int), ('bits_out', C.c_void_p)]
+                ('mask', C.c_void_p), ('mask_ld', C.c_int), ('bits_out', C.c_void_p),
+                ('x2', C.c_void_p), ('x2_ld', C.c_int), ('Cin2', C.c_int), ('x2_stride', C.c_int), ('x2_H', C.c_int), ('x2_W', C.c_int)]
 
 
 class GconvDesc(C.Structure):
diff --git a/birdsoundclassif_amd/csrc/igemm.hip b/birdsoundclassif_amd/csrc/igemm.hip
--- a/birdsoundclassif_amd/csrc/igemm.hip
+++ b/birdsoundclassif_amd/csrc/igemm.hip
@@ -258,9 +258,10 @@
   const float* x; const float* w; float* y; const float* scale; const float* shift; const float* residual;
   int M, x_ld, w_ld, y_ld, res_ld, m_tiles; float alpha; int act;
   unsigned* bits_out; int n_words;
+  const float* x2; int x2_ld, k32a;
 };
 constexpr int SPITCH = 36;
-template <int K32, int NT, int NTG, int WAVES>
+template <int K32, int NT, int NTG, int WAVES, bool X2 = false>
 __global__ __launch_bounds__(WAVES * 64, 1) void stream1x1_kernel(const StreamParams p) {
   constexpr int K = K32 * 32, N = NT * 32, WP = K + 4;
   constexpr bool CHUNKED = K32 > 2;
@@ -283,7 +284,14 @@
     m = m < p.M ? m : p.M - 1;
     return p.x + (long long)m * p.x_ld + 16 * lh;
   };
-  auto load_chunk = [&](const float* xp, int kc, f32x4* dst) {
+  auto row_ptr2 = [&](int tile) -> const float* {
+    if constexpr (!X2) return nullptr;
+    int m = tile * 32 + li;
+    m = m < p.M ? m : p.M - 1;
+    return p.x2 + ((long long)m * p.x2_ld + 16 * lh - p.k32a * 32);
+  };
+  auto load_chunk = [&](const float* xp, int kc, f32x4* dst, const float* xp2 = nullptr) {
+    if constexpr (X2) xp = kc >= p.k32a ? xp2 : xp;
 #pragma unroll
     for (int q = 0; q < 4; ++q) dst[q] = *reinterpret_cast<const f32x4*>(xp + kc * 32 + 4 * q);
   };
@@ -291,19 +299,21 @@
   int tile = blockIdx.x * WAVES + wave;
   if (tile < p.m_tiles) {
     const float* xp = row_ptr(tile);
-#pragma unroll
-    for (int kc = 0; kc < K32; ++kc) load_chunk(xp, kc, CHUNKED ? a[kc] : an[kc]);
+    const float* xp2 = row_ptr2(tile);
+#pragma unroll
+    for (int kc = 0; kc < K32; ++kc) load_chunk(xp, kc, CHUNKED ? a[kc] : an[kc], xp2);
   }
   for (; tile < p.m_tiles; tile += step) {
     const bool more = tile + step < p.m_tiles;
     const float* xn = row_ptr(more ? tile + step : tile);
+    const float* xn2 = row_ptr2(more ? tile + step : tile);
     if constexpr (!CHUNKED) {
 #pragma unroll
       for (int kc = 0; kc < K32; ++kc)
 #pragma unroll
         for (int q = 0; q < 4; ++q) a[kc][q] = an[kc][q];
 #pragma unroll
-      for (int kc = 0; kc < K32; ++kc) load_chunk(xn, kc, an[kc]);
+      for (int kc = 0; kc < K32; ++kc) load_chunk(xn, kc, an[kc], xn2);
     }
     const int m0 = tile * 32;
     f32x4 rq[NTG][4];
@@ -339,7 +349,7 @@
               for (int e = 0; e < 4; ++e) acc[j] = __builtin_amdgcn_mfma_f32_32x32x2f32(a[kc][q][e], b[q][e], acc[j], 0, 0, 0);
           }
           __builtin_amdgcn_sched_barrier(0);
-          load_chunk(xn, kc, a[kc]);
+          load_chunk(xn, kc, a[kc], xn2);
           __builtin_amdgcn_sched_barrier(0);
         }
       } else {
@@ -447,11 +457,12 @@
   const int M = d->B * d->Ho * d->Wo;
   if (pl.slices) {
     const StreamParams sp{d->x, d->w, d->y, d->scale, d->shift, d->residual, M, d->x_ld, d->w_ld, d->y_ld, d->res_ld, pl.m_tiles,
-                          d->alpha, d->act, d->bits_out, d->N >> 5};
+                          d->alpha, d->act, d->bits_out, d->N >> 5, d->x2, d->x2_ld, d->Cin >> 5};
     switch (pl.kernel) {
       case K_STREAM_64_256: hipLaunchKernelGGL((stream1x1_kernel<2, 8, 4, 8>), grid, block, 0, st, sp); break;
       case K_STREAM_64_64: hipLaunchKernelGGL((stream1x1_kernel<2, 2, 2, 8>), grid, block, 0, st, sp); break;
       case K_STREAM_128_SLICED: hipLaunchKernelGGL((stream1x1_kernel<4, 4, 4, 8>), grid, block, 0, st, sp); break;
+      case K_STREAM_128_X2: hipLaunchKernelGGL((stream1x1_kernel<4, 4, 4, 8, true>), grid, block, 0, st, sp); break;
       default: hipLaunchKernelGGL((stream1x1_kernel<8, 2, 2, 8>), grid, block, 0, st, sp); break;
     }
     return nbm_launch_status();
@@ -459,7 +470,7 @@
   IgemmParams p{};
   p.x = d->x; p.w = d->w; p.y = d->y; p.scale = d->scale; p.shift = d->shift; p.residual = d->residual;
   p.x_gs = d->x_gs; p.w_gs = d->w_gs; p.y_gs = d->y_gs; p.res_gs = d->res_gs;
-  p.M = M; p.N = d->N; p.K = d->kh * d->kw * d->Cin;
+  p.M = M; p.N = d->N; p.K = d->kh * d->kw * d->Cin + (d->x2 ? d->Cin2 : 0);
   p.nk = (p.K + BK - 1) / BK;
   p.H = d->H; p.W = d->W; p.Cin = d->Cin; p.kh = d->kh; p.kw = d->kw; p.stride = d->stride; p.pad = d->pad;
   p.Ho = d->Ho; p.Wo = d->Wo; p.HoWo = d->Ho * d->Wo;
@@ -469,6 +480,7 @@
   p.m_tiles = pl.m_tiles; p.n_tiles = pl.n_tiles; p.vec_epi = pl.vec_epi;
   if (d->mask) { p.mask = d->mask; p.mask_ld = d->mask_ld; }
   p.bits_out = d->bits_out;
+  if (d->x2) { p.x2 = d->x2; p.x2_ld = d->x2_ld; p.x2_stride = d->x2_stride; p.x2_H = d->x2_H; p.x2_W = d->x2_W; }
   if (d->up) {
     p.up = d->up; p.up_H = d->up_H; p.up_W = d->up_W;
     p.up_sh = d->Ho > 1 ? (float)(d->up_H - 1) / (float)(d->Ho - 1) : 0.f;
@@ -482,7 +494,7 @@
   switch (pl.kernel) {
     case K_FWD_ROWS: hipLaunchKernelGGL((igemm_kernel<128, 128, 64, 64, A_FAST, EPI_STD, 1, true>), grid, block, 0, st, p); break;
     case K_FWD_SPLIT_R0: case K_FWD_SPLIT_R2: case K_FWD_SPLIT_R4: return split_launch(p, pl, st);
-    case K_FWD_H16: return h16_launch(p, pl, st);
+    case K_FWD_H16: case K_FWD_H16_X2: return h16_launch(p, pl, st);
     case K_FWD_128_S1: hipLaunchKernelGGL((igemm_kernel<128, 128, 64, 64, A_FAST, EPI_STD, 1>), grid, block, 0, st, p); break;
     case K_FWD_128_FAST: hipLaunchKernelGGL((igemm_kernel<128, 128, 64, 64, A_FAST, EPI_STD>), grid, block, 0, st, p); break;
     case K_FWD_128_GENERIC: hipLaunchKernelGGL((igemm_kernel<128, 128, 64, 64, A_GENERIC, EPI_STD>), grid, block, 0, st, p); break;
diff --git a/birdsoundclassif_amd/csrc/igemm_h16.hip b/birdsoundclassif_amd/csrc/igemm_h16.hip
--- a/birdsoundclassif_amd/csrc/igemm_h16.hip
+++ b/birdsoundclassif_amd/csrc/igemm_h16.hip
@@ -10,6 +10,7 @@
 constexpr int P16 = 20;
 enum { EPI_STD = 0 };
 
+template <bool X2>
 __global__ __launch_bounds__(256, 3) void igemm_h16_kernel(const IgemmParams p) {
   constexpr int STAGES = 1, EPI = EPI_STD;
   constexpr bool ROWS = false;
@@ -63,6 +64,23 @@
   }
   const __amdgpu_buffer_rsrc_t rsrc_a = __builtin_amdgcn_make_buffer_rsrc(const_cast<float*>(xg + blk_base), 0, 0x7ffffff0, 0x00020000);
   const __amdgpu_buffer_rsrc_t rsrc_b = __builtin_amdgcn_make_buffer_rsrc(const_cast<float*>(wgp), 0, 0x7ffffff0, 0x00020000);
+  unsigned a2_rel[2] = {0u, 0u};
+  long long blk_base2 = 0;
+  if constexpr (X2) {
+    auto base2 = [&](int m) -> long long {
+      const int b = (int)nbm_fdiv((unsigned)m, p.fd_howo), rem = m - b * p.HoWo;
+      const int oy = (int)nbm_fdiv((unsigned)rem, p.fd_wo), ox = rem - oy * p.Wo;
+      return ((long long)(b * p.x2_H + oy * p.x2_stride) * p.x2_W + ox * p.x2_stride) * p.x2_ld;
+    };
+    blk_base2 = base2(bm0 < p.M ? bm0 : 0);
+#pragma unroll
+    for (int i = 0; i < 2; ++i) {
+      const int m = bm0 + r0 + 64 * i;
+      a2_rel[i] = m < p.M ? ((unsigned)(base2(m) - blk_base2) + koff) * 4u : 0x80000000u;
+    }
+  }
+  const __amdgpu_buffer_rsrc_t rsrc_a2 =
+      __builtin_amdgcn_make_buffer_rsrc(const_cast<float*>(X2 ? p.x2 + blk_base2 : xg + blk_base), 0, 0x7ffffff0, 0x00020000);
 
   f32x4 ra[2], rb[2];
   int cur_r = 0, cur_s = 0, cur_c0 = 0, cur_h = 0;
@@ -70,10 +88,21 @@
     const int tap = cur_r * p.kw + cur_s;
     const unsigned a_soff = (unsigned)((((long long)cur_r * p.W + cur_s) * p.x_ld + cur_c0 + 8 * cur_h) * 4);
     const unsigned b_soff = (unsigned)((tap * p.Cin + cur_c0 + 8 * cur_h) * 4);
-#pragma unroll
-    for (int i = 0; i < 2; ++i) {
-      const unsigned vo = ((a_taps[i] >> tap) & 1ull) ? a_rel[i] : 0x80000000u;
-      ra[i] = __builtin_bit_cast(f32x4, __builtin_amdgcn_raw_buffer_load_b128(rsrc_a, vo, a_soff, 0));
+    if constexpr (X2) {
+      const bool second = cur_c0 >= p.Cin;
+      const __amdgpu_buffer_rsrc_t rs = second ? rsrc_a2 : rsrc_a;
+      const unsigned soff = (unsigned)((cur_c0 - (second ? p.Cin : 0) + 8 * cur_h) * 4);
+#pragma unroll
+      for (int i = 0; i < 2; ++i) {
+        const unsigned vo = second ? a2_rel[i] : (a_taps[i] & 1ull) ? a_rel[i] : 0x80000000u;
+        ra[i] = __builtin_bit_cast(f32x4, __builtin_amdgcn_raw_buffer_load_b128(rs, vo, soff, 0));
+      }
+    } else {
+#pragma unroll
+      for (int i = 0; i < 2; ++i) {
+        const unsigned vo = ((a_taps[i] >> tap) & 1ull) ? a_rel[i] : 0x80000000u;
+        ra[i] = __builtin_bit_cast(f32x4, __builtin_amdgcn_raw_buffer_load_b128(rsrc_a, vo, a_soff, 0));
+      }
     }
 #pragma unroll
     for (int i = 0; i < 2; ++i)
@@ -166,6 +195,7 @@
 }
 
 int nbm_igemm::h16_launch(const IgemmParams& p, const GemmPlan& pl, hipStream_t st) {
-  hipLaunchKernelGGL(igemm_h16_kernel, dim3(pl.grid[0], pl.grid[1], pl.grid[2]), dim3(256), 0, st, p);
+  if (pl.kernel == K_FWD_H16_X2) hipLaunchKernelGGL(igemm_h16_kernel<true>, dim3(pl.grid[0], pl.grid[1], pl.grid[2]), dim3(256), 0, st, p);
+  else hipLaunchKernelGGL(igemm_h16_kernel<false>, dim3(pl.grid[0], pl.grid[1], pl.grid[2]), dim3(256), 0, st, p);
   return nbm_launch_status();
 }
diff --git a/birdsoundclassif_amd/csrc/igemm_params.h b/birdsoundclassif_amd/csrc/igemm_params.h
--- a/birdsoundclassif_amd/csrc/igemm_params.h
+++ b/birdsoundclassif_amd/csrc/igemm_params.h
@@ -20,6 +20,7 @@
   const float* mask; int mask_ld;
   unsigned* bits_out;
   nbm_fastdiv fd_howo, fd_wo, fd_rows_thw, fd_rows_tw;
+  const float* x2; int x2_ld, x2_stride, x2_H, x2_W;
 };
 
 int split_launch(const IgemmParams& p, const GemmPlan& pl, hipStream_t st);
diff --git a/birdsoundclassif_amd/csrc/igemm_plan.h b/birdsoundclassif_amd/csrc/igemm_plan.h
--- a/birdsoundclassif_amd/csrc/igemm_plan.h
+++ b/birdsoundclassif_amd/csrc/igemm_plan.h
@@ -59,7 +59,9 @@
   X(K_TN_64_STRIDED, "igemm_tn_kernel<64,1,128>")                                                                                    \
   X(K_SPLIT_TN_R0, "igemm_split_tn_kernel<0>")                              \
   X(K_SPLIT_TN_R2, "igemm_split_tn_kernel<2>")                                                                                       \
-  X(K_SPLIT_TN_R4, "igemm_split_tn_kernel<4>")
+  X(K_SPLIT_TN_R4, "igemm_split_tn_kernel<4>")                                                                                        \
+  X(K_STREAM_128_X2, "stream1x1_kernel<4,4,4,8,true>")                     \
+  X(K_FWD_H16_X2, "igemm_h16_kernel<true>")
 
 enum GemmKernel {
 #define X(id, name) id,
@@ -84,6 +86,7 @@
 constexpr int STREAM_MIN_ROWS = 8192;
 constexpr int SPLIT_TN_MIN_ROWS = 192;
 constexpr long long ROWS_SPAN_MAX = 0x7fffffffll;
+constexpr long long X2_SPAN_MAX = 0x70000000ll;
 constexpr long long DGRAD_SPAN_MAX = 0x70000000ll;
 constexpr long long TN_SPAN_MAX = 0x40000000ll;
 
@@ -112,8 +115,17 @@
     return plan_error(NBM_EINVAL);
   if ((d.H + 2 * d.pad - d.kh) / d.stride + 1 != d.Ho || (d.W + 2 * d.pad - d.kw) / d.stride + 1 != d.Wo) return plan_error(NBM_EINVAL);
   if (d.x_ld < d.Cin || d.y_ld < d.N || (d.residual && d.res_ld < d.N)) return plan_error(NBM_EINVAL);
+  if (d.x2) {
+    if (d.Cin2 <= 0 || d.x2_stride <= 0 || d.x2_H <= 0 || d.x2_W <= 0 || d.x2_ld < d.Cin2) return plan_error(NBM_EINVAL);
+    if (d.kh != 1 || d.kw != 1 || d.stride != 1 || d.pad != 0 || d.groups != 1 || d.rows || d.up || d.mask || d.bits_out || d.shift_per_row ||
+        (d.Cin % PLAN_BK) || (d.Cin2 % PLAN_BK) || (d.x2_ld & 3) || !aligned16(d.x2))
+      return plan_error(NBM_EUNSUPPORTED);
+    if ((d.x2_H - 1) / d.x2_stride + 1 != d.Ho || (d.x2_W - 1) / d.x2_stride + 1 != d.Wo) return plan_error(NBM_EINVAL);
+    if (sw.split_bf16) return plan_error(NBM_EUNSUPPORTED);
+    if (129ll * d.x2_stride * d.x2_W * d.x2_ld * 4 > X2_SPAN_MAX) return plan_error(NBM_EUNSUPPORTED);
+  }
   GemmPlan pl{};
-  const int taps = d.kh * d.kw, K = taps * d.Cin, nk = (K + PLAN_BK - 1) / PLAN_BK;
+  const int taps = d.kh * d.kw, K = taps * d.Cin + (d.x2 ? d.Cin2 : 0), nk = (K + PLAN_BK - 1) / PLAN_BK;
   if (d.N > 128 && (d.N & 127) == 64 && !d.rows && !d.up && !d.bits_out && !d.shift_per_row && (d.Cin % PLAN_BK) == 0 && K > SHORTK_STEPS * PLAN_BK) {
     nbm_gemm_desc a = d;
     a.N = d.N - 64;
@@ -128,7 +140,7 @@
                 (!d.scale || aligned16(d.scale)) && (!d.shift || d.shift_per_row || aligned16(d.shift)) &&
                 (!d.mask || ((d.mask_ld & 3) == 0 && aligned16(d.mask))))
                    ? 1 : 0;
-  if ((d.w_ld & 3) || (d.w_gs & 3) || !aligned16(d.w)) return plan_error(NBM_EALIGN);
+  if ((d.w_ld & 3) || (d.w_gs & 3) || !aligned16(d.w)) return plan_error(d.x2 ? NBM_EUNSUPPORTED : NBM_EALIGN);
   if (d.bits_out && (!pl.vec_epi || (d.N & 31) || d.groups != 1 || d.rows)) return plan_error(NBM_EUNSUPPORTED);
   if (d.up && (!pl.vec_epi || d.groups != 1 || d.up_H <= 0 || d.up_W <= 0 || !aligned16(d.up))) return plan_error(NBM_EUNSUPPORTED);
   pl.fast = ((d.Cin % PLAN_BK) == 0 && (d.x_ld & 3) == 0 && (d.x_gs & 3) == 0 && aligned16(d.x)) ? 1 : 0;
@@ -148,9 +160,12 @@
   }
   if (sw.stream1x1 && d.kh == 1 && d.kw == 1 && d.stride == 1 && d.pad == 0 && d.groups == 1 && fast_vec && !d.up && !d.mask &&
       !d.shift_per_row && (d.N % 32) == 0 && M >= STREAM_MIN_ROWS) {
-    const int k32 = d.Cin / 32, nt = d.N / 32;
+    const int k32 = K / 32, nt = d.N / 32;
     int kernel = -1, wg_per_cu = 1, slices = 1;
-    if (k32 == 2 && nt == 8 && d.residual) kernel = K_STREAM_64_256;
+    if (d.x2) {
+      if (k32 == 4 && d.x2_stride == 1 && nt % 4 == 0 && nt <= 32) kernel = K_STREAM_128_X2, slices = nt / 4;
+    }
+    else if (k32 == 2 && nt == 8 && d.residual) kernel = K_STREAM_64_256;
     else if (k32 == 2 && nt == 2) kernel = K_STREAM_64_64, wg_per_cu = 2;
     else if (k32 == 8 && nt == 2) kernel = K_STREAM_256_64;
     else if (d.residual && k32 == 4 && nt % 4 == 0 && nt <= 32) kernel = K_STREAM_128_SLICED, slices = nt / 4;
@@ -165,6 +180,12 @@
       plan_kernel(pl, kernel, wgs < gx ? wgs : gx, slices, 1, waves * 64);
       return pl;
     }
+  }
+  if (d.x2) {
+    if (!(sw.h16 && fast_vec && nk >= DEEPK_STEPS)) return plan_error(NBM_EUNSUPPORTED);
+    pl.n_tiles = (d.N + 127) / 128;
+    plan_kernel(pl, K_FWD_H16_X2, pl.m_tiles * pl.n_tiles, 1, 1);
+    return pl;
   }
   if (d.N > 64) {
     pl.n_tiles = (d.N + 127) / 128;
diff --git a/birdsoundclassif_amd/csrc/pointwise.hip b/birdsoundclassif_amd/csrc/pointwise.hip
--- a/birdsoundclassif_amd/csrc/pointwise.hip
+++ b/birdsoundclassif_amd/csrc/pointwise.hip
@@ -561,7 +561,7 @@
 
 }
 
-extern "C" const char* nbm_version(void) { return "nbm_hip 0.5 (gfx950)"; }
+extern "C" const char* nbm_version(void) { return "nbm_hip 0.6 (gfx950)"; }
 
 extern "C" int nbm_graph_census(void* graph, long long counts[6]) {
   if (!graph || !counts) return NBM_EINVAL;
diff --git a/birdsoundclassif_amd/nets/_prep.py b/birdsoundclassif_amd/nets/_prep.py
--- a/birdsoundclassif_amd/nets/_prep.py
+++ b/birdsoundclassif_amd/nets/_prep.py
@@ -133,6 +133,21 @@
     extra = (weight._version, bias._version, mean._version, var._version, None if conv_bias is None else conv_bias._version,
              mean.data_ptr(), var.data_ptr(), bias.data_ptr())
     return _cached(weight, ('bn', conv_bias is not None), make, extra=extra, epoch=not frozen)
+
+
+def shortcut_fold(w3, bn3, wd, bnd):
+    bufs = [t for bn in (bn3, bnd) for t in (bn.weight, bn.bias, bn.running_mean, bn.running_var)]
+
+    def make():
+        def affine64(bn):
+            sc = bn.weight.detach().double() * (bn.running_var.double() + 1e-5).rsqrt()
+            return sc, bn.bias.detach().double() - bn.running_mean.double() * sc
+        (s3, b3), (sd, bd) = affine64(bn3), affine64(bnd)
+        n = w3.shape[0]
+        wcat = torch.cat([w3.detach().double().reshape(n, -1) * s3[:, None], wd.detach().double().reshape(n, -1) * sd[:, None]], 1)
+        return wcat.float().contiguous(), (b3 + bd).float().contiguous()
+    extra = (wd.data_ptr(), wd._version) + tuple(v for t in bufs for v in (t.data_ptr(), t._version))
+    return _cached(w3, 'scfold', make, extra=extra, epoch=w3.requires_grad or wd.requires_grad)
 
 
 def _rpn_composite64(out_w, out_b, dw_w, dw_b, pt_w, rmask, smask, lat_wk, alpha):
diff --git a/birdsoundclassif_amd/nets/backbone.py b/birdsoundclassif_amd/nets/backbone.py
--- a/birdsoundclassif_amd/nets/backbone.py
+++ b/birdsoundclassif_amd/nets/backbone.py
@@ -1,3 +1,5 @@
+import os
+
 import torch
 from torch import nn
 
@@ -9,6 +11,21 @@
 _RESNET_LAYERS = {'resnet50': [3, 4, 6, 3], 'resnet101': [3, 4, 23, 3], 'resnet152': [3, 8, 36, 3]}
 _RESNEXT = {'resnext50_32x4d': ([3, 4, 6, 3], 32, 4), 'resnext101_32x8d': ([3, 4, 23, 3], 32, 8),
             'resnext101_64x4d': ([3, 4, 23, 3], 64, 4)}
+
+
+SHORTCUT_FOLD = os.environ.get('NBM_SHORTCUT_FOLD', '1') != '0'
+
+
+def _conv3_folded(blk, o, x):
+    if not (isinstance(blk.bn3, FrozenBatchNorm2d) and isinstance(blk.downsample[1], FrozenBatchNorm2d)):
+        return None
+    wcat, shift = _prep.shortcut_fold(blk.conv3.weight, blk.bn3, blk.downsample[0].weight, blk.downsample[1])
+    B, Ho, Wo, cmid = o.shape
+    y = torch.empty((B, Ho, Wo, wcat.shape[0]), device=o.device, dtype=torch.float32)
+    kw = dict(B=B, H=Ho, W=Wo, Cin=cmid, N=wcat.shape[0], shift=shift, act=ops.ACT_RELU, x2=x, x2_stride=blk.stride)
+    if ops.gemm_plan(0, ops.gemm_desc(o, wcat, y, **kw)).rc:
+        return None
+    return ops.gemm_conv(o, wcat, y, **kw)
 
 
 class FrozenBatchNorm2d(nn.Module):
@@ -59,6 +76,10 @@
         else:
             o = Fn.conv(o, self.conv2.weight, scale=s, shift=b, kh=3, kw=3, stride=self.stride, pad=1, act=ops.ACT_RELU)
         if self.downsample is not None:
+            if SHORTCUT_FOLD and not torch.is_grad_enabled() and x.dim() == 4:
+                y = _conv3_folded(self, o, x)
+                if y is not None:
+                    return y
             s, b = self.downsample[1].affine()
             idt = Fn.conv(x, self.downsample[0].weight, scale=s, shift=b, stride=self.stride)
         else:
diff --git a/birdsoundclassif_amd/ops.py b/birdsoundclassif_amd/ops.py
--- a/birdsoundclassif_amd/ops.py
+++ b/birdsoundclassif_amd/ops.py
@@ -60,10 +60,11 @@
     return _lib.load()
 
 
-def gemm_conv(x, w, y, *, B, H, W, Cin, N, kh=1, kw=1, stride=1, pad=0, Ho=None, Wo=None,
+def gemm_desc(x, w, y, *, B, H, W, Cin, N, kh=1, kw=1, stride=1, pad=0, Ho=None, Wo=None,
               x_ld=None, w_ld=None, y_ld=None, scale=None, shift=None, residual=None, res_ld=None,
               groups=1, x_gs=0, w_gs=0, y_gs=0, res_gs=0, alpha=1.0, act=ACT_NONE, shift_per_row=False, up=None,
-              rows=None, rows_mode=0, rows_count=0, rows_blocks=None, rows_thw=(0, 0), mask=None, mask_ld=None, bits_out=None):
+              rows=None, rows_mode=0, rows_count=0, rows_blocks=None, rows_thw=(0, 0), mask=None, mask_ld=None, bits_out=None,
+              x2=None, x2_ld=None, Cin2=None, x2_stride=1, x2_hw=None):
     Ho = (H + 2 * pad - kh) // stride + 1 if Ho is None else Ho
     Wo = (W + 2 * pad - kw) // stride + 1 if Wo is None else Wo
     d = GemmDesc()
@@ -76,7 +77,6 @@
     d.B, d.H, d.W, d.Cin, d.N = B, H, W, Cin, N
     d.kh, d.kw, d.stride, d.pad, d.Ho, d.Wo = kh, kw, stride, pad, Ho, Wo
     d.x_ld = Cin if x_ld is None else x_ld
-    d.w_ld = kh * kw * Cin if w_ld is None else w_ld
     d.y_ld = N if y_ld is None else y_ld
     d.res_ld = (N if res_ld is None else res_ld) if residual is not None else 0
     d.alpha, d.act, d.shift_per_row = float(alpha), int(act), int(bool(shift_per_row))
@@ -91,19 +91,36 @@
         d.rows, d.rows_mode, d.rows_count = rows.data_ptr(), int(rows_mode), int(rows_count)
         d.rows_blocks = rows_blocks.data_ptr() if rows_blocks is not None else None
         d.rows_TH, d.rows_TW = rows_thw
+    if x2 is not None:
+        d.x2 = _chk(x2, name='x2').data_ptr()
+        d.x2_H, d.x2_W = x2.shape[1:3] if x2_hw is None else x2_hw
+        d.Cin2 = int(x2.shape[-1] if Cin2 is None else Cin2)
+        d.x2_ld = int(x2.shape[-1] if x2_ld is None else x2_ld)
+        d.x2_stride = int(x2_stride)
+    d.w_ld = kh * kw * Cin + d.Cin2 if w_ld is None else w_ld
+    return d
+
+
+def gemm_conv(x, w, y, *, rows_blocks=None, **kw):
+    d = gemm_desc(x, w, y, rows_blocks=rows_blocks, **kw)
+    B, H, W, Cin, N, kh, kw_, stride, groups, Ho, Wo = d.B, d.H, d.W, d.Cin, d.N, d.kh, d.kw, d.stride, d.groups, d.Ho, d.Wo
+    rows, rows_mode, rows_count = d.rows, d.rows_mode, d.rows_count
+    Kc = kh * kw_ * Cin + d.Cin2
     if FLOPS is not None:
         if rows is None:
-            FLOPS[0] += 2.0 * B * Ho * Wo * N * kh * kw * Cin * groups
+            FLOPS[0] += 2.0 * B * Ho * Wo * N * Kc * groups
         elif rows_blocks is None:
             FLOPS[0] += 2.0 * rows_count * N * Cin
         else:
             FLOPS_DEFERRED.append((rows_blocks.clone(), 2.0 * 128 * (16 if rows_mode == 2 else 1) * N * Cin))
-    if _prof_all() or (PROFILE is not None and PROFILE_ONLY == 'deepk' and is_deepk(Cin, N, kh, kw, rows)):
+    if _prof_all() or (PROFILE is not None and PROFILE_ONLY == 'deepk' and is_deepk(Kc // (kh * kw_), N, kh, kw_, rows)):
         ev0, ev1 = torch.cuda.Event(enable_timing=True), torch.cuda.Event(enable_timing=True)
         ev0.record()
         check(lib().nbm_gemm_conv(C.byref(d), _stream()), 'nbm_gemm_conv')
         ev1.record()
-        if rows is None:
+        if d.x2:
+            PROFILE.append(((Kc, N, kh, H, W, B, groups, stride, _PROFILE_LABEL or ('x2', Cin, d.Cin2, d.x2_stride)), ev0, ev1))
+        elif rows is None:
             PROFILE.append(((Cin, N, kh, H, W, B, groups, stride, _PROFILE_LABEL), ev0, ev1))
         elif rows_blocks is None:
             PROFILE.append(((Cin, N, kh, rows_count, 1, 1, groups, stride, ('rows', H, W)), ev0, ev1))
diff --git a/include/nbm_hip.h b/include/nbm_hip.h
--- a/include/nbm_hip.h
+++ b/include/nbm_hip.h
@@ -46,6 +46,8 @@
   const float* mask;
   int mask_ld;
   unsigned* bits_out;
+  const float* x2;
+  int x2_ld, Cin2, x2_stride, x2_H, x2_W;
 } nbm_gemm_desc;
 
 int nbm_gemm_conv(const nbm_gemm_desc* d, void* stream);
```
